# wexiangis/wmix

Hardware: AMD Instinct MI355X
Metric: 10 ms frames/s (higher is better)
Workload: dtype f32

## Files before the change

include/wmix_amd.h:

```cpp
#ifndef WMIX_AMD_H
#define WMIX_AMD_H

#include <stddef.h>
#include <stdint.h>

#ifdef __cplusplus
extern "C" {
#endif

#define WMX_EINVAL (-10001)
#define WMX_ENODEV (-10002)
#define WMX_ESTATE (-10003)
#define WMX_EHIP_BASE (-11000)
#define WMX_IS_HIP_ERROR(rc) ((rc) <= WMX_EHIP_BASE && (rc) > WMX_EHIP_BASE - 10000)

const char *wmx_last_error(void);
int wmx_device_count(void);
int wmx_handle_device(const void *handle);
int wmx_version(void);
const char *wmx_build_info(void);



#define WMX_LAW_A 0
// ... 227 lines not shown
int wmx_rtp_reset_streams(wmx_rtp *h, const int32_t *host_idx, int n, void *stream);
int wmx_rtp_export(wmx_rtp *h, int stream_index, uint16_t *seq, uint32_t *timestamp);
#define WMX_RTP_SEQ_MISORDER 16
#define WMX_RTP_CALLS_COUNT(c) ((c) & 7u)
#define WMX_RTP_CALLS_SLOT(c, j) (((c) >> (4 + 4 * (j))) & 3u)
#define WMX_RTP_CALLS_SILENCE(c, j) (((c) >> (6 + 4 * (j))) & 1u)
int wmx_rtp_sequence_legs(wmx_rtp *h, int max_packets, int max_gap, const uint16_t *d_seq_raw, uint32_t *d_len, uint32_t *d_calls,
                          void *stream);
int wmx_rtp_reset_sequence(wmx_rtp *h, const int32_t *host_idx, int n, void *stream);
int wmx_rtp_export_sequence(wmx_rtp *h, uint16_t *next, uint8_t *synced, uint32_t *lost, uint32_t *late, uint32_t *dup,
                            uint32_t *resync, uint32_t *overflow, void *stream);
int wmx_rtp_conceal_legs(wmx_rtp *h, int max_packets, const int16_t *d_pcm, long source_stride, long pcm_packet_stride,
                         const uint32_t *d_len, const uint32_t *d_calls, int16_t *d_pcm_out, uint32_t *d_len_out, void *stream);
int wmx_rtp_reset_conceal(wmx_rtp *h, const int32_t *host_idx, int n, void *stream);
int wmx_rtp_export_conceal(wmx_rtp *h, int16_t *hist, uint32_t *concealed, void *stream);
int wmx_rtp_detect_dtmf_legs(wmx_rtp *h, int max_packets, const uint8_t *d_in, long leg_stride, long packet_stride,
                             const int32_t *d_recv, int16_t *d_pcm, long source_stride, long pcm_packet_stride, const uint32_t *d_len,
                             const uint32_t *d_calls, int event_pt, int suppress, void *stream);
int wmx_rtp_reset_dtmf(wmx_rtp *h, const int32_t *host_idx, int n, void *stream);
int wmx_rtp_export_dtmf(wmx_rtp *h, uint32_t *count, uint8_t *ring, void *stream);
#define WMX_CODEC_REFERENCE 0
#define WMX_CODEC_PCMA 1
#define WMX_CODEC_PCMU 2
#define WMX_CODEC_BY_PT 3
int wmx_rtp_set_codecs(wmx_rtp *h, const int32_t *host_idx, int n, int in_codec, int out_law, void *stream);
int wmx_rtp_export_codecs(wmx_rtp *h, uint8_t *in_codec, uint8_t *out_law, uint32_t *refused, void *stream);
int wmx_rtp_ingest_legs_codecs(wmx_rtp *h, int max_packets, const uint8_t *d_packets, long leg_stride, long packet_stride,
                               const int32_t *d_recv_bytes, int16_t *d_pcm, long source_stride, long pcm_packet_stride,
                               uint32_t *d_len, uint16_t *d_seq_raw, void *stream);

typedef struct wmx_pipe wmx_pipe;
int wmx_pipe_create(wmx_pipe **out, int n_streams, int slots, int law, int agc_value, unsigned stages);
int wmx_pipe_create_pcm(wmx_pipe **out, int n_streams, int slots, int chn, int freq, int interval_ms, int agc_value, unsigned stages);
int wmx_pipe_create_pcm_calls(wmx_pipe **out, int n_streams, int slots, int chn, int freq, int interval_ms, int agc_value, unsigned stages);
int wmx_pipe_destroy(wmx_pipe *h);
int wmx_pipe_slots(const wmx_pipe *h);
int wmx_pipe_datagram_bytes(const wmx_pipe *h);
uint8_t *wmx_pipe_in(wmx_pipe *h, int slot);
const uint8_t *wmx_pipe_out(wmx_pipe *h, int slot);
int16_t *wmx_pipe_far(wmx_pipe *h, int slot);
int wmx_pipe_submit(wmx_pipe *h, const int16_t *d_far, int *slot, void *stream);
int wmx_pipe_wait(wmx_pipe *h, int slot);
long wmx_pipe_failed_steps(const wmx_pipe *h);
int wmx_pipe_poll(wmx_pipe *h, int slot);
int wmx_pipe_step_resident(wmx_pipe *h, const uint8_t *d_in, long in_stride, const int16_t *d_far, uint8_t *d_out, long out_stride,
                           void *stream);
wmx_chain *wmx_pipe_chain(wmx_pipe *h);
wmx_rtp *wmx_pipe_senders(wmx_pipe *h);

typedef struct wmx_conf wmx_conf;
int wmx_conf_create(wmx_conf **out, int n_legs, int slots, int max_packets, int law);
int wmx_conf_destroy(wmx_conf *h);
int wmx_conf_set_conferences(wmx_conf *h, int n_conf, const int32_t *host_off, const int32_t *host_members, void *stream);
int wmx_conf_mute(wmx_conf *h, const uint8_t *host_mask, void *stream);
int wmx_conf_speakers(wmx_conf *h, int max_speakers, uint32_t floor, int decay_shift);
int wmx_conf_sequence(wmx_conf *h, int on, int max_gap);
int wmx_conf_export_sequence(wmx_conf *h, uint16_t *next, uint8_t *synced, uint32_t *lost, uint32_t *late, uint32_t *dup,
                             uint32_t *resync, uint32_t *overflow, void *stream);
int wmx_conf_conceal(wmx_conf *h, int on);
int wmx_conf_export_conceal(wmx_conf *h, uint32_t *concealed, void *stream);
int wmx_conf_dtmf(wmx_conf *h, int on, int suppress, int event_pt);
int wmx_conf_export_dtmf(wmx_conf *h, uint32_t *count, uint8_t *ring, void *stream);
int wmx_conf_denoise(wmx_conf *h, int on);
wmx_nsx *wmx_conf_denoiser(wmx_conf *h);
int wmx_conf_level(wmx_conf *h, int on, int value);
wmx_agc *wmx_conf_leveller(wmx_conf *h);
int wmx_conf_gate(wmx_conf *h, int on);
wmx_vad *wmx_conf_gater(wmx_conf *h);
int wmx_conf_export_gate(wmx_conf *h, uint8_t *reduce, uint32_t *voiced, uint32_t *unvoiced, void *stream);
int wmx_conf_set_codecs(wmx_conf *h, const int32_t *host_idx, int n, int in_codec, int out_law, void *stream);
int wmx_conf_export_codecs(wmx_conf *h, uint8_t *in_codec, uint8_t *out_law, uint32_t *refused, void *stream);
int wmx_conf_set_play_correct(wmx_conf *h, uint32_t bytes);
int wmx_conf_reset_legs(wmx_conf *h, const int32_t *host_idx, int n, void *stream);
int wmx_conf_slots(const wmx_conf *h);
int wmx_conf_in_row_bytes(const wmx_conf *h);
uint8_t *wmx_conf_in(wmx_conf *h, int slot);
int32_t *wmx_conf_recv(wmx_conf *h, int slot);
const uint8_t *wmx_conf_out(wmx_conf *h, int slot);
int wmx_conf_next_slot(const wmx_conf *h);
int wmx_conf_submit(wmx_conf *h, int *slot, void *stream);
int wmx_conf_wait(wmx_conf *h, int slot);
int wmx_conf_poll(wmx_conf *h, int slot);
int wmx_conf_step_resident(wmx_conf *h, const uint8_t *d_in, const int32_t *d_recv, uint8_t *d_out, void *stream);
int wmx_conf_export_legs(wmx_conf *h, uint32_t *head, uint32_t *tick, uint32_t *dropped, uint32_t *env, uint8_t *speaking, void *stream);
wmx_mix *wmx_conf_mix(wmx_conf *h);
wmx_rtp *wmx_conf_senders(wmx_conf *h);

typedef struct wmx_rt wmx_rt;
int wmx_rt_create_pcm(wmx_rt **out, long n_streams, int sub_batch, int slots, int chn, int freq, int interval_ms, int agc_value, unsigned stages);
int wmx_rt_create_rtp(wmx_rt **out, long n_streams, int sub_batch, int slots, int law, int agc_value, unsigned stages);
int wmx_rt_create_pcm_calls(wmx_rt **out, long n_streams, int sub_batch, int slots, int chn, int freq, int interval_ms, int agc_value, unsigned stages);
int wmx_rt_destroy(wmx_rt *h);
int wmx_rt_set_compute_streams(wmx_rt *h, int n);
int wmx_rt_batches(const wmx_rt *h);
int wmx_rt_batch_streams(const wmx_rt *h, int batch);
wmx_pipe *wmx_rt_pipe(wmx_rt *h, int batch);
int16_t *wmx_rt_far(wmx_rt *h, int slot);
int wmx_rt_submit(wmx_rt *h, const int16_t *d_far, int *slot, void *stream);
#define WMX_DROPPED 1
int wmx_rt_try_submit(wmx_rt *h, const int16_t *d_far, int *slot, void *stream);
long wmx_rt_dropped_ticks(const wmx_rt *h);
int wmx_rt_next_slot(const wmx_rt *h);
int wmx_rt_wait(wmx_rt *h);
int wmx_rt_poll(wmx_rt *h);
int wmx_rt_tick(wmx_rt *h, const int16_t *d_far, int *slot, void *stream);
int wmx_rt_step_resident(wmx_rt *h, uint8_t *d_rows, long stride, const int16_t *d_far, uint8_t *d_out, long out_stride, void *stream);

typedef struct wmx_pkgfifo wmx_pkgfifo;
int wmx_pkgfifo_create(wmx_pkgfifo **out, int n_streams, int n_slots, int pkg_bytes, int interval_ms, int frame_bytes);
int wmx_pkgfifo_destroy(wmx_pkgfifo *h);
int wmx_pkgfifo_add(wmx_pkgfifo *h, const uint8_t *d_pkgs, long stride, void *stream);
int wmx_pkgfifo_get(wmx_pkgfifo *h, uint8_t *d_out, long stride, int delayms, void *stream);

typedef struct wmx_tick wmx_tick;
int wmx_tick_create(wmx_tick **out, int n_groups, int rec_per_group, int chn, int freq, int interval_ms, int aec_delay_ms, int agc_value,
                    unsigned stages);
int wmx_tick_destroy(wmx_tick *h);
int wmx_tick_set_stages(wmx_tick *h, unsigned stages, int agc_value);
int wmx_tick_play_ns(wmx_tick *h, int on);
int wmx_tick_rw_test(wmx_tick *h, int on);
int wmx_tick_bridge(wmx_tick *h, int parties);
int wmx_tick_bridge_mute(wmx_tick *h, const uint8_t *host_mask, void *stream);
int wmx_tick_bridge_conferences(wmx_tick *h, int n_conf, const int32_t *host_off, const int32_t *host_members, void *stream);
int wmx_tick_bridge_speakers(wmx_tick *h, int max_speakers, uint32_t floor, int decay_shift);
int wmx_tick_bridge_speaking(wmx_tick *h, uint8_t *host_speaking, uint32_t *host_env, void *stream);
int wmx_tick_set_play_correct(wmx_tick *h, uint32_t bytes);
int wmx_tick_package_samples(const wmx_tick *h);
int wmx_tick_load(wmx_tick *h, const int16_t *d_src, uint32_t srcU8Len, int freq, int channels, int sample, int n_src, long group_stride,
                  long source_stride, int reduce, uint32_t *head, uint32_t *tick, void *stream);
int wmx_tick_play(wmx_tick *h, int16_t *d_play, long play_stride, void *stream);
const int16_t *wmx_tick_far(const wmx_tick *h);
int wmx_tick_record(wmx_tick *h, int16_t *d_rec, long rec_stride, int16_t *d_rec_1x8000, long out_stride, uint32_t out_capacity,
                    uint32_t *out_len, void *stream);
int wmx_tick_run(wmx_tick *h, int16_t *d_play, long play_stride, int16_t *d_rec, long rec_stride, int16_t *d_rec_1x8000, long out_stride,
                 uint32_t out_capacity, uint32_t *out_len, void *stream);
wmx_mix *wmx_tick_mix(wmx_tick *h);
wmx_chain *wmx_tick_chain(wmx_tick *h);
wmx_pkgfifo *wmx_tick_fifo(wmx_tick *h);

int wmx_debug_fft(int kind, int n_batch, void *d_data, int32_t *d_aux, void *stream);
int wmx_debug_spl(int kind, const int32_t *d_a, const int32_t *d_b, const int32_t *d_c, int32_t *d_y, size_t n, void *stream);
int wmx_debug_ns_libm(int kind, const float *x, float *y, size_t n);
int wmx_debug_ns_libm_device(int kind, const float *d_x, const float *d_a, const float *d_b, float *d_y, size_t n, void *stream);
int wmx_debug_ns_libm_dbl(int kind, const float *x, double *y, size_t n);
int wmx_debug_ns_libm_dbl_device(int kind, const float *d_x, double *d_y, size_t n, void *stream);
int wmx_debug_aec_libm_device(int kind, const float *d_x, float *d_y, size_t n, void *stream);
int wmx_debug_ns_window(int L, float *host_window);
int wmx_debug_div(const float *d_a, const float *d_b, float *d_q_ordinary, float *d_q_ieee, size_t n, void *stream);
int wmx_debug_div_host(const float *a, const float *b, float *q, size_t n);
int wmx_debug_aec_decide(const float *sd_rows, const float *se_rows, const int32_t *prev_state, int32_t *out, size_t n);
int wmx_debug_aec_decide_device(const float *d_sd_rows, const float *d_se_rows, const int32_t *d_prev_state, int32_t *d_out, size_t n, void *stream);
int wmx_debug_pow(const float *x, const float *e, float *y, size_t n);
int wmx_debug_pow_device(const float *d_x, const float *d_e, float *d_y, size_t n, void *stream);

#ifdef __cplusplus
}
#endif
#endif
```

wmix_amd/csrc/aec.hip:

```cpp
#include <algorithm>
#include <chrono>
#include <cmath>
#include <cstdlib>
#include <cstring>
#include <cstddef>
#include <unordered_map>
#include <vector>
#include "wmx_internal.h"
#include "aec_ctl.h"
#include "aec_gate.h"
#include "cohort_hip.h"
#include "fft_regs.h"
#include "libm_dev.h"

namespace wmx {
namespace {

constexpr int BP = 68;
enum : int {
    AS_W_RE = 0,
    AS_W_IM = AS_W_RE + 12 * BP,
    AS_DPOW = AS_W_IM + 12 * BP,
    AS_DMIN = AS_DPOW + BP,
    AS_DINIT = AS_DMIN + BP,
    AS_SD = AS_DINIT + BP,
    AS_SE = AS_SD + BP,
    AS_SX = AS_SE + BP,
    AS_SDE_RE = AS_SX + BP,
    AS_SDE_IM = AS_SDE_RE + BP,
    AS_SXD_RE = AS_SDE_IM + BP,
    AS_SXD_IM = AS_SXD_RE + BP,
    AS_DPREV = AS_SXD_IM + BP,
    AS_EPREV = AS_DPREV + 64,
    AS_OUTBUF = AS_EPREV + 64,
    AS_NEAR_RING = AS_OUTBUF + 64,
    AS_OUT_RING = AS_NEAR_RING + kAecRing,
    AS_SCAL = AS_OUT_RING + kAecRing,
    AS_HNLFBMIN = AS_SCAL + 0,
    AS_HNLFBLOCALMIN = AS_SCAL + 1,
    AS_HNLXDAVGMIN = AS_SCAL + 2,
    AS_OVERDRIVE = AS_SCAL + 3,
    AS_OVERDRIVESM = AS_SCAL + 4,
    AS_HNLNEWMIN = AS_SCAL + 5,
    AS_HNLMINCTR = AS_SCAL + 6,
    AS_DELAYIDX = AS_SCAL + 7,
    AS_STNEAR = AS_SCAL + 8,
    AS_ECHOSTATE = AS_SCAL + 9,
    AS_DIVERGE = AS_SCAL + 10,
    AS_NOISECTR = AS_SCAL + 12,
    AS_DELAYCTR = AS_SCAL + 13,
    AS_NSEED = AS_SCAL + 11,
    AS_WORDS = AS_SCAL + 16,
};
static_assert(AS_WORDS % 4 == 0, "state block must be a whole number of 16-byte chunks");

struct AecFarBufs {
    float *pre;
    float *tring;
    float *hist;
    float *nyq;
    float *hist_w;
    float *xpow_seq;
    float *xpow;
    size_t group_words;
};
__device__ __forceinline__ AecFarBufs far_group(const AecFarBufs &F, int g) {
    const size_t o = (size_t)g * F.group_words;
    return AecFarBufs{F.pre + o, F.tring + o, F.hist + o, F.nyq + o, F.hist_w + o, F.xpow_seq + o, F.xpow + o, F.group_words};
}

struct AecConsts {
    FftTables tab;
    float hanning[BP], weight[BP], overdrive[BP];
};
constexpr int kAecConstWords = sizeof(AecConsts) / 4;
struct AecConstsNear {
    FftTables tab;
    float hanning[BP];
};
static_assert(offsetof(AecConsts, weight) == sizeof(AecConstsNear), "AecConstsNear is a prefix of AecConsts");
constexpr int kAecConstNearWords = sizeof(AecConstsNear) / 4;

__device__ __forceinline__ float sat16f(float v) { return v > 32767.f ? 32767.f : (v < -32768.f ? -32768.f : v); }

__device__ __forceinline__ v2f cmul_conj_w(float wr, float wi, v2f t) { return v2f{wr, wr} * t + v2f{wi, -wi} * swap(t); }

__device__ __forceinline__ void unpack_bin(const float *a, int b, float &re, float &im) {
    if (b == 0) {
        re = a[0];
        im = 0.f;
    } else if (b == kAecPart) {
        re = a[1];
        im = 0.f;
    } else {
        re = a[2 * b];
        im = a[2 * b + 1];
    }
}

template <class Src>
__device__ __forceinline__ void aec_fft_fwd(float *row, const FftTables *T, int gl, Src src) {
    Cx v[4];
#pragma unroll
    for (int m = 0; m < 4; m++) v[m] = src(fft64_src_point(gl, m));
    fft64_regs<false>(v, T, gl);
#pragma unroll
    for (int m = 0; m < 4; m++) *reinterpret_cast<float2 *>(row + 2 * (gl + 16 * m)) = make_float2(v[m].r, v[m].i);
}

__global__ __launch_bounds__(64) void aec_far_kernel(AecFarBufs F_all, const float *__restrict__ consts_g, AecPlan *plans,
                                                     int n_packets, int n_classes, const int32_t *__restrict__ plan_of,
                                                     const int16_t *far_pcm, long far_packet_stride,
                                                     long far_group_stride, int chn, float gpow1np, int plan_by_value,
                                                     const AecPlan plan_value) {
    __shared__ AecConstsNear K;
    __shared__ float fa[4][132];
    const int lane = threadIdx.x;
    if (plan_by_value) {
        const int *src = reinterpret_cast<const int *>(&plan_value);
        int *dst = reinterpret_cast<int *>(plans);
        constexpr int NW = (int)(sizeof(AecPlan) / 4), NIT = (NW + 63) / 64;
        int v[NIT];
#pragma unroll
        for (int k = 0; k < NIT; k++) v[k] = src[lane + 64 * k < NW ? lane + 64 * k : 0];
#pragma unroll
        for (int k = 0; k < NIT; k++)
            if (lane + 64 * k < NW) dst[lane + 64 * k] = v[k];
        __threadfence();
        wave_sync();
    }
    const AecFarBufs F = far_group(F_all, (int)blockIdx.x);
    if (far_pcm) far_pcm += (size_t)blockIdx.x * far_group_stride;
    plans += plan_of ? plan_of[blockIdx.x] : (int)blockIdx.x;
    __shared__ float lpre[kAecPreLen];
    float xp0, xp1;
    {
        float *dst = reinterpret_cast<float *>(&K);
        constexpr int NIT = (kAecConstNearWords + 63) / 64, NP = kAecPreLen / 64;
        static_assert(kAecPreLen % 64 == 0, "whole rows of the pre-buffer per lane");
        float c[NIT], pr[NP];
#pragma unroll
        for (int k = 0; k < NIT; k++) c[k] = consts_g[lane + 64 * k < kAecConstNearWords ? lane + 64 * k : 0];
#pragma unroll
        for (int k = 0; k < NP; k++) pr[k] = F.pre[lane + 64 * k];
        xp0 = F.xpow[lane];
        xp1 = F.xpow[lane == 0 ? kAecPart : 0];
#pragma unroll
        for (int k = 0; k < NIT; k++)
            if (lane + 64 * k < kAecConstNearWords) dst[lane + 64 * k] = c[k];
#pragma unroll
        for (int k = 0; k < NP; k++) lpre[lane + 64 * k] = pr[k];
    }
    wave_sync();
    bool xpow_dirty = false;
    __shared__ int lplan[sizeof(AecPlan) / 4];
    for (int p = 0; p < n_packets; p++) {
        {
            const int *src = reinterpret_cast<const int *>(&plans[(size_t)p * n_classes]);
            constexpr int NW = (int)(sizeof(AecPlan) / 4);
            static_assert(NW <= 64, "one word of the plan per lane");
            wave_sync();
            if (lane < NW) lplan[lane] = src[lane];
            wave_sync();
        }
        const AecPlan &lp = *reinterpret_cast<const AecPlan *>(lplan);
        auto rf = [](int v) { return __builtin_amdgcn_readfirstlane(v); };
        struct {
            int has_far, far_n, pre_wr, n_part, n_blk;
            int pre_rd[4], pslot[4], bslot[4], hist_n[4], unwritten[4];
        } pl;
        pl.has_far = rf(lp.has_far);
        pl.far_n = rf(lp.far_n);
        pl.pre_wr = rf(lp.pre_wr);
        pl.n_part = rf(lp.n_part);
        pl.n_blk = rf(lp.n_blk);
#pragma unroll
        for (int q = 0; q < 4; q++) {
            pl.pre_rd[q] = rf(lp.part[q].pre_rd);
            pl.pslot[q] = rf(lp.part[q].far_slot);
            pl.bslot[q] = rf(lp.blk[q].far_slot);
            pl.hist_n[q] = rf(lp.blk[q].hist_n);
            pl.unwritten[q] = rf(lp.blk[q].flags) & kAecFlagFarUnwritten;
        }
        const bool consume = rf(lp.has_near) && !rf(lp.passthrough);
        unsigned tw[4];
        if (consume) {
#pragma unroll
            for (int k = 0; k < 4; k++) {
                if (k >= pl.n_blk) break;
                tw[k] = reinterpret_cast<const unsigned *>(F.tring)[(size_t)pl.bslot[k] * 64 + lane];
            }
        }
        if (pl.has_far) {
            const int16_t *src = far_pcm + (size_t)p * far_packet_stride;
            {
                int16_t s3[3];
#pragma unroll
                for (int j = 0; j < 3; j++) s3[j] = src[(lane + 64 * j < pl.far_n ? lane + 64 * j : 0) * chn];
#pragma unroll
                for (int j = 0; j < 3; j++)
                    if (lane + 64 * j < pl.far_n) {
                        const int at = (pl.pre_wr + lane + 64 * j) % kAecPreLen;
                        lpre[at] = (float)s3[j];
                        F.pre[at] = (float)s3[j];
                    }
            }
            wave_sync();
#pragma unroll
            for (int q = 0; q < 4; q++) {
                if (q >= pl.n_part) break;
                const float a = lpre[(pl.pre_rd[q] + 2 * lane) % kAecPreLen], b = lpre[(pl.pre_rd[q] + 2 * lane + 1) % kAecPreLen];
                reinterpret_cast<unsigned *>(F.tring)[(size_t)pl.pslot[q] * 64 + lane] =
                    (unsigned)(unsigned short)(short)a | ((unsigned)(unsigned short)(short)b << 16);
            }
            wave_sync();
        }
        if (consume) {
            const int gl = fft_index(lane), grp = fft_group(lane);
#pragma unroll
            for (int k0 = 0; k0 < 4; k0 += 2) {
                if (k0 >= pl.n_blk) break;
#pragma unroll
                for (int j = 0; j < 2; j++) {
                    const int k = k0 + j;
                    if (k >= pl.n_blk || pl.unwritten[k]) continue;
                    float t0 = (float)(short)(tw[k] & 0xffffu), t1 = (float)(short)(tw[k] >> 16);
                    if (pl.has_far) {
#pragma unroll
                        for (int q = 0; q < 4; q++) {
                            if (q >= pl.n_part) break;
                            if (pl.pslot[q] != pl.bslot[k]) continue;
                            t0 = lpre[(pl.pre_rd[q] + 2 * lane) % kAecPreLen];
                            t1 = lpre[(pl.pre_rd[q] + 2 * lane + 1) % kAecPreLen];
                        }
                    }
                    const int i0 = 2 * lane, i1 = 2 * lane + 1;
                    fa[2 * j][i0] = t0;
                    fa[2 * j][i1] = t1;
                    fa[2 * j + 1][i0] = t0 * (i0 < kAecPart ? K.hanning[i0] : K.hanning[2 * kAecPart - i0]);
                    fa[2 * j + 1][i1] = t1 * (i1 < kAecPart ? K.hanning[i1] : K.hanning[2 * kAecPart - i1]);
                }
                wave_sync();
#ifndef WMX_AEC_EXP_NOFARFFT
                aec_fft_fwd(fa[grp], &K.tab, gl, [&](int p) {
                    const v2f c = ld_pt(fa[grp], p);
                    return Cx{c.x, c.y};
                });
#endif
                wave_sync();
                const SplitLane cf = rdft128_fwd_coef(&K.tab, lane);
#pragma unroll
                for (int j = 0; j < 2; j++) {
                    const int k = k0 + j;
                    if (k >= pl.n_blk) continue;
                    v2f P = v2f{0.f, 0.f}, Wd = v2f{0.f, 0.f};
                    float xr64 = 0.f, w64 = 0.f;
                    const float xi64 = 0.f;
                    if (!pl.unwritten[k]) {
                        P = rdft128_fwd_bin_u(fa[2 * j], cf, lane);
                        Wd = rdft128_fwd_bin_u(fa[2 * j + 1], cf, lane);
                        if (lane == 0) P.y = 0.f, Wd.y = 0.f;
                        xr64 = fa[2 * j][0] - fa[2 * j][1];
                        w64 = fa[2 * j + 1][0] - fa[2 * j + 1][1];
                    }
                    const int hs = pl.hist_n[k] % kAecHist;
                    F.hist[hs * 130 + lane] = P.x;
                    F.hist[hs * 130 + kAecPart1 + lane] = P.y;
                    F.hist[(hs + kAecHist) * 130 + lane] = P.x;
                    F.hist[(hs + kAecHist) * 130 + kAecPart1 + lane] = P.y;
                    F.hist_w[hs * 130 + lane] = Wd.x;
                    F.hist_w[hs * 130 + kAecPart1 + lane] = Wd.y;
                    if (lane < 2) {
                        const int at = lane == 0 ? kAecPart : kAecPart1 + kAecPart;
                        F.hist[hs * 130 + at] = lane == 0 ? xr64 : xi64;
                        F.hist[(hs + kAecHist) * 130 + at] = lane == 0 ? xr64 : xi64;
                        F.hist_w[hs * 130 + at] = lane == 0 ? w64 : 0.f;
                    }
                    if (lane < 4) F.nyq[2 * (hs + (lane >> 1) * kAecHist) + (lane & 1)] = (lane & 1) ? xi64 : xr64;
                    {
                        const float xr = P.x, xi = P.y;
                        const float far_spectrum = (xr * xr) + (xi * xi);
                        xp0 = 0.9f * xp0 + gpow1np * far_spectrum;
                        F.xpow_seq[hs * BP + lane] = xp0;
                    }
                    {
                        const float far_spectrum = (xr64 * xr64) + (xi64 * xi64);
                        xp1 = 0.9f * xp1 + gpow1np * far_spectrum;
                        if (lane == 0) F.xpow_seq[hs * BP + kAecPart] = xp1;
                    }
                    xpow_dirty = true;
                }
                wave_sync();
            }
        }
    }
    if (xpow_dirty) {
        F.xpow[lane] = xp0;
        if (lane == 0) F.xpow[kAecPart] = xp1;
    }
}

constexpr int kAecWavesPerBlock = 4;
#ifdef WMX_AEC_PROF
__device__ unsigned long long g_aec_prof[16];
#define AEC_PROF(i)                                                              \
    do {                                                                         \
        const long long t_now = clock64();                                       \
        if (lane == 0) W.prof[i] += (unsigned long long)(t_now - t_prev);        \
        t_prev = clock64();                                                      \
    } while (0)
#define AEC_PROF_START long long t_prev = clock64()
#elif defined(WMX_AEC_EXP_BARRIERS)
#define AEC_PROF(i) __builtin_amdgcn_s_barrier()
#define AEC_PROF_START
#else
#define AEC_PROF(i)
#define AEC_PROF_START
#endif
#ifdef WMX_AEC_GATE_PROF
__device__ unsigned long long g_aec_gate[2];
#endif
constexpr int AS_LDS0 = AS_DPOW;
constexpr int AS_LDS_WORDS = AS_WORDS - AS_DPOW;
#ifndef WMX_AEC_FAS
#define WMX_AEC_FAS 138
#endif
constexpr int FAS = WMX_AEC_FAS;

struct alignas(16) AecWaveLds {
    float st[AS_LDS_WORDS];
    float wn[24];
    float fa[8][FAS];
    float cur[64], enew[64];
    int16_t park[kAecFrame];
#ifdef WMX_AEC_PROF
    unsigned long long prof[16];
#endif
};
#define AEC_ST(x) W.st[(x) - AS_LDS0]

struct AecTaps {
    v2f t[12];
};

__device__ __forceinline__ float uniform_ld(const float *p) {
    return *reinterpret_cast<const float __attribute__((address_space(4))) *>(reinterpret_cast<size_t>(p));
}

typedef const float __attribute__((address_space(1))) *GlobalRow;
__device__ __forceinline__ GlobalRow uniform_row(const float *base, int row, int row_words) {
    const float *p = base + (size_t)row * row_words;
    asm volatile("" : "+s"(p));
    return (GlobalRow)p;
}

__device__ __forceinline__ float row_ld(GlobalRow row, unsigned lane_bytes, int word) {
    return *(GlobalRow)((const char __attribute__((address_space(1))) *)(row + word) + lane_bytes);
}

constexpr int kHistRowBytes = 130 * 4, kHistMid = 2860;
struct HistRows {
    GlobalRow base;
    unsigned voff;
};
__device__ __forceinline__ unsigned hist_row_now(int n) { return ((unsigned)n & (unsigned)(kAecHist - 1)) + (unsigned)kAecHist; }
__device__ __forceinline__ HistRows hist_rows(const float *hist, int n, int lane) {
    return HistRows{uniform_row(hist, 0, 0), hist_row_now(n) * (unsigned)kHistRowBytes - (unsigned)kHistMid + 4u * (unsigned)lane};
}
__device__ __forceinline__ void wait_vm() { __builtin_amdgcn_s_waitcnt(0x0f70); }
__device__ __forceinline__ float hist_ld(const HistRows &H, int p, int word) {
    const long imm = kHistMid - kHistRowBytes * p + 4 * word;
    return *(GlobalRow)((const char __attribute__((address_space(1))) *)H.base + (size_t)H.voff + imm);
}

__device__ __noinline__ static float aec_powf(float x, float y, const PowTables *__restrict__ t) { return fast_pow(x, y, t); }

__device__ __forceinline__ int ring_at(int pos, int i) {
    const int t = pos + i;
    return t >= kAecRing ? t - kAecRing : t;
}
__device__ __forceinline__ float *fa_row(AecWaveLds &W, int r) { return &W.fa[0][0] + __umul24((unsigned)r, (unsigned)FAS); }
__device__ __forceinline__ int opaque_lane(int x) {
#ifndef WMX_AEC_HOIST
    asm volatile("" : "+v"(x));
#endif
    __builtin_assume(x >= 0 && x < 64);
    return x;
}

template <int MULT>
__device__ __forceinline__ void aec_block(const AecConstsNear &K, const float *__restrict__ curves_g, const PowTables *__restrict__ powtab, AecWaveLds &W, AecTaps &taps,
                                          const AecFarBufs &F, const AecBlkPlan &bp, const AecNoiseEntry *__restrict__ noise_tab, const int lane_in) {
    int lane = opaque_lane(lane_in);
    int *Si = reinterpret_cast<int *>(W.st) - AS_LDS0;
    const float mu = MULT == 1 ? 0.6f : 0.5f, err_thr = MULT == 1 ? 2e-6f : 1.5e-6f;
    const float scale = 2.0f / 128;
    const int n = bp.hist_n;
    int blk_flags;
    {
        int nctr = __builtin_amdgcn_readfirstlane(Si[AS_NOISECTR]), dctr = __builtin_amdgcn_readfirstlane(Si[AS_DELAYCTR]);
        blk_flags = nctr > 50 ? kAecFlagNoiseMin : 0;
        if (nctr < 500 * MULT) {
            nctr++;
            blk_flags |= kAecFlagNoiseInit;
        }
        dctr++;
        if (dctr == 10 * MULT) dctr = 0;
        if (dctr == 0) blk_flags |= kAecFlagDelayEst;
        if (lane == 0) {
            Si[AS_NOISECTR] = nctr;
            Si[AS_DELAYCTR] = dctr;
        }
    }
    int g = fft_group(lane), gl = fft_index(lane);
#define AEC_RELANE()              \
    do {                          \
        lane = opaque_lane(lane); \
        g = fft_group(lane);      \
        gl = fft_index(lane);     \
    } while (0)
    float *xw = W.fa[1], *dw = W.fa[2], *ew = W.fa[3];
    float *t0 = W.fa[4], *t1 = W.fa[5], *t2 = W.fa[6], *t3 = W.fa[7];
    AEC_PROF_START;

    const unsigned xpow_row = ((unsigned)n & (unsigned)(kAecHist - 1)) * (unsigned)BP;
    const float xpow_lane = row_ld(uniform_row(F.xpow_seq, 0, 0), 4u * (xpow_row + (unsigned)lane), 0);
    W.cur[lane] = AEC_ST(AS_NEAR_RING + ring_at(bp.near_rd, lane));
    wave_sync();
    AEC_PROF(0);
    AEC_RELANE();
    {
        float xr[12], xi[12];
        const HistRows H = hist_rows(F.hist, n, lane);
#pragma unroll
        for (int p = 0; p < 12; p++) {
            xr[p] = hist_ld(H, p, 0);
            xi[p] = hist_ld(H, p, kAecPart1);
        }
        wait_vm();
        const float *NQ = F.nyq + 2 * (hist_row_now(n) - 11);
        typedef float v8f __attribute__((ext_vector_type(8)));
        typedef const v8f __attribute__((address_space(4), aligned(8))) *ConstV8;
        const ConstV8 NQ8 = reinterpret_cast<ConstV8>(reinterpret_cast<size_t>(NQ));
        v8f nq[3];
#pragma unroll
        for (int j = 0; j < 3; j++) nq[j] = NQ8[j];
        float y64 = 0.f;
        v2f y2 = v2f{0.f, 0.f};
#pragma unroll
        for (int p = 0; p < 12; p++) {
            y2 = y2 + cmul_w(xr[p], xi[p], taps.t[p]);
            const float nr = nq[(2 * (11 - p)) >> 3][(2 * (11 - p)) & 7];
            y64 += nr * W.wn[p];
        }
        AEC_PROF(1);
        v2f pt = rdft128_inv_point_lanes(v2f{y2.x, lane == 0 ? y64 : y2.y}, &K.tab, lane);
        pt = fft64_lanes<true>(pt, &K.tab, lane);
        if (lane >= 32) {
            const int i = 2 * (lane - 32);
            W.enew[i] = W.cur[i] - pt.x * scale;
            W.enew[i + 1] = W.cur[i + 1] - pt.y * scale;
        }
    }
    wave_sync();
    AEC_RELANE();
    {
        const bool win = g & 1, err = g >= 2;
        aec_fft_fwd(W.fa[g], &K.tab, gl, [&](int p) {
            const int i = 2 * (p & 31);
            float x0, x1, h0, h1;
            if (p < 32) {
                const float *prev = &AEC_ST(err ? AS_EPREV : AS_DPREV);
                x0 = prev[i], x1 = prev[i + 1];
                h0 = K.hanning[i], h1 = K.hanning[i + 1];
                if (g == 2) x0 = 0.f, x1 = 0.f;
            } else {
                const float *now = err ? W.enew : W.cur;
                x0 = now[i], x1 = now[i + 1];
                h0 = K.hanning[kAecPart - i], h1 = K.hanning[kAecPart - i - 1];
            }
            return Cx{win ? x0 * h0 : x0, win ? x1 * h1 : x1};
        });
    }
    wave_sync();
    AEC_PROF(2);
    AEC_RELANE();
    float dwr, dwi, dw64, dfr, dfi, df64;
    {
        const SplitLane cf = rdft128_fwd_coef(&K.tab, lane);
        const v2f dwb = rdft128_fwd_bin_u(W.fa[1], cf, lane), dfb = rdft128_fwd_bin_u(W.fa[0], cf, lane);
        dwr = dwb.x, dwi = dwb.y, dw64 = W.fa[1][0] - W.fa[1][1];
        dfr = dfb.x, dfi = dfb.y, df64 = W.fa[0][0] - W.fa[0][1];
    }
    {
        struct Pw {
            float dpow, dmin, dinit;
        };
        auto power = [&](int b, float re, float im) {
            Pw r;
            const float ns = re * re + im * im;
            r.dpow = 0.9f * AEC_ST(AS_DPOW + b) + 0.1f * ns;
            r.dmin = AEC_ST(AS_DMIN + b);
            if (blk_flags & kAecFlagNoiseMin) {
                const float down = (r.dpow + 0.1f * (r.dmin - r.dpow)) * 1.0002f, up = r.dmin * 1.0002f;
                r.dmin = r.dpow < r.dmin ? down : up;
            }
            r.dinit = 0.f;
            if (blk_flags & kAecFlagNoiseInit) {
                r.dinit = AEC_ST(AS_DINIT + b);
                const float track = 0.999f * r.dinit + 0.001f * r.dmin;
                r.dinit = r.dmin > r.dinit ? track : r.dmin;
            }
            return r;
        };
        auto put = [&](int b, const Pw &r) {
            AEC_ST(AS_DPOW + b) = r.dpow;
            if (blk_flags & kAecFlagNoiseMin) AEC_ST(AS_DMIN + b) = r.dmin;
            if (blk_flags & kAecFlagNoiseInit) AEC_ST(AS_DINIT + b) = r.dinit;
        };
        const Pw a = power(lane, dfr, dfi);
        put(lane, a);
#if !defined(WMX_AEC_EXP) || WMX_AEC_EXP < 1
        const Pw c = power(kAecPart, df64, 0.f);
        if (lane == 0) put(kAecPart, c);
#endif
    }
    float ewr, ewi, ew64, efr, efi, ef64r, ef64i = 0.f;
    {
        {
            const SplitLane cf = rdft128_fwd_coef(&K.tab, lane);
            const v2f ewb = rdft128_fwd_bin_u(W.fa[3], cf, lane), efb = rdft128_fwd_bin_u(W.fa[2], cf, lane);
            ewr = ewb.x, ewi = ewb.y, ew64 = W.fa[3][0] - W.fa[3][1];
            efr = efb.x, efi = efb.y, ef64r = W.fa[2][0] - W.fa[2][1];
        }
        auto scale_err = [&](float xp, float &er, float &ei) {
            er /= (xp + 1e-10f);
            ei /= (xp + 1e-10f);
            float abs_ef = sqrtf(er * er + ei * ei);
            if (abs_ef > err_thr) {
                abs_ef = err_thr / (abs_ef + 1e-10f);
                er *= abs_ef;
                ei *= abs_ef;
            }
            er *= mu;
            ei *= mu;
        };
        const float xp64 = uniform_ld(F.xpow_seq + xpow_row + kAecPart);
        scale_err(xpow_lane, efr, efi);
#if !defined(WMX_AEC_EXP) || WMX_AEC_EXP < 1
        scale_err(xp64, ef64r, ef64i);
#else
        ef64r *= xp64;
#endif
    }
    wave_sync();
    AEC_RELANE();
    const float e64r = ef64r, e64i = ef64i;
    const int delayIdx0 = Si[AS_DELAYIDX];
    float xwr_pre = 0.f, xwi_pre = 0.f;
#pragma unroll
    for (int pass = 0; pass < 2; pass++) {
        const int base = 8 * pass, cnt = pass == 0 ? 8 : 4;
        if (pass == 1) {
            const unsigned xw_row = ((unsigned)(n - delayIdx0) & (unsigned)(kAecHist - 1)) * 130u;
            const GlobalRow Xw = uniform_row(F.hist_w, 0, 0);
            xwr_pre = row_ld(Xw, 4u * (xw_row + (unsigned)lane), 0);
            xwi_pre = row_ld(Xw, 4u * (xw_row + (unsigned)lane), kAecPart1);
        }
        float nyq_r, nyq_i;
        {
            const unsigned l = (unsigned)lane < 11u ? (unsigned)lane : 11u;
            const v2f v = *reinterpret_cast<const v2f __attribute__((address_space(1))) *>(
                (const char __attribute__((address_space(1))) *)uniform_row(F.nyq, 0, 0) + 8u * (hist_row_now(n) - (unsigned)base - l));
            nyq_r = v.x;
            nyq_i = -v.y;
        }
        {
            float xr[8], xi[8];
            const HistRows H = hist_rows(F.hist, n, lane);
#pragma unroll
            for (int q = 0; q < 8; q++) {
                if (q >= cnt) continue;
                xr[q] = hist_ld(H, base + q, 0);
                xi[q] = hist_ld(H, base + q, kAecPart1);
            }
            wait_vm();
#pragma unroll
            for (int q = 0; q < 8; q++) {
                if (q >= cnt) continue;
                st_pt(W.fa[q], lane, cmul_conj_w(xr[q], xi[q], v2f{efr, efi}));
            }
        }
        wave_sync();
        if (lane < cnt) fa_row(W, lane)[1] = nyq_r * e64r - nyq_i * e64i;
        wave_sync();
        AEC_RELANE();
        if (pass == 0) {
            float *row0 = W.fa[g], *row1 = W.fa[4 + g];
            Cx2 v[4];
#pragma unroll
            for (int m = 0; m < 4; m++) v[m] = rdft128_inv_point_x2(row0, row1, &K.tab, gl, m);
            fft64_regs_x2<true>(v, &K.tab, gl);
            const v2f sc = bc(scale), z = bc(0.f);
            const v2f ar = v[0].r * sc, ai = v[0].i * sc, cr = v[1].r * sc, ci = v[1].i * sc;
            v[0] = Cx2{v2f{row_bitrev(ar.x, lane), row_bitrev(ar.y, lane)}, v2f{row_bitrev(ai.x, lane), row_bitrev(ai.y, lane)}};
            v[2] = Cx2{v2f{row_bitrev(cr.x, lane), row_bitrev(cr.y, lane)}, v2f{row_bitrev(ci.x, lane), row_bitrev(ci.y, lane)}};
            v[1] = Cx2{z, z};
            v[3] = Cx2{z, z};
            fft64_regs_x2<false>(v, &K.tab, gl);
#pragma unroll
            for (int m = 0; m < 4; m++) {
                *reinterpret_cast<float2 *>(row0 + 2 * (gl + 16 * m)) = make_float2(v[m].r.x, v[m].i.x);
                *reinterpret_cast<float2 *>(row1 + 2 * (gl + 16 * m)) = make_float2(v[m].r.y, v[m].i.y);
            }
        } else {
            float *row = W.fa[g];
            Cx v[4];
            {
                const v2f p0 = rdft128_inv_point_m<0>(row, &K.tab, gl), p1 = rdft128_inv_point_m<1>(row, &K.tab, gl);
                const v2f p2 = rdft128_inv_point_m<2>(row, &K.tab, gl), p3 = rdft128_inv_point_m<3>(row, &K.tab, gl);
                v[0] = Cx{p0.x, p0.y}, v[1] = Cx{p1.x, p1.y}, v[2] = Cx{p2.x, p2.y}, v[3] = Cx{p3.x, p3.y};
                fft64_regs<true>(v, &K.tab, gl);
            }
            const Cx a = Cx{row_bitrev(v[0].r * scale, lane), row_bitrev(v[0].i * scale, lane)};
            const Cx c = Cx{row_bitrev(v[1].r * scale, lane), row_bitrev(v[1].i * scale, lane)};
            v[0] = a;
            v[1] = Cx{0.f, 0.f};
            v[2] = c;
            v[3] = Cx{0.f, 0.f};
            fft64_regs<false>(v, &K.tab, gl);
#pragma unroll
            for (int m = 0; m < 4; m++) *reinterpret_cast<float2 *>(row + 2 * (gl + 16 * m)) = make_float2(v[m].r, v[m].i);
        }
        wave_sync();
        AEC_RELANE();
        {
            const SplitLane cf = rdft128_fwd_coef(&K.tab, lane);
#pragma unroll
            for (int q = 0; q < 8; q++) {
                if (q >= cnt) continue;
                const v2f d = rdft128_fwd_bin_u(W.fa[q], cf, lane);
                taps.t[base + q] = taps.t[base + q] + d;
            }
            if (lane < cnt) W.wn[base + lane] += fa_row(W, lane)[0] - fa_row(W, lane)[1];
        }
        wave_sync();
    }
    AEC_PROF(3);

    AEC_RELANE();
    constexpr int prefSize = 24 / MULT, minPref = 4 / MULT;
    const float gc0 = MULT == 1 ? 0.9f : 0.93f, gc1 = MULT == 1 ? 0.1f : 0.07f;
    int delayIdx = delayIdx0;
    if (blk_flags & kAecFlagDelayEst) {
#pragma unroll
        for (int p = 0; p < 12; p++) {
            float *dst = W.fa[p >> 1] + (p & 1) * 66;
            dst[lane] = taps.t[p].x * taps.t[p].x + taps.t[p].y * taps.t[p].y;
            if (lane == 0) dst[64] = W.wn[p] * W.wn[p] + 0.f * 0.f;
        }
        wave_sync();
        if (lane < 12) {
            const float *src = W.fa[lane >> 1] + (lane & 1) * 66;
            float en = 0.f;
            for (int j = 0; j < kAecPart1; j++) en += src[j];
            W.wn[12 + lane] = en;
        }
        wave_sync();
        float best = 0.f;
        delayIdx = 0;
        for (int p = 0; p < 12; p++)
            if (W.wn[12 + p] > best) {
                best = W.wn[12 + p];
                delayIdx = p;
            }
        wave_sync();
        if (lane == 0) Si[AS_DELAYIDX] = delayIdx;
    }
    AEC_PROF(4);
    {
        const float *Xw = F.hist_w + (size_t)(((unsigned)(n - delayIdx) & (unsigned)(kAecHist - 1)) * 130u);
        if (delayIdx != delayIdx0) {
            xwr_pre = Xw[lane];
            xwi_pre = Xw[kAecPart1 + lane];
        }
        xw[lane] = xwr_pre;
        xw[66 + lane] = xwi_pre;
        if (lane == 0) {
            xw[kAecPart] = uniform_ld(Xw + kAecPart);
            xw[66 + kAecPart] = uniform_ld(Xw + kAecPart1 + kAecPart);
        }
        dw[lane] = dwr;
        dw[66 + lane] = dwi;
        ew[lane] = ewr;
        ew[66 + lane] = ewi;
        if (lane == 0) {
            dw[kAecPart] = dw64;
            dw[66 + kAecPart] = 0.f;
            ew[kAecPart] = ew64;
            ew[66 + kAecPart] = 0.f;
        }
    }
    wave_sync();
    AecGate gate = AecGate{0, 0, 0};
    {
        struct Psd {
            float sd, se, sx, sde_r, sde_i, sxd_r, sxd_i;
        };
        auto psd = [&](int b) {
            const float dr = dw[b], di = dw[66 + b], er = ew[b], ei = ew[66 + b];
            const float xr = xw[b], xi = xw[66 + b];
            Psd r;
            r.sd = gc0 * AEC_ST(AS_SD + b) + gc1 * (dr * dr + di * di);
            r.se = gc0 * AEC_ST(AS_SE + b) + gc1 * (er * er + ei * ei);
            const float xx = xr * xr + xi * xi;
            r.sx = gc0 * AEC_ST(AS_SX + b) + gc1 * (xx > 15.f ? xx : 15.f);
            r.sde_r = gc0 * AEC_ST(AS_SDE_RE + b) + gc1 * (dr * er + di * ei);
            r.sde_i = gc0 * AEC_ST(AS_SDE_IM + b) + gc1 * (dr * ei - di * er);
            r.sxd_r = gc0 * AEC_ST(AS_SXD_RE + b) + gc1 * (dr * xr + di * xi);
            r.sxd_i = gc0 * AEC_ST(AS_SXD_IM + b) + gc1 * (dr * xi - di * xr);
            return r;
        };
        auto put = [&](int b, const Psd &r) {
            AEC_ST(AS_SX + b) = r.sx;
            AEC_ST(AS_SD + b) = r.sd;
            AEC_ST(AS_SE + b) = r.se;
            AEC_ST(AS_SDE_RE + b) = r.sde_r;
            AEC_ST(AS_SDE_IM + b) = r.sde_i;
            AEC_ST(AS_SXD_RE + b) = r.sxd_r;
            AEC_ST(AS_SXD_IM + b) = r.sxd_i;
        };
        const Psd a = psd(lane);
        put(lane, a);
#if !defined(WMX_AEC_EXP) || WMX_AEC_EXP < 1
        const Psd c = psd(kAecPart);
        if (lane == 0) put(kAecPart, c);
        float sd_t = a.sd, se_t = a.se;
        aec_gate_wave_sums(sd_t, se_t);
        gate = aec_gate_decide(sd_t + c.sd, se_t + c.se, Si[AS_DIVERGE]);
        gate.decided = __builtin_amdgcn_readfirstlane(gate.decided);
#endif
    }
    wave_sync();
    AEC_PROF(5);
    int diverge = gate.diverge;
    bool reset_filter = gate.reset;
#ifdef WMX_AEC_GATE_PROF
    if (lane == 0) atomicAdd(&g_aec_gate[gate.decided ? 0 : 1], 1ull);
#endif
    if (!gate.decided) {
        float sdSum, seSum;
#if defined(WMX_AEC_EXP) && WMX_AEC_EXP >= 2
        sdSum = AEC_ST(AS_SD), seSum = AEC_ST(AS_SE + 1);
#else
        aec_gate_ordered_sums(&AEC_ST(AS_SD), &AEC_ST(AS_SE), lane, sdSum, seSum);
#endif
        diverge = ((Si[AS_DIVERGE] ? 1.05f : 1.0f) * seSum > sdSum) ? 1 : 0;
        reset_filter = seSum > (19.95f * sdSum);
    }
    wave_sync();
    if (lane == 0) Si[AS_DIVERGE] = diverge;
    if (reset_filter) {
#pragma unroll
        for (int p = 0; p < 12; p++) {
            taps.t[p] = v2f{0.f, 0.f};
            if (lane == 0) W.wn[p] = 0.f;
        }
    }
    AEC_PROF(6);
    AEC_RELANE();
    const uint32_t nseed = (uint32_t)__builtin_amdgcn_readfirstlane(Si[AS_NSEED]);
    const uint2 *jump = reinterpret_cast<const uint2 *>(noise_tab + kAecNoiseTab);
    const uint2 jl = jump[(lane + 63) & 63], j64 = jump[63];
    const AecNoiseEntry nz = noise_tab[((nseed * jl.x + jl.y) & 0x7FFFFFFFu) >> 16];
    const float nz_c = nz.c, nz_s = nz.s;
    if (lane == 0) Si[AS_NSEED] = (int)((nseed * j64.x + j64.y) & 0x7FFFFFFFu);
    {
        auto coh = [&](int b, float &cde, float &cxd) {
            const float sde_r = AEC_ST(AS_SDE_RE + b), sde_i = AEC_ST(AS_SDE_IM + b), sxd_r = AEC_ST(AS_SXD_RE + b),
                        sxd_i = AEC_ST(AS_SXD_IM + b);
            cde = (sde_r * sde_r + sde_i * sde_i) / (AEC_ST(AS_SD + b) * AEC_ST(AS_SE + b) + 1e-10f);
            cxd = (sxd_r * sxd_r + sxd_i * sxd_i) / (AEC_ST(AS_SX + b) * AEC_ST(AS_SD + b) + 1e-10f);
        };
        float a0, a1, c0, c1;
        coh(lane, a0, a1);
#if !defined(WMX_AEC_EXP) || WMX_AEC_EXP < 1
        coh(kAecPart, c0, c1);
#else
        c0 = a0, c1 = a1;
#endif
        if (diverge) {
            ew[lane] = dw[lane];
            ew[66 + lane] = dw[66 + lane];
        }
        t0[lane] = a0;
        t1[lane] = a1;
        if (lane == 0) {
            if (diverge) {
                ew[kAecPart] = dw[kAecPart];
                ew[66 + kAecPart] = dw[66 + kAecPart];
            }
            t0[kAecPart] = c0;
            t1[kAecPart] = c1;
        }
    }
    wave_sync();
    float hNlXdAvg, hNlDeAvg;
#if defined(WMX_AEC_EXP) && WMX_AEC_EXP >= 2
    hNlXdAvg = t1[5] * prefSize, hNlDeAvg = t0[5] * prefSize;
#else
    {
        const float *mine = lane == 1 ? t0 : t1;
        float acc = 0.f;
#pragma unroll
        for (int i = minPref; i < prefSize + minPref; i++) acc += mine[i];
        hNlXdAvg = __int_as_float(__builtin_amdgcn_readlane(__float_as_int(acc), 0));
        hNlDeAvg = __int_as_float(__builtin_amdgcn_readlane(__float_as_int(acc), 1));
    }
#endif
    hNlXdAvg /= prefSize;
    hNlXdAvg = 1 - hNlXdAvg;
    hNlDeAvg /= prefSize;
    float hNlXdAvgMin = AEC_ST(AS_HNLXDAVGMIN), hNlFbMin = AEC_ST(AS_HNLFBMIN), hNlFbLocalMin = AEC_ST(AS_HNLFBLOCALMIN);
    float overDrive = AEC_ST(AS_OVERDRIVE), overDriveSm = AEC_ST(AS_OVERDRIVESM);
    int stNear = Si[AS_STNEAR], echoState, hNlNewMin = Si[AS_HNLNEWMIN], hNlMinCtr = Si[AS_HNLMINCTR];
    if (hNlXdAvg < 0.75f && hNlXdAvg < hNlXdAvgMin) hNlXdAvgMin = hNlXdAvg;
    if (hNlDeAvg > 0.98f && hNlXdAvg > 0.9f)
        stNear = 1;
    else if (hNlDeAvg < 0.95f || hNlXdAvg < 0.8f)
        stNear = 0;
    int mode;
    float hNlFb, hNlFbLow;
    if (hNlXdAvgMin == 1) {
        echoState = 0;
        overDrive = 5.0f;
        if (stNear == 1) {
            mode = 0;
            hNlFb = hNlDeAvg;
            hNlFbLow = hNlDeAvg;
        } else {
            mode = 1;
            hNlFb = hNlXdAvg;
            hNlFbLow = hNlXdAvg;
        }
    } else {
        if (stNear == 1) {
            echoState = 0;
            mode = 0;
            hNlFb = hNlDeAvg;
            hNlFbLow = hNlDeAvg;
        } else {
            echoState = 1;
            mode = 2;
            hNlFb = 0.f;
            hNlFbLow = 0.f;
        }
    }
    for (int b = lane; b < kAecPart1; b += 64) {
        const float cde = t0[b], cxd = 1 - t1[b];
        t2[b] = mode == 0 ? cde : (mode == 1 ? cxd : (cde < cxd ? cde : cxd));
    }
    wave_sync();
#if defined(WMX_AEC_EXP) && WMX_AEC_EXP >= 2
    if (mode == 3) {
#else
    if (mode == 2) {
#endif
        constexpr int i75 = (int)(0.75f * (prefSize - 1)), i50 = (int)(0.5f * (prefSize - 1));
        if (lane < prefSize) {
            const float v = t2[minPref + lane];
            int rank = 0;
            for (int i = 0; i < prefSize; i++) {
                const float u = t2[minPref + i];
                rank += (u < v || (u == v && i < lane)) ? 1 : 0;
            }
            if (rank == i75) t3[0] = v;
            if (rank == i50) t3[1] = v;
        }
        wave_sync();
        hNlFb = t3[0];
        hNlFbLow = t3[1];
        wave_sync();
    }
    if (hNlFbLow < 0.6f && hNlFbLow < hNlFbLocalMin) {
        hNlFbLocalMin = hNlFbLow;
        hNlFbMin = hNlFbLow;
        hNlNewMin = 1;
        hNlMinCtr = 0;
    }
    {
        float t = hNlFbLocalMin + 0.0008f / MULT;
        hNlFbLocalMin = t < 1 ? t : 1;
        t = hNlXdAvgMin + 0.0006f / MULT;
        hNlXdAvgMin = t < 1 ? t : 1;
    }
    if (hNlNewMin == 1) hNlMinCtr++;
    if (hNlMinCtr == 2) {
        hNlNewMin = 0;
        hNlMinCtr = 0;
        const float od = -18.4f / (log_d(hNlFbMin + 1e-10f) + 1e-10f);
        overDrive = od > 5.0f ? od : 5.0f;
    }
    if (overDrive < overDriveSm)
        overDriveSm = 0.99f * overDriveSm + 0.01f * overDrive;
    else
        overDriveSm = 0.9f * overDriveSm + 0.1f * overDrive;
    if (lane == 0) {
        AEC_ST(AS_HNLXDAVGMIN) = hNlXdAvgMin;
        AEC_ST(AS_HNLFBMIN) = hNlFbMin;
        AEC_ST(AS_HNLFBLOCALMIN) = hNlFbLocalMin;
        AEC_ST(AS_OVERDRIVE) = overDrive;
        AEC_ST(AS_OVERDRIVESM) = overDriveSm;
        Si[AS_STNEAR] = stNear;
        Si[AS_ECHOSTATE] = echoState;
        Si[AS_HNLNEWMIN] = hNlNewMin;
        Si[AS_HNLMINCTR] = hNlMinCtr;
    }
    AEC_PROF(7);
    AEC_RELANE();
    const int noise_off = (blk_flags & kAecFlagNoiseInit) ? AS_DINIT : AS_DMIN;
    v2f out_spec = v2f{0.f, 0.f};
    float out_nyq = 0.f;
#if defined(WMX_AEC_EXP) && WMX_AEC_EXP >= 1
    for (int b = lane; b < kAecPart; b += 64) {
#else
    for (int b = lane; b < kAecPart1; b += 64) {
#endif
        float h = t2[b];
        const float wc = curves_g[b];
        if (h > hNlFb) h = wc * hNlFb + (1 - wc) * h;
        h = aec_powf(h, overDriveSm * curves_g[BP + b], powtab);
        float er = ew[b] * h, ei = ew[66 + b] * h;
        ei *= -1;
        float ur = 0.f, ui = 0.f;
        if (b >= 1) {
            const float noise = sqrtf(AEC_ST(noise_off + b));
            ur = noise * nz_c;
            ui = -noise * nz_s;
            if (b == kAecPart) ui = 0.f;
        }
        const float v = 1 - h * h;
        const float tmp = sqrtf(v > 0 ? v : 0);
        er += tmp * ur;
        ei += tmp * ui;
        if (b == kAecPart)
            out_nyq = er;
        else
            out_spec = v2f{er, -ei};
    }
    AEC_PROF(8);
    AEC_RELANE();
    {
        if (lane == 0) out_spec.y = out_nyq;
        v2f pt = rdft128_inv_point_lanes(out_spec, &K.tab, lane);
        pt = fft64_lanes<true>(pt, &K.tab, lane);
        const int i = 2 * (lane & 31);
        if (lane < 32) {
            const float o0 = sat16f(pt.x * scale * K.hanning[i] + AEC_ST(AS_OUTBUF + i));
            const float o1 = sat16f(pt.y * scale * K.hanning[i + 1] + AEC_ST(AS_OUTBUF + i + 1));
            AEC_ST(AS_OUT_RING + ring_at(bp.out_wr, i)) = o0;
            AEC_ST(AS_OUT_RING + ring_at(bp.out_wr, i + 1)) = o1;
        }
        wave_sync();
        if (lane >= 32) {
            AEC_ST(AS_OUTBUF + i) = pt.x * scale * K.hanning[kAecPart - i];
            AEC_ST(AS_OUTBUF + i + 1) = pt.y * scale * K.hanning[kAecPart - i - 1];
        }
    }
    AEC_ST(AS_DPREV + lane) = W.cur[lane];
    AEC_ST(AS_EPREV + lane) = W.enew[lane];
    wave_sync();
    AEC_PROF(9);
#undef AEC_RELANE
}

template <int MULT>
#ifndef WMX_AEC_WAVES
#define WMX_AEC_WAVES 4
#endif
__global__ __attribute__((amdgpu_waves_per_eu(WMX_AEC_WAVES, WMX_AEC_WAVES))) __launch_bounds__(64 * kAecWavesPerBlock) void aec_near_kernel(float *__restrict__ state, AecFarBufs F_all,
                                                                          const float *__restrict__ consts_g,
                                                                          const AecPlan *__restrict__ plans, int n_packets, int n_classes,
                                                                          const int32_t *__restrict__ plan_of,
                                                                          const AecNoiseEntry *__restrict__ noise_tab,
                                                                          const int16_t *near_pcm, int16_t *out_pcm, int n_streams,
                                                                          long stream_stride, long packet_stride, int chn, int pkg,
                                                                          const int *__restrict__ stream_far, const uint8_t *__restrict__ active,
                                                                          const int *__restrict__ order) {
    __shared__ AecConstsNear K;
    __shared__ AecWaveLds Wv[kAecWavesPerBlock];
    const int lane = threadIdx.x & 63;
    const int wave = __builtin_amdgcn_readfirstlane(threadIdx.x >> 6);
    int sidx;
    if (order) {
        const unsigned i = blockIdx.x, per = gridDim.x >> 3;
        sidx = __builtin_amdgcn_readfirstlane(order[((i & 7u) * per + (i >> 3)) * kAecWavesPerBlock + wave]);
    } else {
        sidx = blockIdx.x * kAecWavesPerBlock + wave;
    }
    const bool live = sidx >= 0 && stream_active(active, sidx, n_streams);
    const int sl = (sidx >= 0 && sidx < n_streams) ? sidx : 0;
    const int grp = stream_far ? __builtin_amdgcn_readfirstlane(stream_far[sl]) : 0;
    const AecFarBufs F = far_group(F_all, grp);
    plans += plan_of ? __builtin_amdgcn_readfirstlane(plan_of[grp]) : grp;
    float *gst = state + (size_t)sl * AS_WORDS;
    constexpr int kConstIt = (kAecConstNearWords + 64 * kAecWavesPerBlock - 1) / (64 * kAecWavesPerBlock);
    float kc[kConstIt];
#pragma unroll
    for (int k = 0; k < kConstIt; k++) {
        const int i = threadIdx.x + 64 * kAecWavesPerBlock * k;
        kc[k] = consts_g[i < kAecConstNearWords ? i : 0];
    }
    int16_t pcm0[2][2];
    {
        const int16_t *in0 = near_pcm + (size_t)sl * stream_stride;
#pragma unroll
        for (int s = 0; s < 2; s++)
#pragma unroll
            for (int h = 0; h < 2; h++) {
                const int i = lane + 64 * h;
                const bool want = i < kAecFrame && s * kAecFrame + i < pkg;
                const int16_t v = in0[want ? (s * kAecFrame + i) * chn : 0];
                pcm0[s][h] = want ? v : (int16_t)0;
            }
    }
    AecTaps taps;
#pragma unroll
    for (int p = 0; p < 12; p++) {
        taps.t[p].x = gst[AS_W_RE + p * BP + lane];
        taps.t[p].y = gst[AS_W_IM + p * BP + lane];
    }
    const float wn0 = gst[AS_W_RE + (lane < 12 ? lane : 0) * BP + kAecPart];
    constexpr int kChunks = (AS_LDS_WORDS / 4 + 63) / 64;
    float4 c[kChunks];
    {
        const float4 *g4 = reinterpret_cast<const float4 *>(gst + AS_LDS0);
#pragma unroll
        for (int k = 0; k < kChunks; k++) {
            const int i = lane + 64 * k;
            c[k] = g4[i < AS_LDS_WORDS / 4 ? i : i - 64];
        }
    }
#pragma unroll
    for (int k = 0; k < kConstIt; k++) {
        const int i = threadIdx.x + 64 * kAecWavesPerBlock * k;
        if (i < kAecConstNearWords) reinterpret_cast<float *>(&K)[i] = kc[k];
    }
    asm volatile("s_waitcnt lgkmcnt(0)\n\ts_barrier" ::: "memory");
    if (!live) return;
    const PowTables *powtab = reinterpret_cast<const PowTables *>(consts_g + kAecConstWords);
    AecWaveLds &W = Wv[wave];
#ifdef WMX_AEC_PROF
    if (lane < 16) W.prof[lane] = 0;
#endif
    AEC_PROF_START;
    if (lane < 12) W.wn[lane] = wn0;
    {
        float4 *s4 = reinterpret_cast<float4 *>(W.st);
#pragma unroll
        for (int k = 0; k < kChunks; k++) {
            const int i = lane + 64 * k;
            s4[i < AS_LDS_WORDS / 4 ? i : i - 64] = c[k];
        }
    }
#pragma unroll
    for (int h = 0; h < 2; h++) {
        const int i = lane + 64 * h;
        if (i < kAecFrame) {
            W.fa[0][i] = (float)pcm0[0][h];
            W.park[i] = pcm0[1][h];
        }
    }
    wave_sync();
    AEC_PROF(10);
    for (int p = 0; p < n_packets; p++) {
        const AecPlan &pl = plans[(size_t)p * n_classes];
        if (!pl.has_near) continue;
        const size_t off = (size_t)sidx * stream_stride + (size_t)p * packet_stride;
        const int16_t *in = near_pcm + off;
        int16_t *out = out_pcm + off;
        const bool keep = pl.has_near != kAecNearDiscard;
        if (pl.passthrough) {
            for (int i = lane; keep && i < pkg; i += 64) {
                const int16_t v = in[i * chn];
                for (int c = 0; c < chn; c++) out[i * chn + c] = v;
            }
            continue;
        }
        for (int s = 0; s < pl.n_sub; s++) {
            const AecSubPlan &sp = pl.sub[s];
            const int ln = opaque_lane(lane);
#pragma unroll
            for (int h = 0; h < 2; h++) {
                const int i = ln + 64 * h;
                if (i >= kAecFrame) continue;
                const float v = (p == 0 && s < 2) ? (s == 0 ? W.fa[0][i] : (float)W.park[i]) : (float)in[(s * kAecFrame + i) * chn];
                AEC_ST(AS_NEAR_RING + ring_at(sp.near_wr, i)) = v;
            }
            wave_sync();
            for (int k = 0; k < sp.n_blocks; k++)
                aec_block<MULT>(K, consts_g + kAecConstNearWords, powtab, W, taps, F, pl.blk[sp.first_blk + k], noise_tab, lane);
            for (int i = opaque_lane(lane); keep && i < kAecFrame; i += 64) {
                const int16_t v = (int16_t)AEC_ST(AS_OUT_RING + ring_at(sp.out_rd, i));
                for (int c = 0; c < chn; c++) out[(s * kAecFrame + i) * chn + c] = v;
            }
            wave_sync();
        }
    }
    wave_sync();
    AEC_PROF(11);
    asm volatile("" : "+s"(gst));
    float __attribute__((address_space(1))) *gout = (float __attribute__((address_space(1))) *)gst;
    const int ln = opaque_lane(lane);
#pragma unroll
    for (int p = 0; p < 12; p++) {
        gout[AS_W_RE + p * BP + ln] = taps.t[p].x;
        gout[AS_W_IM + p * BP + ln] = taps.t[p].y;
// ... 699 lines not shown
```

wmix_amd/csrc/fft_ooura.h:

```cpp
#pragma once
#include <hip/hip_runtime.h>
#include <cmath>
#include <cstring>
#include "wmx_internal.h"

namespace wmx {

struct FftTables {
    float w2;
    float pad[3];
    float W1[32][2];
    float W2[32][2];
    float W3[32][2];
    float c[64];
};
static_assert(sizeof(FftTables) == (4 + 64 * 3 + 64) * 4, "FftTables layout");
constexpr int kFftTableWords = sizeof(FftTables) / 4;

inline int host_bitrev(int q, int bits) {
    int r = 0;
    for (int b = 0; b < bits; b++)
        if (q & (1 << b)) r |= 1 << (bits - 1 - b);
    return r;
}

inline void host_expand_twiddles(const float *w, int n, FftTables *t) {
    volatile float tmp;
    t->w2 = w[2];
    t->W1[0][0] = t->W2[0][0] = t->W3[0][0] = 1.f;
    t->W1[1][0] = w[2];
    t->W2[1][1] = 1.f;
    t->W3[1][0] = -w[2];
    for (int b = 2; b < n / 8; b++) {
        int k1 = 2 * (b >> 1), k2 = 2 * k1;
        float wk2r = w[k1], wk2i = w[k1 + 1], wk1r, wk1i, two;
        if ((b & 1) == 0) {
            wk1r = w[k2];
            wk1i = w[k2 + 1];
            two = 2 * wk2i;
            t->W2[b][0] = wk2r;
            t->W2[b][1] = wk2i;
        } else {
            wk1r = w[k2 + 2];
            wk1i = w[k2 + 3];
            two = 2 * wk2r;
            t->W2[b][0] = -wk2i;
            t->W2[b][1] = wk2r;
        }
        tmp = two * wk1i;
        t->W3[b][0] = wk1r - tmp;
        tmp = two * wk1r;
        t->W3[b][1] = tmp - wk1i;
        t->W1[b][0] = wk1r;
        t->W1[b][1] = wk1i;
    }
}

inline void fft_tables_ooura(int n, FftTables *t) {
    std::memset(t, 0, sizeof(*t));
    float w[64];
    const int nw = n >> 2, nwh = nw >> 1;
    {
        float delta = (float)atan(1.0f) / nwh;
        w[0] = 1;
        w[1] = 0;
        w[nwh] = (float)cos(delta * nwh);
        w[nwh + 1] = w[nwh];
        for (int j = 2; j < nwh; j += 2) {
            float x = (float)cos(delta * j), y = (float)sin(delta * j);
            w[j] = x;
            w[j + 1] = y;
            w[nw - j] = y;
            w[nw - j + 1] = x;
        }
        int bits = 0;
        while ((1 << bits) < nwh) bits++;
        for (int q = 0; q < nwh; q++) {
            int r = host_bitrev(q, bits);
            if (r > q) {
                float a = w[2 * q], b = w[2 * q + 1];
                w[2 * q] = w[2 * r];
                w[2 * q + 1] = w[2 * r + 1];
                w[2 * r] = a;
                w[2 * r + 1] = b;
            }
        }
    }
    {
        const int nc = n >> 2, nch = nc >> 1;
        float delta = (float)atan(1.0f) / nch;
        t->c[0] = (float)cos(delta * nch);
        t->c[nch] = 0.5f * t->c[0];
        for (int j = 1; j < nch; j++) {
            t->c[j] = 0.5f * (float)cos(delta * j);
            t->c[nc - j] = 0.5f * (float)sin(delta * j);
        }
    }
    host_expand_twiddles(w, n, t);
}

inline void fft_tables_aec128(FftTables *t) {
    static const unsigned kW[64] = {
        0x3f800000, 0x00000000, 0x3f3504f3, 0x3f3504f3, 0x3f6c835f, 0x3ec3ef16, 0x3ec3ef16, 0x3f6c835f,
        0x3f7b14be, 0x3e47c5c2, 0x3f0e39da, 0x3f54db31, 0x3f54db31, 0x3f0e39da, 0x3e47c5c2, 0x3f7b14be,
        0x3f7ec46d, 0x3dc8bd36, 0x3f22679a, 0x3f45e403, 0x3f61c598, 0x3ef15aea, 0x3e94a031, 0x3f74fa0b,
        0x3f74fa0b, 0x3e94a031, 0x3ef15aea, 0x3f61c598, 0x3f45e403, 0x3f22679a, 0x3dc8bd36, 0x3f7ec46d,
        0x3f3504f3, 0x3effb10f, 0x3efec46d, 0x3efd3aac, 0x3efb14be, 0x3ef853f8, 0x3ef4fa0b, 0x3ef10908,
        0x3eec835f, 0x3ee76bd7, 0x3ee1c598, 0x3edb941a, 0x3ed4db31, 0x3ecd9f02, 0x3ec5e403, 0x3ebdaefa,
        0x3eb504f3, 0x3eabeb4a, 0x3ea2679a, 0x3e987fc0, 0x3e8e39da, 0x3e839c3d, 0x3e715aea, 0x3e5ae880,
        0x3e43ef16, 0x3e2c7cd4, 0x3e14a031, 0x3df8cfcd, 0x3dc7c5c2, 0x3d964083, 0x3d48bd36, 0x3cc8fb30,
    };
    std::memset(t, 0, sizeof(*t));
    float w[64];
    std::memcpy(w, kW, sizeof(w));
    std::memcpy(t->c, w + 32, 32 * sizeof(float));
    host_expand_twiddles(w, 128, t);
}


__device__ __forceinline__ int dev_bitrev(int q, int bits) { return (int)(__brev((unsigned)q) >> (32 - bits)); }

struct Cx { float r, i; };

typedef float v2f __attribute__((ext_vector_type(2)));
__device__ __forceinline__ v2f cx(Cx a) { return v2f{a.r, a.i}; }
__device__ __forceinline__ v2f swap(v2f a) { return __builtin_shufflevector(a, a, 1, 0); }
#define WMX_PK_ADD(name, mods)                                                      \
    __device__ __forceinline__ v2f name(v2f a, v2f b) {                             \
        v2f d;                                                                      \
        asm("v_pk_add_f32 %0, %1, %2 " mods : "=v"(d) : "v"(a), "v"(b));           \
        return d;                                                                   \
    }
WMX_PK_ADD(add_i, "op_sel:[0,1] op_sel_hi:[1,0] neg_lo:[0,1]")
WMX_PK_ADD(sub_i, "op_sel:[0,1] op_sel_hi:[1,0] neg_hi:[0,1]")
WMX_PK_ADD(add_swap, "op_sel:[0,1] op_sel_hi:[1,0]")
WMX_PK_ADD(sub_swap, "op_sel:[0,1] op_sel_hi:[1,0] neg_lo:[0,1] neg_hi:[0,1]")
WMX_PK_ADD(add_conj, "neg_hi:[0,1]")
WMX_PK_ADD(sub_conj, "neg_lo:[0,1]")
WMX_PK_ADD(conj_sub, "neg_hi:[1,1]")
WMX_PK_ADD(conj_add, "neg_lo:[0,1] neg_hi:[1,0]")
#undef WMX_PK_ADD
__device__ __forceinline__ v2f cmul_w(float wr, float wi, v2f t) { return v2f{wr, wr} * t + v2f{-wi, wi} * swap(t); }

__device__ __forceinline__ void bfly4_v(int b, const FftTables *T, v2f v[4]) {
    const v2f x0 = v[0] + v[1], x1 = v[0] - v[1], x2 = v[2] + v[3], x3 = v[2] - v[3];
    v[0] = x0 + x2;
    const float m = b == 1 ? 1.f : 0.f;
    const float w1r = T->W1[b][0], w1i = T->W1[b][1], w2r = T->W2[b][0], w2i = T->W2[b][1];
    const float w3r = T->W3[b][0], w3i = T->W3[b][1];
    v2f t1 = add_i(x1, x3);
    v2f t3 = sub_i(x1, x3);
    t1 = __builtin_elementwise_fma(v2f{-m, m}, swap(t1), t1);
    t3 = __builtin_elementwise_fma(v2f{m, -m}, swap(t3), t3);
    v[2] = cmul_w(w2r, w2i, x0 - x2);
    v[1] = cmul_w(w1r, w1i, t1);
    v[3] = cmul_w(w3r, w3i, t3);
}

__device__ __forceinline__ void bfly4(int b, const FftTables *T, Cx A, Cx B, Cx C, Cx D, float2 &o0, float2 &o1, float2 &o2,
                                      float2 &o3) {
    v2f v[4] = {cx(A), cx(B), cx(C), cx(D)};
    bfly4_v(b, T, v);
    o0 = make_float2(v[0].x, v[0].y);
    o1 = make_float2(v[1].x, v[1].y);
    o2 = make_float2(v[2].x, v[2].y);
    o3 = make_float2(v[3].x, v[3].y);
}

__device__ __forceinline__ void bfly4_store(float *a, int p0, int hc, int b, const FftTables *T, Cx A, Cx B, Cx C, Cx D) {
    const int p1 = p0 + hc, p2 = p1 + hc, p3 = p2 + hc;
    float2 o0, o1, o2, o3;
    bfly4(b, T, A, B, C, D, o0, o1, o2, o3);
    *reinterpret_cast<float2 *>(a + 2 * p0) = o0;
    *reinterpret_cast<float2 *>(a + 2 * p1) = o1;
    *reinterpret_cast<float2 *>(a + 2 * p2) = o2;
    *reinterpret_cast<float2 *>(a + 2 * p3) = o3;
}

template <bool INVERSE>
__device__ __forceinline__ void bfly4_close_v(v2f v[4]) {
    const v2f x2 = v[2] + v[3], x3 = v[2] - v[3];
    if constexpr (!INVERSE) {
        const v2f x0 = v[0] + v[1], x1 = v[0] - v[1];
        v[0] = x0 + x2;
        v[2] = x0 - x2;
        v[1] = add_i(x1, x3);
        v[3] = sub_i(x1, x3);
    } else {
        const v2f x0 = conj_sub(v[0], v[1]), x1 = conj_add(v[0], v[1]);
        v[0] = add_conj(x0, x2);
        v[2] = sub_conj(x0, x2);
        v[1] = sub_swap(x1, x3);
        v[3] = add_swap(x1, x3);
    }
}
template <bool INVERSE>
__device__ __forceinline__ void bfly4_close(Cx A, Cx B, Cx C, Cx D, float2 &o0, float2 &o1, float2 &o2, float2 &o3) {
    v2f v[4] = {cx(A), cx(B), cx(C), cx(D)};
    bfly4_close_v<INVERSE>(v);
    o0 = make_float2(v[0].x, v[0].y);
    o1 = make_float2(v[1].x, v[1].y);
    o2 = make_float2(v[2].x, v[2].y);
    o3 = make_float2(v[3].x, v[3].y);
}

__device__ __forceinline__ Cx ld_cx(const float *a, int p) {
    float2 v = *reinterpret_cast<const float2 *>(a + 2 * p);
    return Cx{v.x, v.y};
}

template <int NC, bool INVERSE>
__device__ __forceinline__ void fft_complex_passes(float *a, const FftTables *T, int lane) {
    static_assert(NC / 4 <= 64, "one butterfly per lane");
    constexpr int BITS = (NC == 128) ? 7 : 6;
    constexpr int NB = NC / 4;
    {
        Cx A{0.f, 0.f}, B = A, C = A, D = A;
        const bool act = lane < NB;
        if (act) {
            const int r0 = dev_bitrev(lane, BITS - 2);
            A = ld_cx(a, r0);
            B = ld_cx(a, r0 + NC / 2);
            C = ld_cx(a, r0 + NC / 4);
            D = ld_cx(a, r0 + 3 * NC / 4);
        }
        wave_sync();
        if (act) bfly4_store(a, 4 * lane, 1, lane, T, A, B, C, D);
        wave_sync();
    }
#pragma unroll
    for (int hc = 4; hc * 4 < NC; hc *= 4) {
        if (lane < NB) {
            const int b = lane / hc, j = lane % hc, p0 = b * 4 * hc + j;
            bfly4_store(a, p0, hc, b, T, ld_cx(a, p0), ld_cx(a, p0 + hc), ld_cx(a, p0 + 2 * hc), ld_cx(a, p0 + 3 * hc));
        }
        wave_sync();
    }
    constexpr int HC = (NC == 128) ? 64 : 16;
    if constexpr (HC * 4 == NC) {
        if (lane < HC) {
            const int p0 = lane, p1 = p0 + HC, p2 = p1 + HC, p3 = p2 + HC;
            const Cx A = ld_cx(a, p0), B = ld_cx(a, p1), C = ld_cx(a, p2), D = ld_cx(a, p3);
            float2 o0, o1, o2, o3;
            bfly4_close<INVERSE>(A, B, C, D, o0, o1, o2, o3);
            *reinterpret_cast<float2 *>(a + 2 * p0) = o0;
            *reinterpret_cast<float2 *>(a + 2 * p1) = o1;
            *reinterpret_cast<float2 *>(a + 2 * p2) = o2;
            *reinterpret_cast<float2 *>(a + 2 * p3) = o3;
        }
    } else {
        for (int p0 = lane; p0 < HC; p0 += 64) {
            const int p1 = p0 + HC;
            const Cx A = ld_cx(a, p0), B = ld_cx(a, p1);
            float2 o0, o1;
            if constexpr (!INVERSE) {
                o0 = make_float2(A.r + B.r, A.i + B.i);
                o1 = make_float2(A.r - B.r, A.i - B.i);
            } else {
                o0 = make_float2(A.r + B.r, -A.i - B.i);
                o1 = make_float2(A.r - B.r, -A.i + B.i);
            }
            *reinterpret_cast<float2 *>(a + 2 * p0) = o0;
            *reinterpret_cast<float2 *>(a + 2 * p1) = o1;
        }
    }
    wave_sync();
}

template <int NC, bool INVERSE>
__device__ __forceinline__ void fft_real_split(float *a, const FftTables *T, int lane) {
    constexpr int NQ = NC / 2;
    for (int q = lane; q < NQ; q += 64) {
        if (q == 0) continue;
        const int j = 2 * q, k = 2 * NC - j;
        const float wkr = 0.5f - T->c[NQ - q], wki = T->c[q];
        const float aj = a[j], aj1 = a[j + 1], ak = a[k], ak1 = a[k + 1];
        const float xr = aj - ak, xi = aj1 + ak1;
        if constexpr (!INVERSE) {
            const float yr = wkr * xr - wki * xi, yi = wkr * xi + wki * xr;
            a[j] = aj - yr;
            a[j + 1] = aj1 - yi;
            a[k] = ak + yr;
            a[k + 1] = ak1 - yi;
        } else {
            const float yr = wkr * xr + wki * xi, yi = wkr * xi - wki * xr;
            a[j] = aj - yr;
            a[j + 1] = yi - aj1;
            a[k] = ak + yr;
            a[k + 1] = yi - ak1;
        }
    }
    if constexpr (INVERSE) {
        if (lane == 0) {
            a[1] = -a[1];
            a[NC + 1] = -a[NC + 1];
        }
    }
    wave_sync();
}

template <int NC>
__device__ __forceinline__ void rdft_forward(float *a, const FftTables *T, int lane) {
    fft_complex_passes<NC, false>(a, T, lane);
    fft_real_split<NC, false>(a, T, lane);
    if (lane == 0) {
        const float a0 = a[0], a1 = a[1];
        a[0] = a0 + a1;
        a[1] = a0 - a1;
    }
    wave_sync();
}

template <int NC>
__device__ __forceinline__ void rdft_inverse(float *a, const FftTables *T, int lane) {
    if (lane == 0) {
        const float a0 = a[0], a1 = a[1];
        const float h = 0.5f * (a0 - a1);
        a[1] = h;
        a[0] = a0 - h;
    }
    wave_sync();
    fft_real_split<NC, true>(a, T, lane);
    fft_complex_passes<NC, true>(a, T, lane);
}

}
```

wmix_amd/csrc/fft_regs.h:

```cpp
#pragma once
#include <cstddef>
#include "fft_ooura.h"

namespace wmx {

__device__ __forceinline__ int fft_group(int lane) { return lane & 3; }
__device__ __forceinline__ int fft_index(int lane) { return lane >> 2; }
template <int CTRL, int BANK_MASK = 0xf>
__device__ __forceinline__ float dpp_mov(float old, float v) {
    return __int_as_float(__builtin_amdgcn_update_dpp(__float_as_int(old), __float_as_int(v), CTRL, 0xf, BANK_MASK, false));
}
template <int X>
__device__ __forceinline__ void xstage1(float &lo, float &hi) {
    typedef unsigned v2u __attribute__((ext_vector_type(2)));
    if constexpr (X == 1) {
        const float nlo = dpp_mov<0x124, 0xA>(lo, hi);
        const float nhi = dpp_mov<0x12C, 0x5>(hi, lo);
        lo = nlo, hi = nhi;
    } else if constexpr (X == 2) {
        const float nlo = dpp_mov<0x128, 0xC>(lo, hi);
        const float nhi = dpp_mov<0x128, 0x3>(hi, lo);
        lo = nlo, hi = nhi;
    } else if constexpr (X == 4) {
        const v2u r = __builtin_amdgcn_permlane16_swap(__float_as_uint(lo), __float_as_uint(hi), false, false);
        lo = __uint_as_float(r.x), hi = __uint_as_float(r.y);
    } else {
        const v2u r = __builtin_amdgcn_permlane32_swap(__float_as_uint(lo), __float_as_uint(hi), false, false);
        lo = __uint_as_float(r.x), hi = __uint_as_float(r.y);
    }
}
template <int X>
__device__ __forceinline__ void xstage(v2f &lo, v2f &hi) {
    float lx = lo.x, hx = hi.x, ly = lo.y, hy = hi.y;
    xstage1<X>(lx, hx);
    xstage1<X>(ly, hy);
    lo = v2f{lx, ly};
    hi = v2f{hx, hy};
}

template <int XA, int XB>
__device__ __forceinline__ void transpose4(v2f v[4]) {
    xstage<XA>(v[0], v[1]);
    xstage<XA>(v[2], v[3]);
    xstage<XB>(v[0], v[2]);
    xstage<XB>(v[1], v[3]);
}

__device__ __forceinline__ int fft64_src_point(int gl, int m) {
    return dev_bitrev(gl, 4) + ((m & 1) << 5) + ((m & 2) << 3);
}

template <bool INVERSE>
__device__ __forceinline__ void fft64_regs(v2f v[4], const FftTables *T, int gl) {
    bfly4_v(gl, T, v);
    transpose4<1, 2>(v);
    bfly4_v(gl >> 2, T, v);
    transpose4<4, 8>(v);
    bfly4_close_v<INVERSE>(v);
}
template <bool INVERSE>
__device__ __forceinline__ void fft64_regs(Cx c[4], const FftTables *T, int gl) {
    v2f v[4] = {cx(c[0]), cx(c[1]), cx(c[2]), cx(c[3])};
    fft64_regs<INVERSE>(v, T, gl);
#pragma unroll
    for (int m = 0; m < 4; m++) c[m] = Cx{v[m].x, v[m].y};
}

struct Cx2 {
    v2f r, i;
};
__device__ __forceinline__ v2f bc(float x) { return v2f{x, x}; }

__device__ __forceinline__ void bfly4_x2(int b, const FftTables *T, Cx2 v[4]) {
    const v2f x0r = v[0].r + v[1].r, x0i = v[0].i + v[1].i, x1r = v[0].r - v[1].r, x1i = v[0].i - v[1].i;
    const v2f x2r = v[2].r + v[3].r, x2i = v[2].i + v[3].i, x3r = v[2].r - v[3].r, x3i = v[2].i - v[3].i;
    v[0].r = x0r + x2r;
    v[0].i = x0i + x2i;
    const v2f m = bc(b == 1 ? 1.f : 0.f);
    const v2f w1r = bc(T->W1[b][0]), w1i = bc(T->W1[b][1]), w2r = bc(T->W2[b][0]), w2i = bc(T->W2[b][1]);
    const v2f w3r = bc(T->W3[b][0]), w3i = bc(T->W3[b][1]);
    v2f tr = x0r - x2r, ti = x0i - x2i;
    v[2].r = w2r * tr - w2i * ti;
    v[2].i = w2r * ti + w2i * tr;
    tr = x1r - x3i;
    ti = x1i + x3r;
    {
        const v2f a = __builtin_elementwise_fma(-m, ti, tr), c = __builtin_elementwise_fma(m, tr, ti);
        tr = a;
        ti = c;
    }
    v[1].r = w1r * tr - w1i * ti;
    v[1].i = w1r * ti + w1i * tr;
    tr = x1r + x3i;
    ti = x1i - x3r;
    {
        const v2f a = __builtin_elementwise_fma(m, ti, tr), c = __builtin_elementwise_fma(-m, tr, ti);
        tr = a;
        ti = c;
    }
    v[3].r = w3r * tr - w3i * ti;
    v[3].i = w3r * ti + w3i * tr;
}

template <bool INVERSE>
__device__ __forceinline__ void bfly4_close_x2(Cx2 v[4]) {
    const v2f x0r = v[0].r + v[1].r, x1r = v[0].r - v[1].r, x2r = v[2].r + v[3].r, x2i = v[2].i + v[3].i, x3r = v[2].r - v[3].r,
              x3i = v[2].i - v[3].i;
    if constexpr (!INVERSE) {
        const v2f x0i = v[0].i + v[1].i, x1i = v[0].i - v[1].i;
        v[0] = Cx2{x0r + x2r, x0i + x2i};
        v[2] = Cx2{x0r - x2r, x0i - x2i};
        v[1] = Cx2{x1r - x3i, x1i + x3r};
        v[3] = Cx2{x1r + x3i, x1i - x3r};
    } else {
        const v2f x0i = -v[0].i - v[1].i, x1i = -v[0].i + v[1].i;
        v[0] = Cx2{x0r + x2r, x0i - x2i};
        v[2] = Cx2{x0r - x2r, x0i + x2i};
        v[1] = Cx2{x1r - x3i, x1i - x3r};
        v[3] = Cx2{x1r + x3i, x1i + x3r};
    }
}

template <int XA, int XB>
__device__ __forceinline__ void transpose4_x2(Cx2 v[4]) {
    xstage<XA>(v[0].r, v[1].r);
    xstage<XA>(v[0].i, v[1].i);
    xstage<XA>(v[2].r, v[3].r);
    xstage<XA>(v[2].i, v[3].i);
    xstage<XB>(v[0].r, v[2].r);
    xstage<XB>(v[0].i, v[2].i);
    xstage<XB>(v[1].r, v[3].r);
    xstage<XB>(v[1].i, v[3].i);
}

template <bool INVERSE>
__device__ __forceinline__ void fft64_regs_x2(Cx2 v[4], const FftTables *T, int gl) {
    bfly4_x2(gl, T, v);
    transpose4_x2<1, 2>(v);
    bfly4_x2(gl >> 2, T, v);
    transpose4_x2<4, 8>(v);
    bfly4_close_x2<INVERSE>(v);
}

__device__ __forceinline__ int mirror64(int p) {
    int q = (64 - p) & 63;
    asm("" : "+v"(q));
    return q;
}

__device__ __forceinline__ v2f ld_pt(const float *row, int p) {
    const float2 v = *reinterpret_cast<const float2 *>(row + 2 * p);
    return v2f{v.x, v.y};
}
__device__ __forceinline__ void st_pt(float *row, int p, v2f c) { *reinterpret_cast<float2 *>(row + 2 * p) = make_float2(c.x, c.y); }

template <int M>
__device__ __forceinline__ v2f rdft128_inv_point_m(const float *a, const FftTables *T, int b) {
    constexpr int OFF = M == 0 ? 0 : (M == 1 ? 32 : (M == 2 ? 16 : 48));
    const int p = dev_bitrev(b, 4) + OFF;
    const v2f own = ld_pt(a, p), other = ld_pt(a, mirror64(p));
    const int q = (M & 1) ? 64 - p : p;
    float wr = 0.5f - T->c[32 - q], wi = T->c[q];
    if constexpr (M == 1) {
        wr = b == 0 ? 0.f : wr;
        wi = b == 0 ? 0.f : wi;
    }
    const v2f x = own + v2f{-other.x, other.y};
    const v2f y = (M & 1) ? cmul_w(wr, wi, x) : cmul_w(wr, -wi, x);
    v2f out = conj_add(own, y);
    if constexpr (M == 0) {
        const float h = 0.5f * (own.x - own.y);
        out = b == 0 ? v2f{own.x - h, -h} : out;
    }
    return out;
}

__device__ __forceinline__ Cx2 rdft128_inv_point_x2(const float *a0, const float *a1, const FftTables *T, int b, int m) {
    v2f u, w;
    switch (m) {
        case 0: u = rdft128_inv_point_m<0>(a0, T, b), w = rdft128_inv_point_m<0>(a1, T, b); break;
        case 1: u = rdft128_inv_point_m<1>(a0, T, b), w = rdft128_inv_point_m<1>(a1, T, b); break;
        case 2: u = rdft128_inv_point_m<2>(a0, T, b), w = rdft128_inv_point_m<2>(a1, T, b); break;
        default: u = rdft128_inv_point_m<3>(a0, T, b), w = rdft128_inv_point_m<3>(a1, T, b); break;
    }
    return Cx2{v2f{u.x, w.x}, v2f{u.y, w.y}};
}

struct SplitLane {
    float wr, wi, z;
};
__device__ __forceinline__ SplitLane rdft128_fwd_coef(const FftTables *T, int lane) {
    const int q = lane < 32 ? lane : 64 - lane;
    float wr = 0.5f - T->c[32 - q], wi = T->c[q];
    wi = lane < 32 ? wi : -wi;
    wr = (lane & 31) == 0 ? 0.f : wr;
    wi = lane == 0 ? 0.5f : (lane == 32 ? 0.f : wi);
    return SplitLane{wr, wi, lane == 0 ? 0.f : 1.f};
}
__device__ __forceinline__ v2f rdft128_fwd_bin_u(const float *a, SplitLane s, int lane) {
    const v2f own = ld_pt(a, lane), other = ld_pt(a, mirror64(lane));
    const v2f x = own + v2f{-other.x, other.y};
    return (own - cmul_w(s.wr, s.wi, x)) * v2f{1.f, s.z};
}

__device__ __forceinline__ v2f lane_fetch(v2f v, int src_lane) {
    return v2f{__int_as_float(__builtin_amdgcn_ds_bpermute(src_lane << 2, __float_as_int(v.x))),
               __int_as_float(__builtin_amdgcn_ds_bpermute(src_lane << 2, __float_as_int(v.y)))};
}

template <int KIND>
__device__ __forceinline__ v2f bfly4_lane(int j, int b, const FftTables *T, v2f A, v2f B, v2f C, v2f D) {
    const float s1 = (j & 1) ? -1.f : 1.f, s2 = (j & 2) ? -1.f : 1.f;
    if constexpr (KIND == 2) {
        A.y = -A.y;
        B.y = -B.y;
    }
    const v2f xa = v2f{fmaf(s1, B.x, A.x), fmaf(s1, B.y, A.y)};
    const v2f xb = v2f{fmaf(s1, D.x, C.x), fmaf(s1, D.y, C.y)};
    v2f r;
    if constexpr (KIND == 2)
        r = (j & 1) ? v2f{-xb.y, -xb.x} : v2f{xb.x, -xb.y};
    else
        r = (j & 1) ? v2f{-xb.y, xb.x} : xb;
    v2f t = v2f{fmaf(s2, r.x, xa.x), fmaf(s2, r.y, xa.y)};
    if constexpr (KIND != 0) return t;
    const float ms = (b == 1 && (j & 1)) ? (j == 1 ? 1.f : -1.f) : 0.f;
    t = __builtin_elementwise_fma(v2f{-ms, ms}, swap(t), t);
    static_assert(offsetof(FftTables, W2) == offsetof(FftTables, W1) + 32 * 2 * sizeof(float) &&
                      offsetof(FftTables, W3) == offsetof(FftTables, W1) + 64 * 2 * sizeof(float),
                  "W1 | W2 | W3 contiguous");
    const float *wp = &T->W1[0][0] + 2 * (j == 0 ? 0 : (j - 1) * 32 + b);
    return cmul_w(wp[0], wp[1], t);
}

template <bool INVERSE>
__device__ __forceinline__ v2f fft64_lanes(v2f pt, const FftTables *T, int lane) {
    {
        const int bt = lane >> 2, r0 = dev_bitrev(bt, 4);
        const v2f A = lane_fetch(pt, r0), B = lane_fetch(pt, r0 + 32), C = lane_fetch(pt, r0 + 16), D = lane_fetch(pt, r0 + 48);
        pt = bfly4_lane<0>(lane & 3, bt, T, A, B, C, D);
    }
    {
        const int base = lane & 0x33;
        const v2f A = lane_fetch(pt, base), B = lane_fetch(pt, base + 4), C = lane_fetch(pt, base + 8), D = lane_fetch(pt, base + 12);
        pt = bfly4_lane<0>((lane >> 2) & 3, lane >> 4, T, A, B, C, D);
    }
    {
        const int base = lane & 15;
        const v2f A = lane_fetch(pt, base), B = lane_fetch(pt, base + 16), C = lane_fetch(pt, base + 32), D = lane_fetch(pt, base + 48);
        pt = bfly4_lane<INVERSE ? 2 : 1>(lane >> 4, 0, T, A, B, C, D);
    }
    return pt;
}

__device__ __forceinline__ v2f rdft128_inv_point_lanes(v2f own, const FftTables *T, int lane) {
    const v2f other = lane_fetch(own, mirror64(lane));
    const int q = lane < 32 ? lane : 64 - lane;
    const float wkr = 0.5f - T->c[32 - q], wki = T->c[q];
    const v2f aj = lane < 32 ? own : other, ak = lane < 32 ? other : own;
    const float xr = aj.x - ak.x, xi = aj.y + ak.y;
    const float yr = wkr * xr + wki * xi, yi = wkr * xi - wki * xr;
    float re = lane < 32 ? aj.x - yr : ak.x + yr;
    float im = lane < 32 ? yi - aj.y : yi - ak.y;
    const float h = 0.5f * (own.x - own.y);
    re = lane == 0 ? own.x - h : (lane == 32 ? own.x : re);
    im = lane == 0 ? -h : (lane == 32 ? -own.y : im);
    return v2f{re, im};
}

__device__ __forceinline__ float row_bitrev(float v, int lane) {
    const int src = (dev_bitrev(lane >> 2, 4) << 2) | (lane & 3);
    return __int_as_float(__builtin_amdgcn_ds_bpermute(src << 2, __float_as_int(v)));
}

}
```

wmix_amd/csrc/ns.hip:

```cpp
#include <cmath>
#include <vector>
#include "stage_life.h"
#include "fft_ooura.h"
#include "libm_dev.h"
#include "ns_layout.h"

namespace wmx {
namespace {

constexpr int kStartupShort = 50;
constexpr int kStartupLong = 200;
constexpr int kHistBins = 1000;
constexpr int kUpdateWindow = 500;
constexpr int kStartBand = 5;

constexpr int kNsWavesPerBlock = 4;

template <int L>
struct NsConstLds {
    FftTables tab;
    float window[L];
    float logi[NsLayout<L>::MP];
    NsLibmTables lm;
};
template <int L>
struct alignas(16) NsWaveLds {
    static constexpr int MP = NsLayout<L>::MP;
    float fa[L];
    float magn[MP], lmagn[MP], noise[MP], snrp[MP], sprob[MP], pause[MP];
    float r0[MP], r1[MP], r2[MP];
#ifdef WMX_NS_PROF
    unsigned long long prof[16];
#endif
};
#ifdef WMX_NS_PROF
__device__ unsigned long long g_ns_prof[16];
#define NS_PROF(i)                                                         \
    do {                                                                   \
        const long long t_now = clock64();                                 \
        if (lane == 0) W.prof[i] += (unsigned long long)(t_now - prof_t0); \
        prof_t0 = clock64();                                               \
    } while (0)
#else
#define NS_PROF(i)
#endif
static_assert(2 * NsLayout<256>::MP >= 256 && 2 * NsLayout<128>::MP >= 128, "r0..r1 must hold L floats");

__device__ __forceinline__ float sat16f(float v) { return v > 32767.f ? 32767.f : (v < -32768.f ? -32768.f : v); }

__device__ __forceinline__ float sum_range(const float *x, int lo, int hi, int lane) {
    float acc = 0.f;
    int i = lo;
#pragma unroll 1
    for (; i < hi && (i & 3); i++) acc += x[i];
#pragma unroll 4
    for (; i + 8 <= hi; i += 8) {
        const float4 a = *reinterpret_cast<const float4 *>(x + i), b = *reinterpret_cast<const float4 *>(x + i + 4);
        acc += a.x;
        acc += a.y;
        acc += a.z;
        acc += a.w;
        acc += b.x;
        acc += b.y;
        acc += b.z;
        acc += b.w;
    }
#pragma unroll 1
    for (; i < hi; i++) acc += x[i];
    return acc;
}

template <int MP4>
__device__ __forceinline__ float sum_lanes(const float *mine) {
    float acc = 0.f;
#pragma unroll 4
    for (int i = 0; i < MP4; i += 2) {
        const float4 a = *reinterpret_cast<const float4 *>(mine + 4 * i);
        acc += a.x;
        acc += a.y;
        acc += a.z;
        acc += a.w;
        if (i + 1 < MP4) {
            const float4 b = *reinterpret_cast<const float4 *>(mine + 4 * i + 4);
            acc += b.x;
            acc += b.y;
            acc += b.z;
            acc += b.w;
        }
    }
    return acc;
}
__device__ __noinline__ static float tanh_call(float x, const NsLibmTables *m) { return fast_tanh(x, *m); }
__device__ __forceinline__ float lane_value(float v, int k) { return __int_as_float(__builtin_amdgcn_readlane(__float_as_int(v), k)); }

template <int L, int CHN>
__device__ void ns_frame(const NsConstLds<L> &K, NsWaveLds<L> &W, float *__restrict__ st, unsigned short *__restrict__ hist,
                         const int16_t *in, int16_t *out, const int pkg, const int lane_in) {
    using Y = NsLayout<L>;
    constexpr int chn = CHN;
    int lane = lane_in;
#define NS_RELANE() asm volatile("" : "+v"(lane))
    NS_RELANE();
#ifdef WMX_NS_PROF
    long long prof_t0 = clock64();
#endif
    constexpr int M = Y::M, B = Y::B, NT = L / 64, NC = L / 2;
    struct StF {
        GlobalF g;
        unsigned i;
        __device__ __forceinline__ operator float() const { return row_ld(g, i); }
        __device__ __forceinline__ void operator=(float v) const { row_st(g, i, v); }
    };
    struct StI {
        GlobalF g;
        unsigned i;
        __device__ __forceinline__ operator int() const { return __float_as_int(row_ld(g, i)); }
        __device__ __forceinline__ void operator=(int v) const { row_st(g, i, __int_as_float(v)); }
    };
    const GlobalF st_row = global_row(st, 0);
#define ST(idx) (StF{st_row, (unsigned)(idx)})
#define STI(idx) (StI{st_row, (unsigned)(idx)})
    float *tdst = W.r0;

    const float scv = lane < 24 ? ST(Y::SCALARS + lane) : 0.f;
#define SCF(f) lane_value(scv, Y::f - Y::SCALARS)
#define SCI(f) __float_as_int(lane_value(scv, Y::f - Y::SCALARS))
    float buf[NT], hb[NT], synt[NT];
#pragma unroll
    for (int k = 0; k < NT; k++) {
        const int i = lane + 64 * k;
        constexpr int KEEP = L - B;
        const bool all_old = 64 * k + 63 < KEEP, all_new = 64 * k >= KEEP;
        const bool is_old = all_old || (!all_new && i < KEEP);
        float o = 0.f, oh = 0.f;
        int16_t n = 0, nh = 0;
        if (!all_new) o = ST(Y::IN_BUF + (is_old ? i + B : 0));
        if (!all_old) n = in[(is_old ? 0 : i - KEEP) * chn];
        buf[k] = is_old ? o : (float)n;
        synt[k] = (64 * k < KEEP && i < KEEP) ? ST(Y::SYNT_BUF + (i < KEEP ? i : 0)) : 0.f;
        hb[k] = 0.f;
        if (chn == 2) {
            if (!all_new) oh = ST(Y::HB_BUF + (is_old ? i + B : 0));
            if (!all_old) nh = in[(is_old ? 0 : i - KEEP) * chn + 1];
            hb[k] = is_old ? oh : (float)nh;
        }
    }
#if defined(WMX_NS_EXP) && WMX_NS_EXP == 1
    constexpr int NI = M / 64;
#else
    constexpr int NI = (M + 63) / 64;
#endif
    float pf_quant[NI], pf_dens[NI][3], pf_lq[NI][3], pf_pause[NI];
#pragma unroll
    for (int k = 0; k < NI; k++) {
        const int b = lane + 64 * k < M ? lane + 64 * k : M - 1;
        pf_pause[k] = ST(Y::MAGN_AVG_PAUSE + b);
        pf_quant[k] = ST(Y::QUANTILE + b);
#pragma unroll
        for (int q = 0; q < 3; q++) {
            pf_dens[k][q] = ST(Y::DENSITY + q * Y::MP + b);
            pf_lq[k][q] = ST(Y::LQUANTILE + q * Y::MP + b);
        }
    }
    wave_sync();
#pragma unroll
    for (int k = 0; k < NT; k++) {
        const int i = lane + 64 * k;
        if (64 * k + 63 < B) continue;
        if (i >= B) {
            ST(Y::IN_BUF + i) = buf[k];
            if (chn == 2) ST(Y::HB_BUF + i) = hb[k];
        }
    }
    float e1[NT];
    bool any_term = false;
#pragma unroll
    for (int k = 0; k < NT; k++) {
        const int i = lane + 64 * k;
        const float w = K.window[i] * buf[k];
        W.fa[i] = w;
        e1[k] = w * w;
        any_term |= e1[k] != 0.0f;
    }
    wave_sync();
    NS_PROF(0);

    float hb_gain = 1.f;
    const bool zero_frame = __builtin_amdgcn_ballot_w64(any_term) == 0;
    float t_re[(Y::M + 63) / 64], t_im[(Y::M + 63) / 64], t_prev[(Y::M + 63) / 64], t_snrq[(Y::M + 63) / 64];

    if (!zero_frame) {
        const int block_ind = SCI(S_BLOCK_IND) + 1;
        STI(Y::S_BLOCK_IND) = block_ind;
        const int update_flag = SCI(S_UPDATE_FLAG);
        const bool startup = block_ind < kStartupShort;
        const float overdrive = 1.1f, denoise_bound = 0.125f;

        NS_RELANE();
        rdft_forward<NC>(W.fa, &K.tab, lane);
        if (lane < Y::MP - M) W.r0[M + lane] = 0.f;
        NS_PROF(1);

        NS_RELANE();
#pragma unroll
        for (int k = 0; k < NI; k++) {
            const int b0 = lane + 64 * k;
            const bool ok = (64 * k + 63 < M) || b0 < M;
            const int b = ok ? b0 : M - 1;
            float re, im, mg;
            if (k == NI - 1) {
                re = W.fa[1];
                im = 0.f;
                mg = fabsf(re) + 1.f;
            } else {
                const float a0 = W.fa[2 * b], a1 = W.fa[2 * b + 1];
                const bool dc = k == 0 && b == 0;
                re = a0;
                im = dc ? 0.f : a1;
                const float g = sqrtf(re * re + im * im) + 1.f;
                mg = dc ? fabsf(re) + 1.f : g;
            }
            const float lm = fast_log_ge1(mg, K.lm);
            const float pz = pf_pause[k];
            t_re[k] = re;
            t_im[k] = im;
            if (!ok) continue;
            W.magn[b] = mg;
            W.lmagn[b] = lm;
            W.pause[b] = pz;
            W.r0[b] = re * re + im * im;
            W.r1[b] = b >= kStartBand ? K.logi[b] * lm : 0.f;
            W.r2[b] = b >= 1 ? lm : 0.f;
            W.snrp[b] = b >= kStartBand ? lm : 0.f;
        }
        wave_sync();
        NS_PROF(2);
        float signal_energy, sum_magn, avg_magn, flat_mean, avg_pause, sum_log_magn = 0.f, sum_log_i_log_magn = 0.f;
        {
            const float *mine =
                lane == 1 ? W.magn : (lane == 2 ? W.r2 : (lane == 3 ? W.pause : (lane == 4 ? W.snrp : (lane == 5 ? W.r1 : W.r0))));
            const float acc = sum_lanes<Y::MP / 4>(mine);
            const float mean = acc / ((float)M);
            signal_energy = lane_value(mean, 0);
            sum_magn = lane_value(acc, 1);
            avg_magn = lane_value(mean, 1);
            flat_mean = lane_value(mean, 2);
            avg_pause = lane_value(mean, 3);
            if (startup) {
                sum_log_magn = lane_value(acc, 4);
                sum_log_i_log_magn = lane_value(acc, 5);
            }
        }
        const float magn0 = W.magn[0];
        wave_sync();
        NS_PROF(3);

        NS_RELANE();
        int updates = SCI(S_UPDATES);
        if (updates < kStartupLong) updates++;
        STI(Y::S_UPDATES) = updates;
        const int cnt0 = SCI(S_COUNTER + 0), cnt1 = SCI(S_COUNTER + 1), cnt2 = SCI(S_COUNTER + 2);
        float pf_nprev[NI], pf_mprev[NI], pf_smooth[NI], pf_lrt[NI];
#pragma unroll
        for (int k = 0; k < NI; k++) {
            const int b = lane + 64 * k < M ? lane + 64 * k : M - 1;
            pf_nprev[k] = ST(Y::NOISE_PREV + b);
            pf_mprev[k] = ST(Y::MAGN_PREV + b);
            pf_smooth[k] = ST(Y::SMOOTH + b);
            pf_lrt[k] = ST(Y::LOG_LRT + b);
        }
#pragma unroll
        for (int k = 0; k < NI; k++) {
            const int b0 = lane + 64 * k;
            const bool ok = (64 * k + 63 < M) || b0 < M;
            const int b = ok ? b0 : M - 1;
            const float lm = W.lmagn[b];
            float quant = pf_quant[k], lq = 0.f;
#pragma unroll
            for (int q = 0; q < 3; q++) {
                const int cnt = q == 0 ? cnt0 : (q == 1 ? cnt1 : cnt2);
                const float c1 = (float)(cnt + 1), cf = (float)cnt;
                float dens = pf_dens[k][q];
                lq = pf_lq[k][q];
                float delta;
                if (dens > 1.0f)
                    delta = div_ordinary(40.f * 1.f, dens);
                else
                    delta = 40.f;
                lq += div_ordinary(lm > lq ? 0.25f * delta : -((1.f - 0.25f) * delta), c1);
                if (fabsf(lm - lq) < 0.01f) {
                    dens = div_ordinary(cf * dens + 1.f / (2.f * 0.01f), c1);
                    if (ok) ST(Y::DENSITY + q * Y::MP + b) = dens;
                }
                if (ok) ST(Y::LQUANTILE + q * Y::MP + b) = lq;
                if (cnt >= kStartupLong && updates >= kStartupLong) quant = fast_exp(lq, K.lm);
            }
            if (updates < kStartupLong) quant = fast_exp(lq, K.lm);
            if (ok) {
                if (updates < kStartupLong || cnt0 >= kStartupLong || cnt1 >= kStartupLong || cnt2 >= kStartupLong) ST(Y::QUANTILE + b) = quant;
                W.noise[b] = quant;
            }
        }
        STI(Y::S_COUNTER + 0) = cnt0 >= kStartupLong ? 1 : cnt0 + 1;
        STI(Y::S_COUNTER + 1) = cnt1 >= kStartupLong ? 1 : cnt1 + 1;
        STI(Y::S_COUNTER + 2) = cnt2 >= kStartupLong ? 1 : cnt2 + 1;

        NS_RELANE();
        NS_PROF(4);
        if (startup) {
            const float white = SCF(S_WHITE) + avg_magn * overdrive;
            ST(Y::S_WHITE) = white;
            const float sum_log_i = K.logi[Y::MP - 2], sum_log_i_sq = K.logi[Y::MP - 1];
            float t1 = sum_log_i_sq * ((float)(M - kStartBand));
            t1 -= (sum_log_i * sum_log_i);
            float t2 = (sum_log_i_sq * sum_log_magn - sum_log_i * sum_log_i_log_magn);
            float t3 = t2 / t1;
            if (t3 < 0.f) t3 = 0.f;
            const float pink_num = SCF(S_PINK_NUM) + t3;
            ST(Y::S_PINK_NUM) = pink_num;
            t2 = (sum_log_i * sum_log_magn);
            t2 -= ((float)(M - kStartBand)) * sum_log_i_log_magn;
            t3 = t2 / t1;
            if (t3 < 0.f) t3 = 0.f;
            if (t3 > 1.f) t3 = 1.f;
            const float pink_exp = SCF(S_PINK_EXP) + t3;
            ST(Y::S_PINK_EXP) = pink_exp;
            float pnum = 0.0f, pexp = 0.0f;
            if (pink_exp > 0.f) {
                pnum = exp_d(pink_num / (float)(block_ind + 1));
                pnum *= (float)(block_ind + 1);
                pexp = pink_exp / (float)(block_ind + 1);
            }
#pragma unroll 1
            for (int b = lane; b < M; b += 64) {
                float pn;
                if (pink_exp == 0.f) {
                    pn = white;
                } else {
                    const float band = (float)(b < kStartBand ? kStartBand : b);
                    pn = div_pow_d(pnum, band, pexp);
                }
                W.r1[b] = pn;
                float nz = W.noise[b];
                nz *= (float)(block_ind);
                const float t = pn * (float)(kStartupShort - block_ind);
                nz += (t / (float)(block_ind + 1));
                nz /= (float)kStartupShort;
                W.noise[b] = nz;
            }
        }
        float feat_norm = SCF(S_FEAT_NORM);
        if (block_ind < kStartupLong) {
            feat_norm *= (float)block_ind;
            feat_norm += signal_energy;
            feat_norm /= (float)(block_ind + 1);
        }

        NS_RELANE();
#pragma unroll
        for (int k = 0; k < NI; k++) {
            const int b0 = lane + 64 * k;
            const bool ok = (64 * k + 63 < M) || b0 < M;
            const int b = ok ? b0 : M - 1;
            const float mg = W.magn[b], nz = W.noise[b];
            const float np = pf_nprev[k];
            const float pe = div_ordinary(pf_mprev[k], np + 0.0001f) * pf_smooth[k];
            float sq = 0.f;
            if (mg > nz) sq = div_ordinary(mg, nz + 0.0001f) - 1.f;
            const float dm = mg - avg_magn, dp = W.pause[b] - avg_pause;
            t_prev[k] = pe;
            t_snrq[k] = sq;
            if (!ok) continue;
            W.r0[b] = dm * dp;
            W.r2[b] = dp * dp;
            W.lmagn[b] = dm * dm;
        }
#pragma unroll
        for (int k = 0; k < NI; k++) {
            const int b0 = lane + 64 * k;
            const bool ok = (64 * k + 63 < M) || b0 < M;
            const int b = ok ? b0 : M - 1;
            const float sp = 0.98f * t_prev[k] + (1.f - 0.98f) * t_snrq[k];
            const float t1 = 1.f + 2.f * sp;
            const float t2 = div_ordinary(2.f * sp, t1 + 0.0001f);
            const float bessel = (t_snrq[k] + 1.f) * t2;
            float v = pf_lrt[k];
            v += 0.5f * (bessel - fast_log_ge1(t1, K.lm) - v);
            if (!ok) continue;
            ST(Y::LOG_LRT + b) = v;
            W.sprob[b] = v;
        }
        wave_sync();
        NS_PROF(5);
        float feat_flat = SCF(S_FEAT_FLAT);
        {
            float den = sum_magn;
            den -= magn0;
            den = den / (float)M;
            const float tmp = fast_exp(flat_mean, K.lm) / den;
            feat_flat += 0.3f * (tmp - feat_flat);
        }
        float cov, var_pause, var_magn, ksum;
        {
            const float acc = sum_lanes<Y::MP / 4>(lane == 1 ? W.r2 : (lane == 2 ? W.lmagn : (lane == 3 ? W.sprob : W.r0)));
            const float mean = acc / ((float)M);
            cov = lane_value(mean, 0);
            var_pause = lane_value(mean, 1);
            var_magn = lane_value(mean, 2);
            ksum = lane_value(mean, 3);
        }
        wave_sync();
        NS_PROF(6);
        float feat_acc = SCF(S_FEAT_ACC) + signal_energy;
        float feat_diff = SCF(S_FEAT_DIFF);
        {
            float d = var_magn - (cov * cov) / (var_pause + 0.0001f);
            d = d / (feat_norm + 0.0001f);
            feat_diff += 0.3f * (d - feat_diff);
        }
        float feat_lrt = SCF(S_FEAT_LRT);
        float thr_lrt = SCF(S_THR_LRT), thr_flat = SCF(S_THR_FLAT), thr_diff = SCF(S_THR_DIFF);
        float w_lrt = SCF(S_W_LRT), w_flat = SCF(S_W_FLAT), w_diff = SCF(S_W_DIFF);
        if (update_flag >= 1) {
            const int countdown = SCI(S_COUNTDOWN) - 1;
            if (countdown > 0) {
                if (lane == 0) {
                    auto bump = [&](int i) { atomicAdd(reinterpret_cast<unsigned *>(hist) + (i >> 1), (i & 1) ? 0x10000u : 1u); };
                    if ((feat_lrt < kHistBins * 0.1f) && (feat_lrt >= 0.0f)) bump((int)(feat_lrt / 0.1f));
                    if ((feat_flat < kHistBins * 0.05f) && (feat_flat >= 0.0f)) bump(kHistBins + (int)(feat_flat / 0.05f));
                    if ((feat_diff < kHistBins * 0.1f) && (feat_diff >= 0.0f)) bump(2 * kHistBins + (int)(feat_diff / 0.1f));
                }
                STI(Y::S_COUNTDOWN) = countdown;
            } else {
                unsigned hc_[3][8];
#pragma unroll
                for (int w_ = 0; w_ < 3; w_++) {
                    const unsigned *hsrc_ = reinterpret_cast<const unsigned *>(hist + w_ * kHistBins);
#pragma unroll
                    for (int q = 0; q < 8; q++) {
                        const int d_ = 64 * q + lane;
                        const unsigned v_ = hsrc_[d_ < kHistBins / 2 ? d_ : 0];
                        hc_[w_][q] = d_ < kHistBins / 2 ? v_ : 0u;
                    }
                }
#define NS_WALK(which, ...)                                                                                        \
    {                                                                                                              \
        constexpr int CH_ = 2 * L, QPC_ = L / 64, NCH_ = 8 / QPC_;  \
        const unsigned(&c_)[8] = hc_[which];                                                                       \
        _Pragma("unroll") for (int part_ = 0; part_ < NCH_; part_++) {                                             \
            unsigned *stage_ = reinterpret_cast<unsigned *>(W.fa);                                                 \
            _Pragma("unroll") for (int q = 0; q < QPC_; q++) stage_[64 * q + lane] = c_[QPC_ * part_ + q];         \
            wave_sync();                                                                                           \
            const unsigned short *h16_ = reinterpret_cast<const unsigned short *>(W.fa);                           \
            _Pragma("unroll 1") for (int base = CH_ * part_; base < CH_ * part_ + CH_ && base < kHistBins; base += 64) { \
                const int hv = (int)h16_[base - CH_ * part_ + lane];                                               \
                unsigned long long m = __builtin_amdgcn_ballot_w64(hv != 0);                                       \
                while (m) {                                                                                        \
                    const int j = __builtin_ctzll(m);                                                              \
                    m &= m - 1;                                                                                    \
                    const int i = base + j, h = __builtin_amdgcn_readlane(hv, j);                                  \
                    __VA_ARGS__                                                                                    \
                }                                                                                                  \
            }                                                                                                      \
            wave_sync();                                                                                           \
        }                                                                                                          \
    }
                static_assert(L == 128 || L == 256, "the staging above is sized for these");
                float avg = 0.0f, avg_compl = 0.0f, avg_sq = 0.0f;
                int num = 0;
                NS_WALK(0, {
                    const float mid = ((float)i + 0.5f) * 0.1f;
                    if (mid <= 1.f) {
                        avg += h * mid;
                        num += h;
                    }
                    avg_sq += h * mid * mid;
                    avg_compl += h * mid;
                })
                if (num > 0) avg = avg / ((float)num);
                avg_compl = avg_compl / ((float)kUpdateWindow);
                avg_sq = avg_sq / ((float)kUpdateWindow);
                const float fluct = avg_sq - avg * avg_compl;
                if (fluct < 0.05f) {
                    thr_lrt = 1.f;
                } else {
                    thr_lrt = 1.2f * avg;
                    if (thr_lrt < 0.2f) thr_lrt = 0.2f;
                    if (thr_lrt > 1.f) thr_lrt = 1.f;
                }
                int w1a = 0, w2a = 0, w1b = 0, w2b = 0;
                float p1a = 0.0f, p2a = 0.0f, p1b = 0.0f, p2b = 0.0f;
                {
                    int max1 = 0, max2 = 0;
                    NS_WALK(1, {
                        const float mid = ((float)i + 0.5f) * 0.05f;
                        if (h > max1) {
                            max2 = max1, w2a = w1a, p2a = p1a;
                            max1 = h, w1a = h, p1a = mid;
                        } else if (h > max2) {
                            max2 = h, w2a = h, p2a = mid;
                        }
                    })
                }
                {
                    int max1 = 0, max2 = 0;
                    NS_WALK(2, {
                        const float mid = ((float)i + 0.5f) * 0.1f;
                        if (h > max1) {
                            max2 = max1, w2b = w1b, p2b = p1b;
                            max1 = h, w1b = h, p1b = mid;
                        } else if (h > max2) {
                            max2 = h, w2b = h, p2b = mid;
                        }
                    })
                }
#undef NS_WALK
                const int thres_weight = 150;
                int use_flat = 1, use_diff = 1;
                if ((fabsf(p2a - p1a) < 2 * 0.05f) && (w2a > 0.5f * w1a)) {
                    w1a += w2a;
                    p1a = 0.5f * (p1a + p2a);
                }
                if (w1a < thres_weight || p1a < 0.6f) use_flat = 0;
                if (use_flat == 1) {
                    thr_flat = 0.9f * p1a;
                    if (thr_flat < 0.1f) thr_flat = 0.1f;
                    if (thr_flat > 0.95f) thr_flat = 0.95f;
                }
                if ((fabsf(p2b - p1b) < 2 * 0.1f) && (w2b > 0.5f * w1b)) {
                    w1b += w2b;
                    p1b = 0.5f * (p1b + p2b);
                }
                thr_diff = 1.2f * p1b;
                if (w1b < thres_weight) use_diff = 0;
                if (thr_diff < 0.16f) thr_diff = 0.16f;
                if (thr_diff > 1.f) thr_diff = 1.f;
                if (fluct < 0.05f) use_diff = 0;
                const float fsum = (float)(1 + use_flat + use_diff);
                w_lrt = 1.f / fsum;
                w_flat = ((float)use_flat) / fsum;
                w_diff = ((float)use_diff) / fsum;
                wave_sync();
                for (int i = lane; i < 3 * kHistBins; i += 64) hist[i] = 0;
                STI(Y::S_COUNTDOWN) = kUpdateWindow;
                if (update_flag == 1) {
                    STI(Y::S_UPDATE_FLAG) = 0;
                } else {
                    feat_acc = feat_acc / ((float)kUpdateWindow);
                    feat_norm = 0.5f * (feat_acc + feat_norm);
                    feat_acc = 0.f;
                }
                ST(Y::S_THR_LRT) = thr_lrt;
                ST(Y::S_THR_FLAT) = thr_flat;
                ST(Y::S_THR_DIFF) = thr_diff;
                ST(Y::S_W_LRT) = w_lrt;
                ST(Y::S_W_FLAT) = w_flat;
                ST(Y::S_W_DIFF) = w_diff;
            }
        }
        ST(Y::S_FEAT_FLAT) = feat_flat;
        ST(Y::S_FEAT_DIFF) = feat_diff;
        ST(Y::S_FEAT_NORM) = feat_norm;
        ST(Y::S_FEAT_ACC) = feat_acc;

        NS_RELANE();
        NS_PROF(7);
        feat_lrt = ksum;
        ST(Y::S_FEAT_LRT) = feat_lrt;
        float prior = SCF(S_PRIOR);
        {
            float width = 4.0f;
            if (ksum < thr_lrt) width = 2.f * 4.0f;
            const float a0 = width * (ksum - thr_lrt);
            width = 4.0f;
            if (feat_flat > thr_flat) width = 2.f * 4.0f;
            const float a1 = (float)1 * width * (thr_flat - feat_flat);
            width = 4.0f;
            if (feat_diff < thr_diff) width = 2.f * 4.0f;
            const float a2 = width * (feat_diff - thr_diff);
            const float th = fast_tanh(lane == 1 ? a1 : (lane == 2 ? a2 : a0), K.lm);
            const float ind0 = 0.5f * (lane_value(th, 0) + 1.f);
            const float ind1 = 0.5f * (lane_value(th, 1) + 1.f);
            const float ind2 = 0.5f * (lane_value(th, 2) + 1.f);
            const float ind = w_lrt * ind0 + w_flat * ind1 + w_diff * ind2;
            prior += 0.1f * (ind - prior);
            if (prior > 1.f) prior = 1.f;
            if (prior < 0.01f) prior = 0.01f;
            ST(Y::S_PRIOR) = prior;
        }
        const float gain_prior = (1.f - prior) / (prior + 0.0001f);
#pragma unroll
        for (int k = 0; k < NI; k++) {
            const int b0 = lane + 64 * k;
            const bool ok = (64 * k + 63 < M) || b0 < M;
            const int b = ok ? b0 : M - 1;
            float inv = fast_exp(-W.sprob[b], K.lm);
            inv = gain_prior * inv;
            const float spb = 1.f / (1.f + inv);
            if (ok) W.sprob[b] = spb;
        }
        wave_sync();
        NS_PROF(8);
        NS_RELANE();
#pragma unroll
        for (int k = 0; k < NI; k++) {
            const int b0 = lane + 64 * k;
            const bool ok = (64 * k + 63 < M) || b0 < M;
            const int b = ok ? b0 : M - 1;
            const float ps = W.sprob[b], pn = 1.f - ps, mg = W.magn[b], np = pf_nprev[k];
            float gamma_old = 0.9f;
            if (b > 0 && W.sprob[b - 1] > 0.2f) gamma_old = 0.99f;
            const float tmp = gamma_old * np + (1.f - gamma_old) * (pn * mg + ps * np);
            float gamma = 0.9f;
            if (ps > 0.2f) gamma = 0.99f;
            if (ps < 0.2f) {
                float pz = W.pause[b];
                pz += 0.05f * (mg - pz);
                if (ok) ST(Y::MAGN_AVG_PAUSE + b) = pz;
            }
            float nz;
            if (gamma == gamma_old) {
                nz = tmp;
            } else {
                nz = gamma * np + (1.f - gamma) * (pn * mg + ps * np);
                if (tmp < nz) nz = tmp;
            }
            float init_est = 0.f;
            if (startup) {
                init_est = ST(Y::INIT_MAGN + b) + mg;
                if (ok) ST(Y::INIT_MAGN + b) = init_est;
            }
            float cur = 0.f;
            if (mg > nz) cur = div_ordinary(mg, nz + 0.0001f) - 1.f;
            const float snr = 0.98f * t_prev[k] + (1.f - 0.98f) * cur;
            float f = div_ordinary(snr, overdrive + snr);
            if (f < denoise_bound) f = denoise_bound;
            if (f > 1.f) f = 1.f;
            if (startup) {
                float ft = (init_est - overdrive * W.r1[b]);
                ft /= (init_est + 0.0001f);
                if (ft < denoise_bound) ft = denoise_bound;
                if (ft > 1.f) ft = 1.f;
                f *= (float)(block_ind);
                ft *= (float)(kStartupShort - block_ind);
                f += ft;
                f /= (float)(kStartupShort);
            }
            const float re = t_re[k] * f, im = t_im[k] * f;
            if (!ok) continue;
            ST(Y::SMOOTH + b) = f;
            ST(Y::MAGN_PREV + b) = mg;
            ST(Y::NOISE_PREV + b) = nz;
            W.snrp[b] = f;
            if (b == 0)
                W.fa[0] = re;
            else if (b == M - 1)
                W.fa[1] = re;
            else {
                W.fa[2 * b] = re;
                W.fa[2 * b + 1] = im;
            }
        }
        wave_sync();
        NS_PROF(9);
        NS_RELANE();
        rdft_inverse<NC>(W.fa, &K.tab, lane);
        NS_PROF(10);
        float td[NT];
#pragma unroll
        for (int k = 0; k < NT; k++) {
            const int i = lane + 64 * k;
            td[k] = W.fa[i] * (2.f / L);
            tdst[i] = td[k] * td[k];
        }
        wave_sync();
        NS_PROF(11);
        float factor = 1.f;
        if (block_ind > kStartupLong) {
#pragma unroll
            for (int k = 0; k < NT; k++) W.fa[lane + 64 * k] = e1[k];
            wave_sync();
            const float acc = sum_lanes<L / 4>(lane == 1 ? W.fa : tdst);
            const float energy2 = lane_value(acc, 0), energy1 = lane_value(acc, 1);
            float gain = sqrtf(energy2 / (energy1 + 1.f));
            float factor1 = 1.f, factor2 = 1.f;
            if (gain > 0.5f) {
                factor1 = 1.f + 1.3f * (gain - 0.5f);
                if (gain * factor1 > 1.f) factor1 = 1.f / gain;
            }
            if (gain < 0.5f) {
                if (gain <= denoise_bound) gain = denoise_bound;
                factor2 = 1.f - 0.3f * (0.5f - gain);
            }
            factor = prior * factor1 + (1.f - prior) * factor2;
        }
#pragma unroll
        for (int k = 0; k < NT; k++) {
            const int i = lane + 64 * k;
            const float w = K.window[i] * td[k];
            synt[k] += factor * w;
        }
        if (chn == 2) {
            constexpr int D = M / 4;
            float avg_prob = sum_range(W.sprob, M - D - 1, M - 1, lane);
            avg_prob = avg_prob / ((float)D);
            avg_prob *= sum_magn / sum_magn;
            float avg_gain = sum_range(W.snrp, M - D - 1, M - 1, lane);
            avg_gain = avg_gain / ((float)D);
            const float t = 2.f * avg_prob - 1.f;
            const float gain_mod = 0.5f * (1.f + tanh_call(1.0f * t, &K.lm));
            float g = 0.5f * gain_mod + 0.5f * avg_gain;
            if (avg_prob >= 0.5f) g = 0.25f * gain_mod + 0.75f * avg_gain;
            g = g * 1.0f;
            if (g < denoise_bound) g = denoise_bound;
            if (g > 1.f) g = 1.f;
            hb_gain = g;
        }
        wave_sync();
        NS_PROF(12);
    }

        NS_RELANE();
#pragma unroll
    for (int k = 0; k < NT; k++) {
        const int i = lane + 64 * k;
        if (i >= B) ST(Y::SYNT_BUF + i - B) = synt[k];
        tdst[i] = sat16f(synt[k]);
        if (chn == 2) W.fa[i] = zero_frame ? sat16f(hb[k]) : sat16f(hb_gain * hb[k]);
    }
    wave_sync();
    for (int i = lane; i < pkg; i += 64) {
        const float lo = (i < B) ? tdst[i] : 0.f;
        out[i * chn] = (int16_t)lo;
        if (chn == 2) out[i * chn + 1] = (int16_t)((i < B) ? W.fa[i] : 0.f);
    }
    wave_sync();
    NS_PROF(13);
#undef NS_RELANE
#undef SCF
#undef SCI
#undef ST
#undef STI
}

#ifndef WMX_NS_W128
#define WMX_NS_W128 7
#endif
#ifndef WMX_NS_W256
#define WMX_NS_W256 5
#endif
template <int L>
struct NsOcc {
    static constexpr int kWaves = L == 128 ? WMX_NS_W128 : WMX_NS_W256;
};
template <int L, int CHN>
__global__ __launch_bounds__(64 * kNsWavesPerBlock) __attribute__((amdgpu_waves_per_eu(NsOcc<L>::kWaves, NsOcc<L>::kWaves))) void ns_kernel(float *__restrict__ state, unsigned short *__restrict__ hists,
                                                                      const float *__restrict__ consts, const int16_t *in, int16_t *out,
                                                                      int n_streams, int n_packets, long stream_stride,
                                                                      long packet_stride, int pkg, const uint8_t *__restrict__ active) {
    using Y = NsLayout<L>;
    __shared__ NsConstLds<L> K;
    __shared__ NsWaveLds<L> Wv[kNsWavesPerBlock];
    {
        float *dst = reinterpret_cast<float *>(&K);
        constexpr int NCONST = sizeof(NsConstLds<L>) / 4, NIT = (NCONST + 64 * kNsWavesPerBlock - 1) / (64 * kNsWavesPerBlock);
        float c[NIT];
#pragma unroll
        for (int k = 0; k < NIT; k++) {
            const int i = threadIdx.x + 64 * kNsWavesPerBlock * k;
            c[k] = consts[i < NCONST ? i : 0];
        }
#pragma unroll
        for (int k = 0; k < NIT; k++) {
            const int i = threadIdx.x + 64 * kNsWavesPerBlock * k;
            if (i < NCONST) dst[i] = c[k];
        }
    }
    __syncthreads();
    const int lane = threadIdx.x & 63;
    const int wave = __builtin_amdgcn_readfirstlane(threadIdx.x >> 6);
    const int sidx = blockIdx.x * kNsWavesPerBlock + wave;
    if (!stream_active(active, sidx, n_streams)) return;
    float *st = state + (size_t)sidx * Y::WORDS;
    unsigned short *hist = hists + (size_t)sidx * 3 * kHistBins;
    {
        float *wb = Wv[wave].magn;
        constexpr int NARR = 9;
        if (lane < NARR * (Y::MP - Y::M)) wb[(lane / (Y::MP - Y::M)) * Y::MP + Y::M + lane % (Y::MP - Y::M)] = 0.f;
    }
#ifdef WMX_NS_PROF
    if (lane < 16) Wv[wave].prof[lane] = 0;
#endif
    for (int p = 0; p < n_packets; p++) {
        const size_t off = (size_t)sidx * stream_stride + (size_t)p * packet_stride;
        ns_frame<L, CHN>(K, Wv[wave], st, hist, in + off, out + off, pkg, lane);
    }
#ifdef WMX_NS_PROF
    if (lane < 16) atomicAdd(&g_ns_prof[lane], Wv[wave].prof[lane]);
#endif
}
#ifdef WMX_NS_PROF
extern "C" int wmx_debug_ns_prof(unsigned long long *out16, int reset) {
    (void)hipDeviceSynchronize();
    (void)hipMemcpyFromSymbol(out16, HIP_SYMBOL(g_ns_prof), sizeof(unsigned long long) * 16);
    if (reset) {
        unsigned long long z[16] = {0};
        (void)hipMemcpyToSymbol(HIP_SYMBOL(g_ns_prof), z, sizeof(z));
    }
    return 0;
}
#endif

}
}

struct wmx_ns {
    int device;
    int n_streams, chn, freq, L, pkg;
    float *d_state;
    unsigned short *d_hist;
    float *d_consts;
    float *d_tmpl;
    size_t words;
    wmx::StreamLife life;
};

namespace {

template <int L>
void build_ns_template(std::vector<float> &st, std::vector<float> &consts) {
    using Y = wmx::NsLayout<L>;
    st.assign(Y::WORDS, 0.f);
    int *sti = reinterpret_cast<int *>(st.data());
    for (int q = 0; q < 3; q++)
        for (int b = 0; b < Y::M; b++) {
            st[Y::LQUANTILE + q * Y::MP + b] = 8.f;
            st[Y::DENSITY + q * Y::MP + b] = 0.3f;
        }
    for (int q = 0; q < 3; q++) sti[Y::S_COUNTER + q] = (int)floor((float)(200 * (q + 1)) / (float)3);
    for (int b = 0; b < Y::M; b++) {
        st[Y::SMOOTH + b] = 1.f;
        st[Y::LOG_LRT + b] = 0.5f;
    }
    sti[Y::S_UPDATES] = 0;
    sti[Y::S_BLOCK_IND] = -1;
    sti[Y::S_UPDATE_FLAG] = 2;
    sti[Y::S_COUNTDOWN] = 500;
    st[Y::S_PRIOR] = 0.5f;
    st[Y::S_FEAT_FLAT] = 0.5f;
    st[Y::S_FEAT_LRT] = 0.5f;
    st[Y::S_FEAT_DIFF] = 0.5f;
    st[Y::S_THR_LRT] = 0.5f;
    st[Y::S_THR_FLAT] = 0.5f;
    st[Y::S_THR_DIFF] = 0.5f;
    st[Y::S_W_LRT] = 1.f;
    static_assert(offsetof(wmx::NsConstLds<L>, lm) == (wmx::kFftTableWords + L + Y::MP) * 4, "constants block layout");
    consts.assign(sizeof(wmx::NsConstLds<L>) / 4, 0.f);
    wmx::ns_libm_tables(reinterpret_cast<wmx::NsLibmTables *>(consts.data() + wmx::kFftTableWords + L + Y::MP));
    wmx::FftTables tab;
    wmx::fft_tables_ooura(L, &tab);
    std::memcpy(consts.data(), &tab, sizeof(tab));
    float *win = consts.data() + wmx::kFftTableWords;
    const int ramp = (L == 128) ? 48 : 96;
    const double half_pi = 1.5707963267948966;
    for (int i = 0; i < L; i++) {
        double v = (i < ramp) ? sin(half_pi * i / ramp) : (i < L - ramp ? 1.0 : sin(half_pi * (L - i) / ramp));
        win[i] = (float)(floor(v * 1e8 + 0.5) / 1e8);
    }
    float *logi = win + L;
    volatile float acc1 = 0.0f, acc2 = 0.0f;
    for (int i = 0; i < Y::M; i++) {
        float li = (i == 0) ? 0.f : (float)log((double)(float)i);
        logi[i] = li;
        if (i >= 5) {
            acc1 = acc1 + li;
            volatile float sq = li * li;
            acc2 = acc2 + sq;
        }
    }
// ... 275 lines not shown
```

wmix_amd/csrc/wmx_internal.h:

```cpp
#pragma once
#include <hip/hip_runtime.h>
#include <cstdarg>
#include <cstdint>
#include <cstdio>
#include <cstring>
#include <vector>
#include "../../include/wmix_amd.h"
#include "build_flags.h"
#include "leg_calls.h"

#ifdef WMX_FAULT_INJECTION
namespace wmx {
hipError_t fault_point();
}
#define WMX_FAULT_OR(expr) (wmx::fault_point() != hipSuccess ? hipErrorUnknown : (expr))
#else
#define WMX_FAULT_OR(expr) (expr)
#endif

#define WMX_HIP(expr)                                                         \
    do {                                                                      \
        hipError_t _e = WMX_FAULT_OR(expr);                                   \
        if (_e != hipSuccess) return wmx::hip_fail(_e, #expr, __FILE__, __LINE__); \
    } while (0)
// ... 56 lines not shown
        set_error("%s: d_pcm %p is not on a 2-byte boundary (the rows are read and written as int16)", entry, (const void *)d_pcm);
        return WMX_EINVAL;
    }
    return 0;
}

static inline int zeroed_block(void **out, size_t bytes, const char *what, size_t fill_off = 0, int fill = 0, size_t fill_bytes = 0) {
    void *p = nullptr;
    WMX_HIP(hipMalloc(&p, bytes));
    hipError_t e = hipMemset(p, 0, bytes);
    if (e == hipSuccess && fill_bytes) e = hipMemset(static_cast<uint8_t *>(p) + fill_off, fill, fill_bytes);
    if (e == hipSuccess) e = hipDeviceSynchronize();
    if (e != hipSuccess) {
        (void)hipFree(p);
        return hip_fail(e, what, __FILE__, __LINE__);
    }
    *out = p;
    return 0;
}

static inline int upload_idx(int32_t *&d_idx, size_t &cap, const int32_t *host_idx, int n, hipStream_t s) {
    WMX_HIP(hipStreamSynchronize(s));
    if ((size_t)n > cap) {
        if (d_idx) (void)hipFree(d_idx);
        d_idx = nullptr, cap = 0;
        WMX_HIP(hipMalloc(&d_idx, (size_t)n * sizeof(int32_t)));
        cap = (size_t)n;
    }
    WMX_HIP(hipMemcpy(d_idx, host_idx, (size_t)n * sizeof(int32_t), hipMemcpyHostToDevice));
    return 0;
}

bool runtime_exiting();

struct SchedCache {
    struct Entry {
        uint64_t k0, k1;
        void *p;
        size_t n;
        int device;
        uint64_t last_use;
        hipEvent_t ev;
    };
    static constexpr size_t kMax = 64;
    std::vector<Entry *> e;
    uint64_t tick = 0;
    SchedCache() = default;
    SchedCache(const SchedCache &) = delete;
    SchedCache &operator=(const SchedCache &) = delete;
    Entry *find(uint64_t k0, uint64_t k1) {
        for (Entry *x : e)
            if (x->k0 == k0 && x->k1 == k1) {
                x->last_use = ++tick;
                return x;
            }
        return nullptr;
    }
    static void drop(Entry *x) {
        if (!runtime_exiting()) {
            DeviceScope on(x->device);
            if (x->ev) {
                (void)hipEventSynchronize(x->ev);
                (void)hipEventDestroy(x->ev);
            }
            if (x->p) (void)hipFree(x->p);
        }
        delete x;
    }
    int add(uint64_t k0, uint64_t k1, const void *host, size_t bytes, size_t n, Entry **out) {
        if (e.size() >= kMax) {
            size_t lru = 0;
            for (size_t i = 1; i < e.size(); i++)
                if (e[i]->last_use < e[lru]->last_use) lru = i;
            drop(e[lru]);
            e.erase(e.begin() + (long)lru);
        }
        int dev = -1;
        WMX_HIP(hipGetDevice(&dev));
        void *p = nullptr;
        if (bytes) {
            WMX_HIP(hipMalloc(&p, bytes));
            hipError_t er = hipMemcpy(p, host, bytes, hipMemcpyHostToDevice);
            if (er != hipSuccess) {
                (void)hipFree(p);
                return hip_fail(er, "hipMemcpy(schedule)", __FILE__, __LINE__);
            }
        }
        Entry *x = new Entry{k0, k1, p, n, dev, ++tick, nullptr};
        e.push_back(x);
        *out = x;
        return 0;
    }
    int used(Entry *x, hipStream_t s) {
        if (!x->ev) WMX_HIP(hipEventCreateWithFlags(&x->ev, hipEventDisableTiming));
        WMX_HIP(hipEventRecord(x->ev, s));
        return 0;
    }
    void clear() {
        for (Entry *x : e) drop(x);
        e.clear();
    }
    ~SchedCache() { clear(); }
};

hipStream_t legacy_stream_create();
void legacy_stream_destroy(hipStream_t s);
hipStream_t thread_stream();

int aec_fork_far(wmx_aec *h, hipStream_t stream);
void aec_cancel_fork(wmx_aec *h);
int aecm_fork_far(wmx_aecm *h, hipStream_t stream);
void aecm_cancel_fork(wmx_aecm *h);
void chain_gate_after_ns(wmx_chain *h, hipEvent_t ev);
void chain_cohorts_when_made(wmx_chain *h, int n_cohorts, const int32_t *stream_cohort);

void zoom_gather_list(int inChn, int inFreq, uint32_t inLen, int outChn, int outFreq, std::vector<int32_t> &idx);

struct MixPlayView {
    int device, n_groups, chn, freq;
    uint32_t ring_bytes, head_off;
    int16_t *d_rings;
};
MixPlayView mix_play_view(const wmx_mix *m);
void mix_played(wmx_mix *m, uint32_t bytes);

#ifdef __HIPCC__
__device__ __forceinline__ void wave_sync() {
    __builtin_amdgcn_fence(__ATOMIC_ACQ_REL, "wavefront");
    __builtin_amdgcn_wave_barrier();
    __builtin_amdgcn_fence(__ATOMIC_ACQ_REL, "wavefront");
}
__device__ __forceinline__ void touch_line(const void *p, int &sink) {
    asm volatile("global_load_ubyte %0, %1, off" : "+v"(sink) : "v"(p) : "memory");
}
typedef float __attribute__((address_space(1))) *GlobalF;
typedef const float __attribute__((address_space(1))) *GlobalCF;
__device__ __forceinline__ GlobalF global_row(float *uniform_base, int word) {
    float *p = uniform_base + word;
    asm("" : "+s"(p));
    return (GlobalF)p;
}
__device__ __forceinline__ GlobalCF global_row(const float *uniform_base, int word) {
    const float *p = uniform_base + word;
    asm("" : "+s"(p));
    return (GlobalCF)p;
}
__device__ __forceinline__ float row_ld(GlobalCF row, unsigned idx) {
    return *(GlobalCF)((const char __attribute__((address_space(1))) *)row + 4u * idx);
}
__device__ __forceinline__ void row_st(GlobalF row, unsigned idx, float v) {
    *(GlobalF)((char __attribute__((address_space(1))) *)row + 4u * idx) = v;
}

template <class T>
__global__ void fill_rows_idx(T *state, const T *tmpl, int words, const int32_t *idx, int n_idx) {
    for (int j = blockIdx.x; j < n_idx; j += gridDim.x) {
        T *dst = state + (size_t)idx[j] * words;
        for (int i = threadIdx.x; i < words; i += blockDim.x) dst[i] = tmpl ? tmpl[i] : T(0);
    }
}
__device__ __forceinline__ bool stream_active(const uint8_t *active, int sidx, int n_streams) {
    return sidx < n_streams && (!active || active[sidx] != 0);
}
__device__ __forceinline__ void touch_done(int &sink) { asm volatile("s_waitcnt vmcnt(0)" : "+v"(sink) : : "memory"); }
#endif

}

#define WMX_LAUNCH_CHECK() WMX_HIP(hipGetLastError())

#define WMX_ON_DEVICE(h)                              \
    wmx::DeviceScope _dev_scope((h) ? (h)->device : -1); \
    WMX_HIP(_dev_scope.err)
```

Baseline: 62.27 million.

## Replace lane-index comparisons with constant inverse-ballot lane masks

Swaps per-lane predicates such as lane==0, lane<32 and group tests for compile-time 64-bit masks that are applied through the inverse-ballot builtin. These go straight into the exec/SGPR mask, so no VALU compares or VGPRs are spent on them. The change is threaded through the FFT helpers with an HwLanes tag and also reaches the NS kernel. It assumes a fixed wave64 lane layout and adds debug entry points for checking the masks.

```diff
diff --git a/include/wmix_amd.h b/include/wmix_amd.h
--- a/include/wmix_amd.h
+++ b/include/wmix_amd.h
@@ -403,6 +403,9 @@
 int wmx_debug_aec_decide_device(const float *d_sd_rows, const float *d_se_rows, const int32_t *d_prev_state, int32_t *d_out, size_t n, void *stream);
 int wmx_debug_pow(const float *x, const float *e, float *y, size_t n);
 int wmx_debug_pow_device(const float *d_x, const float *d_e, float *d_y, size_t n, void *stream);
+int wmx_debug_lane_sites(void);
+const char *wmx_debug_lane_site_name(int site);
+int wmx_debug_lane_masks(int block_threads, uint64_t diverge_mask, int32_t *d_out, void *stream);
 
 #ifdef __cplusplus
 }
diff --git a/wmix_amd/csrc/aec.hip b/wmix_amd/csrc/aec.hip
--- a/wmix_amd/csrc/aec.hip
+++ b/wmix_amd/csrc/aec.hip
@@ -98,14 +98,22 @@
     }
 }
 
+template <class Src, class... Map>
+__device__ __forceinline__ void aec_fft_fwd_map(float *row, const FftTables *T, int gl, Src src, Map... map) {
+    Cx v[4];
+#pragma unroll
+    for (int m = 0; m < 4; m++) v[m] = src(fft64_src_point(gl, m));
+    fft64_regs<false>(v, T, gl, map...);
+#pragma unroll
+    for (int m = 0; m < 4; m++) *reinterpret_cast<float2 *>(row + 2 * (gl + 16 * m)) = make_float2(v[m].r, v[m].i);
+}
 template <class Src>
 __device__ __forceinline__ void aec_fft_fwd(float *row, const FftTables *T, int gl, Src src) {
-    Cx v[4];
-#pragma unroll
-    for (int m = 0; m < 4; m++) v[m] = src(fft64_src_point(gl, m));
-    fft64_regs<false>(v, T, gl);
-#pragma unroll
-    for (int m = 0; m < 4; m++) *reinterpret_cast<float2 *>(row + 2 * (gl + 16 * m)) = make_float2(v[m].r, v[m].i);
+    aec_fft_fwd_map(row, T, gl, src);
+}
+template <class Src>
+__device__ __forceinline__ void aec_fft_fwd(float *row, const FftTables *T, int gl, HwLanes hw, Src src) {
+    aec_fft_fwd_map(row, T, gl, src, hw);
 }
 
 __global__ __launch_bounds__(64) void aec_far_kernel(AecFarBufs F_all, const float *__restrict__ consts_g, AecPlan *plans,
@@ -391,6 +399,8 @@
 template <int MULT>
 __device__ __forceinline__ void aec_block(const AecConstsNear &K, const float *__restrict__ curves_g, const PowTables *__restrict__ powtab, AecWaveLds &W, AecTaps &taps,
                                           const AecFarBufs &F, const AecBlkPlan &bp, const AecNoiseEntry *__restrict__ noise_tab, const int lane_in) {
+    using namespace site;
+    constexpr HwLanes hw{};
     int lane = opaque_lane(lane_in);
     int *Si = reinterpret_cast<int *>(W.st) - AS_LDS0;
     const float mu = MULT == 1 ? 0.6f : 0.5f, err_thr = MULT == 1 ? 2e-6f : 1.5e-6f;
@@ -407,7 +417,7 @@
         dctr++;
         if (dctr == 10 * MULT) dctr = 0;
         if (dctr == 0) blk_flags |= kAecFlagDelayEst;
-        if (lane == 0) {
+        if (lanes<aec_lane0>()) {
             Si[AS_NOISECTR] = nctr;
             Si[AS_DELAYCTR] = dctr;
         }
@@ -454,9 +464,9 @@
             y64 += nr * W.wn[p];
         }
         AEC_PROF(1);
-        v2f pt = rdft128_inv_point_lanes(v2f{y2.x, lane == 0 ? y64 : y2.y}, &K.tab, lane);
-        pt = fft64_lanes<true>(pt, &K.tab, lane);
-        if (lane >= 32) {
+        v2f pt = rdft128_inv_point_lanes(v2f{y2.x, lanes<aec_lane0>() ? y64 : y2.y}, &K.tab, lane, hw);
+        pt = fft64_lanes<true>(pt, &K.tab, lane, hw);
+        if (lanes<aec_upper>()) {
             const int i = 2 * (lane - 32);
             W.enew[i] = W.cur[i] - pt.x * scale;
             W.enew[i + 1] = W.cur[i + 1] - pt.y * scale;
@@ -465,15 +475,15 @@
     wave_sync();
     AEC_RELANE();
     {
-        const bool win = g & 1, err = g >= 2;
-        aec_fft_fwd(W.fa[g], &K.tab, gl, [&](int p) {
+        const bool win = lanes<aec_win>(), err = lanes<aec_err>();
+        aec_fft_fwd(W.fa[g], &K.tab, gl, hw, [&](int p) {
             const int i = 2 * (p & 31);
             float x0, x1, h0, h1;
             if (p < 32) {
                 const float *prev = &AEC_ST(err ? AS_EPREV : AS_DPREV);
                 x0 = prev[i], x1 = prev[i + 1];
                 h0 = K.hanning[i], h1 = K.hanning[i + 1];
-                if (g == 2) x0 = 0.f, x1 = 0.f;
+                if (lanes<aec_ef>()) x0 = 0.f, x1 = 0.f;
             } else {
                 const float *now = err ? W.enew : W.cur;
                 x0 = now[i], x1 = now[i + 1];
@@ -487,7 +497,7 @@
     AEC_RELANE();
     float dwr, dwi, dw64, dfr, dfi, df64;
     {
-        const SplitLane cf = rdft128_fwd_coef(&K.tab, lane);
+        const SplitLane cf = rdft128_fwd_coef(&K.tab, lane, hw);
         const v2f dwb = rdft128_fwd_bin_u(W.fa[1], cf, lane), dfb = rdft128_fwd_bin_u(W.fa[0], cf, lane);
         dwr = dwb.x, dwi = dwb.y, dw64 = W.fa[1][0] - W.fa[1][1];
         dfr = dfb.x, dfi = dfb.y, df64 = W.fa[0][0] - W.fa[0][1];
@@ -522,13 +532,13 @@
         put(lane, a);
 #if !defined(WMX_AEC_EXP) || WMX_AEC_EXP < 1
         const Pw c = power(kAecPart, df64, 0.f);
-        if (lane == 0) put(kAecPart, c);
+        if (lanes<aec_lane0>()) put(kAecPart, c);
 #endif
     }
     float ewr, ewi, ew64, efr, efi, ef64r, ef64i = 0.f;
     {
         {
-            const SplitLane cf = rdft128_fwd_coef(&K.tab, lane);
+            const SplitLane cf = rdft128_fwd_coef(&K.tab, lane, hw);
             const v2f ewb = rdft128_fwd_bin_u(W.fa[3], cf, lane), efb = rdft128_fwd_bin_u(W.fa[2], cf, lane);
             ewr = ewb.x, ewi = ewb.y, ew64 = W.fa[3][0] - W.fa[3][1];
             efr = efb.x, efi = efb.y, ef64r = W.fa[2][0] - W.fa[2][1];
@@ -592,22 +602,22 @@
             }
         }
         wave_sync();
-        if (lane < cnt) fa_row(W, lane)[1] = nyq_r * e64r - nyq_i * e64i;
+        if (pass == 0 ? lanes<aec_upd8>() : lanes<aec_upd4>()) fa_row(W, lane)[1] = nyq_r * e64r - nyq_i * e64i;
         wave_sync();
         AEC_RELANE();
         if (pass == 0) {
             float *row0 = W.fa[g], *row1 = W.fa[4 + g];
             Cx2 v[4];
 #pragma unroll
-            for (int m = 0; m < 4; m++) v[m] = rdft128_inv_point_x2(row0, row1, &K.tab, gl, m);
-            fft64_regs_x2<true>(v, &K.tab, gl);
+            for (int m = 0; m < 4; m++) v[m] = rdft128_inv_point_x2(row0, row1, &K.tab, gl, m, hw);
+            fft64_regs_x2<true>(v, &K.tab, gl, hw);
             const v2f sc = bc(scale), z = bc(0.f);
             const v2f ar = v[0].r * sc, ai = v[0].i * sc, cr = v[1].r * sc, ci = v[1].i * sc;
             v[0] = Cx2{v2f{row_bitrev(ar.x, lane), row_bitrev(ar.y, lane)}, v2f{row_bitrev(ai.x, lane), row_bitrev(ai.y, lane)}};
             v[2] = Cx2{v2f{row_bitrev(cr.x, lane), row_bitrev(cr.y, lane)}, v2f{row_bitrev(ci.x, lane), row_bitrev(ci.y, lane)}};
             v[1] = Cx2{z, z};
             v[3] = Cx2{z, z};
-            fft64_regs_x2<false>(v, &K.tab, gl);
+            fft64_regs_x2<false>(v, &K.tab, gl, hw);
 #pragma unroll
             for (int m = 0; m < 4; m++) {
                 *reinterpret_cast<float2 *>(row0 + 2 * (gl + 16 * m)) = make_float2(v[m].r.x, v[m].i.x);
@@ -617,10 +627,10 @@
             float *row = W.fa[g];
             Cx v[4];
             {
-                const v2f p0 = rdft128_inv_point_m<0>(row, &K.tab, gl), p1 = rdft128_inv_point_m<1>(row, &K.tab, gl);
-                const v2f p2 = rdft128_inv_point_m<2>(row, &K.tab, gl), p3 = rdft128_inv_point_m<3>(row, &K.tab, gl);
+                const v2f p0 = rdft128_inv_point_m<0>(row, &K.tab, gl, hw), p1 = rdft128_inv_point_m<1>(row, &K.tab, gl, hw);
+                const v2f p2 = rdft128_inv_point_m<2>(row, &K.tab, gl, hw), p3 = rdft128_inv_point_m<3>(row, &K.tab, gl, hw);
                 v[0] = Cx{p0.x, p0.y}, v[1] = Cx{p1.x, p1.y}, v[2] = Cx{p2.x, p2.y}, v[3] = Cx{p3.x, p3.y};
-                fft64_regs<true>(v, &K.tab, gl);
+                fft64_regs<true>(v, &K.tab, gl, hw);
             }
             const Cx a = Cx{row_bitrev(v[0].r * scale, lane), row_bitrev(v[0].i * scale, lane)};
             const Cx c = Cx{row_bitrev(v[1].r * scale, lane), row_bitrev(v[1].i * scale, lane)};
@@ -628,21 +638,21 @@
             v[1] = Cx{0.f, 0.f};
             v[2] = c;
             v[3] = Cx{0.f, 0.f};
-            fft64_regs<false>(v, &K.tab, gl);
+            fft64_regs<false>(v, &K.tab, gl, hw);
 #pragma unroll
             for (int m = 0; m < 4; m++) *reinterpret_cast<float2 *>(row + 2 * (gl + 16 * m)) = make_float2(v[m].r, v[m].i);
         }
         wave_sync();
         AEC_RELANE();
         {
-            const SplitLane cf = rdft128_fwd_coef(&K.tab, lane);
+            const SplitLane cf = rdft128_fwd_coef(&K.tab, lane, hw);
 #pragma unroll
             for (int q = 0; q < 8; q++) {
                 if (q >= cnt) continue;
                 const v2f d = rdft128_fwd_bin_u(W.fa[q], cf, lane);
                 taps.t[base + q] = taps.t[base + q] + d;
             }
-            if (lane < cnt) W.wn[base + lane] += fa_row(W, lane)[0] - fa_row(W, lane)[1];
+            if (pass == 0 ? lanes<aec_upd8>() : lanes<aec_upd4>()) W.wn[base + lane] += fa_row(W, lane)[0] - fa_row(W, lane)[1];
         }
         wave_sync();
     }
@@ -657,10 +667,13 @@
         for (int p = 0; p < 12; p++) {
             float *dst = W.fa[p >> 1] + (p & 1) * 66;
             dst[lane] = taps.t[p].x * taps.t[p].x + taps.t[p].y * taps.t[p].y;
-            if (lane == 0) dst[64] = W.wn[p] * W.wn[p] + 0.f * 0.f;
+        }
+        if (lanes<aec_lane0>()) {
+#pragma unroll
+            for (int p = 0; p < 12; p++) (W.fa[p >> 1] + (p & 1) * 66)[64] = W.wn[p] * W.wn[p] + 0.f * 0.f;
         }
         wave_sync();
-        if (lane < 12) {
+        if (lanes<aec_parts>()) {
             const float *src = W.fa[lane >> 1] + (lane & 1) * 66;
             float en = 0.f;
             for (int j = 0; j < kAecPart1; j++) en += src[j];
@@ -675,7 +688,7 @@
                 delayIdx = p;
             }
         wave_sync();
-        if (lane == 0) Si[AS_DELAYIDX] = delayIdx;
+        if (lanes<aec_lane0>()) Si[AS_DELAYIDX] = delayIdx;
     }
     AEC_PROF(4);
     {
@@ -686,7 +699,7 @@
         }
         xw[lane] = xwr_pre;
         xw[66 + lane] = xwi_pre;
-        if (lane == 0) {
+        if (lanes<aec_lane0>()) {
             xw[kAecPart] = uniform_ld(Xw + kAecPart);
             xw[66 + kAecPart] = uniform_ld(Xw + kAecPart1 + kAecPart);
         }
@@ -694,7 +707,7 @@
         dw[66 + lane] = dwi;
         ew[lane] = ewr;
         ew[66 + lane] = ewi;
-        if (lane == 0) {
+        if (lanes<aec_lane0>()) {
             dw[kAecPart] = dw64;
             dw[66 + kAecPart] = 0.f;
             ew[kAecPart] = ew64;
@@ -734,7 +747,7 @@
         put(lane, a);
 #if !defined(WMX_AEC_EXP) || WMX_AEC_EXP < 1
         const Psd c = psd(kAecPart);
-        if (lane == 0) put(kAecPart, c);
+        if (lanes<aec_lane0>()) put(kAecPart, c);
         float sd_t = a.sd, se_t = a.se;
         aec_gate_wave_sums(sd_t, se_t);
         gate = aec_gate_decide(sd_t + c.sd, se_t + c.se, Si[AS_DIVERGE]);
@@ -746,7 +759,7 @@
     int diverge = gate.diverge;
     bool reset_filter = gate.reset;
 #ifdef WMX_AEC_GATE_PROF
-    if (lane == 0) atomicAdd(&g_aec_gate[gate.decided ? 0 : 1], 1ull);
+    if (lanes<aec_lane0>()) atomicAdd(&g_aec_gate[gate.decided ? 0 : 1], 1ull);
 #endif
     if (!gate.decided) {
         float sdSum, seSum;
@@ -759,12 +772,13 @@
         reset_filter = seSum > (19.95f * sdSum);
     }
     wave_sync();
-    if (lane == 0) Si[AS_DIVERGE] = diverge;
+    if (lanes<aec_lane0>()) Si[AS_DIVERGE] = diverge;
     if (reset_filter) {
 #pragma unroll
-        for (int p = 0; p < 12; p++) {
-            taps.t[p] = v2f{0.f, 0.f};
-            if (lane == 0) W.wn[p] = 0.f;
+        for (int p = 0; p < 12; p++) taps.t[p] = v2f{0.f, 0.f};
+        if (lanes<aec_lane0>()) {
+#pragma unroll
+            for (int p = 0; p < 12; p++) W.wn[p] = 0.f;
         }
     }
     AEC_PROF(6);
@@ -774,7 +788,7 @@
     const uint2 jl = jump[(lane + 63) & 63], j64 = jump[63];
     const AecNoiseEntry nz = noise_tab[((nseed * jl.x + jl.y) & 0x7FFFFFFFu) >> 16];
     const float nz_c = nz.c, nz_s = nz.s;
-    if (lane == 0) Si[AS_NSEED] = (int)((nseed * j64.x + j64.y) & 0x7FFFFFFFu);
+    if (lanes<aec_lane0>()) Si[AS_NSEED] = (int)((nseed * j64.x + j64.y) & 0x7FFFFFFFu);
     {
         auto coh = [&](int b, float &cde, float &cxd) {
             const float sde_r = AEC_ST(AS_SDE_RE + b), sde_i = AEC_ST(AS_SDE_IM + b), sxd_r = AEC_ST(AS_SXD_RE + b),
@@ -795,7 +809,7 @@
         }
         t0[lane] = a0;
         t1[lane] = a1;
-        if (lane == 0) {
+        if (lanes<aec_lane0>()) {
             if (diverge) {
                 ew[kAecPart] = dw[kAecPart];
                 ew[66 + kAecPart] = dw[66 + kAecPart];
@@ -810,7 +824,7 @@
     hNlXdAvg = t1[5] * prefSize, hNlDeAvg = t0[5] * prefSize;
 #else
     {
-        const float *mine = lane == 1 ? t0 : t1;
+        const float *mine = lanes<aec_lane1>() ? t0 : t1;
         float acc = 0.f;
 #pragma unroll
         for (int i = minPref; i < prefSize + minPref; i++) acc += mine[i];
@@ -867,7 +881,7 @@
     if (mode == 2) {
 #endif
         constexpr int i75 = (int)(0.75f * (prefSize - 1)), i50 = (int)(0.5f * (prefSize - 1));
-        if (lane < prefSize) {
+        if (MULT == 1 ? lanes<aec_pref24>() : lanes<aec_pref12>()) {
             const float v = t2[minPref + lane];
             int rank = 0;
             for (int i = 0; i < prefSize; i++) {
@@ -905,7 +919,7 @@
         overDriveSm = 0.99f * overDriveSm + 0.01f * overDrive;
     else
         overDriveSm = 0.9f * overDriveSm + 0.1f * overDrive;
-    if (lane == 0) {
+    if (lanes<aec_lane0>()) {
         AEC_ST(AS_HNLXDAVGMIN) = hNlXdAvgMin;
         AEC_ST(AS_HNLFBMIN) = hNlFbMin;
         AEC_ST(AS_HNLFBLOCALMIN) = hNlFbLocalMin;
@@ -951,18 +965,18 @@
     AEC_PROF(8);
     AEC_RELANE();
     {
-        if (lane == 0) out_spec.y = out_nyq;
-        v2f pt = rdft128_inv_point_lanes(out_spec, &K.tab, lane);
-        pt = fft64_lanes<true>(pt, &K.tab, lane);
+        if (lanes<aec_lane0>()) out_spec.y = out_nyq;
+        v2f pt = rdft128_inv_point_lanes(out_spec, &K.tab, lane, hw);
+        pt = fft64_lanes<true>(pt, &K.tab, lane, hw);
         const int i = 2 * (lane & 31);
-        if (lane < 32) {
+        if (lanes<aec_lower>()) {
             const float o0 = sat16f(pt.x * scale * K.hanning[i] + AEC_ST(AS_OUTBUF + i));
             const float o1 = sat16f(pt.y * scale * K.hanning[i + 1] + AEC_ST(AS_OUTBUF + i + 1));
             AEC_ST(AS_OUT_RING + ring_at(bp.out_wr, i)) = o0;
             AEC_ST(AS_OUT_RING + ring_at(bp.out_wr, i + 1)) = o1;
         }
         wave_sync();
-        if (lane >= 32) {
+        if (lanes<aec_upper>()) {
             AEC_ST(AS_OUTBUF + i) = pt.x * scale * K.hanning[kAecPart - i];
             AEC_ST(AS_OUTBUF + i + 1) = pt.y * scale * K.hanning[kAecPart - i - 1];
         }
diff --git a/wmix_amd/csrc/fft_ooura.h b/wmix_amd/csrc/fft_ooura.h
--- a/wmix_amd/csrc/fft_ooura.h
+++ b/wmix_amd/csrc/fft_ooura.h
@@ -3,6 +3,7 @@
 #include <cmath>
 #include <cstring>
 #include "wmx_internal.h"
+#include "lane_sites.h"
 
 namespace wmx {
 
@@ -142,10 +143,10 @@
 #undef WMX_PK_ADD
 __device__ __forceinline__ v2f cmul_w(float wr, float wi, v2f t) { return v2f{wr, wr} * t + v2f{-wi, wi} * swap(t); }
 
-__device__ __forceinline__ void bfly4_v(int b, const FftTables *T, v2f v[4]) {
+__device__ __forceinline__ void bfly4_v(int b, const FftTables *T, v2f v[4], bool b1) {
     const v2f x0 = v[0] + v[1], x1 = v[0] - v[1], x2 = v[2] + v[3], x3 = v[2] - v[3];
     v[0] = x0 + x2;
-    const float m = b == 1 ? 1.f : 0.f;
+    const float m = b1 ? 1.f : 0.f;
     const float w1r = T->W1[b][0], w1i = T->W1[b][1], w2r = T->W2[b][0], w2i = T->W2[b][1];
     const float w3r = T->W3[b][0], w3i = T->W3[b][1];
     v2f t1 = add_i(x1, x3);
@@ -156,21 +157,22 @@
     v[1] = cmul_w(w1r, w1i, t1);
     v[3] = cmul_w(w3r, w3i, t3);
 }
+__device__ __forceinline__ void bfly4_v(int b, const FftTables *T, v2f v[4]) { bfly4_v(b, T, v, b == 1); }
 
 __device__ __forceinline__ void bfly4(int b, const FftTables *T, Cx A, Cx B, Cx C, Cx D, float2 &o0, float2 &o1, float2 &o2,
-                                      float2 &o3) {
+                                      float2 &o3, bool b1) {
     v2f v[4] = {cx(A), cx(B), cx(C), cx(D)};
-    bfly4_v(b, T, v);
+    bfly4_v(b, T, v, b1);
     o0 = make_float2(v[0].x, v[0].y);
     o1 = make_float2(v[1].x, v[1].y);
     o2 = make_float2(v[2].x, v[2].y);
     o3 = make_float2(v[3].x, v[3].y);
 }
 
-__device__ __forceinline__ void bfly4_store(float *a, int p0, int hc, int b, const FftTables *T, Cx A, Cx B, Cx C, Cx D) {
+__device__ __forceinline__ void bfly4_store(float *a, int p0, int hc, int b, const FftTables *T, Cx A, Cx B, Cx C, Cx D, bool b1) {
     const int p1 = p0 + hc, p2 = p1 + hc, p3 = p2 + hc;
     float2 o0, o1, o2, o3;
-    bfly4(b, T, A, B, C, D, o0, o1, o2, o3);
+    bfly4(b, T, A, B, C, D, o0, o1, o2, o3, b1);
     *reinterpret_cast<float2 *>(a + 2 * p0) = o0;
     *reinterpret_cast<float2 *>(a + 2 * p1) = o1;
     *reinterpret_cast<float2 *>(a + 2 * p2) = o2;
@@ -209,14 +211,24 @@
     return Cx{v.x, v.y};
 }
 
-template <int NC, bool INVERSE>
+template <bool HW, uint64_t M>
+__device__ __forceinline__ bool lane_pred(bool arith) {
+    if constexpr (HW)
+        return lanes<M>();
+    else
+        return arith;
+}
+
+template <int NC, bool INVERSE, bool HW = false>
 __device__ __forceinline__ void fft_complex_passes(float *a, const FftTables *T, int lane) {
+    using namespace site;
+    constexpr uint64_t kAct = NC == 128 ? oo128_act : oo64_act;
     static_assert(NC / 4 <= 64, "one butterfly per lane");
     constexpr int BITS = (NC == 128) ? 7 : 6;
     constexpr int NB = NC / 4;
     {
         Cx A{0.f, 0.f}, B = A, C = A, D = A;
-        const bool act = lane < NB;
+        const bool act = lane_pred<HW, kAct>(lane < NB);
         if (act) {
             const int r0 = dev_bitrev(lane, BITS - 2);
             A = ld_cx(a, r0);
@@ -225,20 +237,22 @@
             D = ld_cx(a, r0 + 3 * NC / 4);
         }
         wave_sync();
-        if (act) bfly4_store(a, 4 * lane, 1, lane, T, A, B, C, D);
+        if (act) bfly4_store(a, 4 * lane, 1, lane, T, A, B, C, D, lane_pred<HW, oo_p1_b1>(lane == 1));
         wave_sync();
     }
 #pragma unroll
     for (int hc = 4; hc * 4 < NC; hc *= 4) {
-        if (lane < NB) {
+        if (lane_pred<HW, kAct>(lane < NB)) {
             const int b = lane / hc, j = lane % hc, p0 = b * 4 * hc + j;
-            bfly4_store(a, p0, hc, b, T, ld_cx(a, p0), ld_cx(a, p0 + hc), ld_cx(a, p0 + 2 * hc), ld_cx(a, p0 + 3 * hc));
+            const bool b1 = hc == 4 ? lane_pred<HW, oo_hc4_b1>(b == 1) : lane_pred<HW, oo_hc16_b1>(b == 1);
+            bfly4_store(a, p0, hc, b, T, ld_cx(a, p0), ld_cx(a, p0 + hc), ld_cx(a, p0 + 2 * hc), ld_cx(a, p0 + 3 * hc), b1);
         }
         wave_sync();
     }
     constexpr int HC = (NC == 128) ? 64 : 16;
     if constexpr (HC * 4 == NC) {
-        if (lane < HC) {
+        static_assert(HC == 16, "site::oo64_close");
+        if (lane_pred<HW, oo64_close>(lane < HC)) {
             const int p0 = lane, p1 = p0 + HC, p2 = p1 + HC, p3 = p2 + HC;
             const Cx A = ld_cx(a, p0), B = ld_cx(a, p1), C = ld_cx(a, p2), D = ld_cx(a, p3);
             float2 o0, o1, o2, o3;
@@ -267,11 +281,11 @@
     wave_sync();
 }
 
-template <int NC, bool INVERSE>
+template <int NC, bool INVERSE, bool HW = false>
 __device__ __forceinline__ void fft_real_split(float *a, const FftTables *T, int lane) {
+    using namespace site;
     constexpr int NQ = NC / 2;
-    for (int q = lane; q < NQ; q += 64) {
-        if (q == 0) continue;
+    auto pair = [&](int q) {
         const int j = 2 * q, k = 2 * NC - j;
         const float wkr = 0.5f - T->c[NQ - q], wki = T->c[q];
         const float aj = a[j], aj1 = a[j + 1], ak = a[k], ak1 = a[k + 1];
@@ -289,9 +303,16 @@
             a[k] = ak + yr;
             a[k + 1] = yi - ak1;
         }
+    };
+    if constexpr (HW) {
+        static_assert(NQ == 64 || NQ == 32, "site::oo64_split");
+        if ((NQ == 64 || lanes<oo64_split>()) && !lanes<oo_lane0>()) pair(lane);
+    } else {
+        for (int q = lane; q < NQ; q += 64)
+            if (q != 0) pair(q);
     }
     if constexpr (INVERSE) {
-        if (lane == 0) {
+        if (lane_pred<HW, oo_lane0>(lane == 0)) {
             a[1] = -a[1];
             a[NC + 1] = -a[NC + 1];
         }
@@ -299,11 +320,11 @@
     wave_sync();
 }
 
-template <int NC>
+template <int NC, bool HW = false>
 __device__ __forceinline__ void rdft_forward(float *a, const FftTables *T, int lane) {
-    fft_complex_passes<NC, false>(a, T, lane);
-    fft_real_split<NC, false>(a, T, lane);
-    if (lane == 0) {
+    fft_complex_passes<NC, false, HW>(a, T, lane);
+    fft_real_split<NC, false, HW>(a, T, lane);
+    if (lane_pred<HW, site::oo_lane0>(lane == 0)) {
         const float a0 = a[0], a1 = a[1];
         a[0] = a0 + a1;
         a[1] = a0 - a1;
@@ -311,17 +332,25 @@
     wave_sync();
 }
 
-template <int NC>
+template <int NC, bool HW = false>
 __device__ __forceinline__ void rdft_inverse(float *a, const FftTables *T, int lane) {
-    if (lane == 0) {
+    if (lane_pred<HW, site::oo_lane0>(lane == 0)) {
         const float a0 = a[0], a1 = a[1];
         const float h = 0.5f * (a0 - a1);
         a[1] = h;
         a[0] = a0 - h;
     }
     wave_sync();
-    fft_real_split<NC, true>(a, T, lane);
-    fft_complex_passes<NC, true>(a, T, lane);
-}
-
-}
+    fft_real_split<NC, true, HW>(a, T, lane);
+    fft_complex_passes<NC, true, HW>(a, T, lane);
+}
+template <int NC>
+__device__ __forceinline__ void rdft_forward(float *a, const FftTables *T, int lane, HwLanes) {
+    rdft_forward<NC, true>(a, T, lane);
+}
+template <int NC>
+__device__ __forceinline__ void rdft_inverse(float *a, const FftTables *T, int lane, HwLanes) {
+    rdft_inverse<NC, true>(a, T, lane);
+}
+
+}
diff --git a/wmix_amd/csrc/fft_regs.h b/wmix_amd/csrc/fft_regs.h
--- a/wmix_amd/csrc/fft_regs.h
+++ b/wmix_amd/csrc/fft_regs.h
@@ -1,6 +1,7 @@
 #pragma once
 #include <cstddef>
 #include "fft_ooura.h"
+#include "lane_sites.h"
 
 namespace wmx {
 
@@ -59,9 +60,17 @@
     bfly4_close_v<INVERSE>(v);
 }
 template <bool INVERSE>
-__device__ __forceinline__ void fft64_regs(Cx c[4], const FftTables *T, int gl) {
+__device__ __forceinline__ void fft64_regs(v2f v[4], const FftTables *T, int gl, HwLanes) {
+    bfly4_v(gl, T, v, lanes<site::fft_p1_b1>());
+    transpose4<1, 2>(v);
+    bfly4_v(gl >> 2, T, v, lanes<site::fft_p2_b1>());
+    transpose4<4, 8>(v);
+    bfly4_close_v<INVERSE>(v);
+}
+template <bool INVERSE, class... Map>
+__device__ __forceinline__ void fft64_regs(Cx c[4], const FftTables *T, int gl, Map... map) {
     v2f v[4] = {cx(c[0]), cx(c[1]), cx(c[2]), cx(c[3])};
-    fft64_regs<INVERSE>(v, T, gl);
+    fft64_regs<INVERSE>(v, T, gl, map...);
 #pragma unroll
     for (int m = 0; m < 4; m++) c[m] = Cx{v[m].x, v[m].y};
 }
@@ -71,12 +80,12 @@
 };
 __device__ __forceinline__ v2f bc(float x) { return v2f{x, x}; }
 
-__device__ __forceinline__ void bfly4_x2(int b, const FftTables *T, Cx2 v[4]) {
+__device__ __forceinline__ void bfly4_x2(int b, const FftTables *T, Cx2 v[4], bool b1) {
     const v2f x0r = v[0].r + v[1].r, x0i = v[0].i + v[1].i, x1r = v[0].r - v[1].r, x1i = v[0].i - v[1].i;
     const v2f x2r = v[2].r + v[3].r, x2i = v[2].i + v[3].i, x3r = v[2].r - v[3].r, x3i = v[2].i - v[3].i;
     v[0].r = x0r + x2r;
     v[0].i = x0i + x2i;
-    const v2f m = bc(b == 1 ? 1.f : 0.f);
+    const v2f m = bc(b1 ? 1.f : 0.f);
     const v2f w1r = bc(T->W1[b][0]), w1i = bc(T->W1[b][1]), w2r = bc(T->W2[b][0]), w2i = bc(T->W2[b][1]);
     const v2f w3r = bc(T->W3[b][0]), w3i = bc(T->W3[b][1]);
     v2f tr = x0r - x2r, ti = x0i - x2i;
@@ -101,6 +110,7 @@
     v[3].r = w3r * tr - w3i * ti;
     v[3].i = w3r * ti + w3i * tr;
 }
+__device__ __forceinline__ void bfly4_x2(int b, const FftTables *T, Cx2 v[4]) { bfly4_x2(b, T, v, b == 1); }
 
 template <bool INVERSE>
 __device__ __forceinline__ void bfly4_close_x2(Cx2 v[4]) {
@@ -141,6 +151,14 @@
     transpose4_x2<4, 8>(v);
     bfly4_close_x2<INVERSE>(v);
 }
+template <bool INVERSE>
+__device__ __forceinline__ void fft64_regs_x2(Cx2 v[4], const FftTables *T, int gl, HwLanes) {
+    bfly4_x2(gl, T, v, lanes<site::fft_p1_b1>());
+    transpose4_x2<1, 2>(v);
+    bfly4_x2(gl >> 2, T, v, lanes<site::fft_p2_b1>());
+    transpose4_x2<4, 8>(v);
+    bfly4_close_x2<INVERSE>(v);
+}
 
 __device__ __forceinline__ int mirror64(int p) {
     int q = (64 - p) & 63;
@@ -155,33 +173,42 @@
 __device__ __forceinline__ void st_pt(float *row, int p, v2f c) { *reinterpret_cast<float2 *>(row + 2 * p) = make_float2(c.x, c.y); }
 
 template <int M>
-__device__ __forceinline__ v2f rdft128_inv_point_m(const float *a, const FftTables *T, int b) {
+__device__ __forceinline__ v2f rdft128_inv_point_m(const float *a, const FftTables *T, int b, bool b0) {
     constexpr int OFF = M == 0 ? 0 : (M == 1 ? 32 : (M == 2 ? 16 : 48));
     const int p = dev_bitrev(b, 4) + OFF;
     const v2f own = ld_pt(a, p), other = ld_pt(a, mirror64(p));
     const int q = (M & 1) ? 64 - p : p;
     float wr = 0.5f - T->c[32 - q], wi = T->c[q];
     if constexpr (M == 1) {
-        wr = b == 0 ? 0.f : wr;
-        wi = b == 0 ? 0.f : wi;
+        wr = b0 ? 0.f : wr;
+        wi = b0 ? 0.f : wi;
     }
     const v2f x = own + v2f{-other.x, other.y};
     const v2f y = (M & 1) ? cmul_w(wr, wi, x) : cmul_w(wr, -wi, x);
     v2f out = conj_add(own, y);
     if constexpr (M == 0) {
         const float h = 0.5f * (own.x - own.y);
-        out = b == 0 ? v2f{own.x - h, -h} : out;
+        out = b0 ? v2f{own.x - h, -h} : out;
     }
     return out;
 }
-
-__device__ __forceinline__ Cx2 rdft128_inv_point_x2(const float *a0, const float *a1, const FftTables *T, int b, int m) {
+template <int M>
+__device__ __forceinline__ v2f rdft128_inv_point_m(const float *a, const FftTables *T, int b) {
+    return rdft128_inv_point_m<M>(a, T, b, b == 0);
+}
+template <int M>
+__device__ __forceinline__ v2f rdft128_inv_point_m(const float *a, const FftTables *T, int gl, HwLanes) {
+    return rdft128_inv_point_m<M>(a, T, gl, lanes<site::fft_inv_b0>());
+}
+
+template <class... Map>
+__device__ __forceinline__ Cx2 rdft128_inv_point_x2(const float *a0, const float *a1, const FftTables *T, int b, int m, Map... map) {
     v2f u, w;
     switch (m) {
-        case 0: u = rdft128_inv_point_m<0>(a0, T, b), w = rdft128_inv_point_m<0>(a1, T, b); break;
-        case 1: u = rdft128_inv_point_m<1>(a0, T, b), w = rdft128_inv_point_m<1>(a1, T, b); break;
-        case 2: u = rdft128_inv_point_m<2>(a0, T, b), w = rdft128_inv_point_m<2>(a1, T, b); break;
-        default: u = rdft128_inv_point_m<3>(a0, T, b), w = rdft128_inv_point_m<3>(a1, T, b); break;
+        case 0: u = rdft128_inv_point_m<0>(a0, T, b, map...), w = rdft128_inv_point_m<0>(a1, T, b, map...); break;
+        case 1: u = rdft128_inv_point_m<1>(a0, T, b, map...), w = rdft128_inv_point_m<1>(a1, T, b, map...); break;
+        case 2: u = rdft128_inv_point_m<2>(a0, T, b, map...), w = rdft128_inv_point_m<2>(a1, T, b, map...); break;
+        default: u = rdft128_inv_point_m<3>(a0, T, b, map...), w = rdft128_inv_point_m<3>(a1, T, b, map...); break;
     }
     return Cx2{v2f{u.x, w.x}, v2f{u.y, w.y}};
 }
@@ -189,13 +216,19 @@
 struct SplitLane {
     float wr, wi, z;
 };
+__device__ __forceinline__ SplitLane rdft128_fwd_coef(const FftTables *T, int lane, bool lower, bool wr0, bool l0, bool l32) {
+    const int q = lower ? lane : 64 - lane;
+    float wr = 0.5f - T->c[32 - q], wi = T->c[q];
+    wi = lower ? wi : -wi;
+    wr = wr0 ? 0.f : wr;
+    wi = l0 ? 0.5f : (l32 ? 0.f : wi);
+    return SplitLane{wr, wi, l0 ? 0.f : 1.f};
+}
 __device__ __forceinline__ SplitLane rdft128_fwd_coef(const FftTables *T, int lane) {
-    const int q = lane < 32 ? lane : 64 - lane;
-    float wr = 0.5f - T->c[32 - q], wi = T->c[q];
-    wi = lane < 32 ? wi : -wi;
-    wr = (lane & 31) == 0 ? 0.f : wr;
-    wi = lane == 0 ? 0.5f : (lane == 32 ? 0.f : wi);
-    return SplitLane{wr, wi, lane == 0 ? 0.f : 1.f};
+    return rdft128_fwd_coef(T, lane, lane < 32, (lane & 31) == 0, lane == 0, lane == 32);
+}
+__device__ __forceinline__ SplitLane rdft128_fwd_coef(const FftTables *T, int lane, HwLanes) {
+    return rdft128_fwd_coef(T, lane, lanes<site::fwd_lower>(), lanes<site::fwd_wr0>(), lanes<site::fwd_lane0>(), lanes<site::fwd_lane32>());
 }
 __device__ __forceinline__ v2f rdft128_fwd_bin_u(const float *a, SplitLane s, int lane) {
     const v2f own = ld_pt(a, lane), other = ld_pt(a, mirror64(lane));
@@ -208,9 +241,12 @@
                __int_as_float(__builtin_amdgcn_ds_bpermute(src_lane << 2, __float_as_int(v.y)))};
 }
 
+struct Bfly4Pred {
+    bool j_odd, j_hi, rot_p, rot_m;
+};
 template <int KIND>
-__device__ __forceinline__ v2f bfly4_lane(int j, int b, const FftTables *T, v2f A, v2f B, v2f C, v2f D) {
-    const float s1 = (j & 1) ? -1.f : 1.f, s2 = (j & 2) ? -1.f : 1.f;
+__device__ __forceinline__ v2f bfly4_lane(int j, int b, const FftTables *T, v2f A, v2f B, v2f C, v2f D, Bfly4Pred P) {
+    const float s1 = P.j_odd ? -1.f : 1.f, s2 = P.j_hi ? -1.f : 1.f;
     if constexpr (KIND == 2) {
         A.y = -A.y;
         B.y = -B.y;
@@ -219,12 +255,12 @@
     const v2f xb = v2f{fmaf(s1, D.x, C.x), fmaf(s1, D.y, C.y)};
     v2f r;
     if constexpr (KIND == 2)
-        r = (j & 1) ? v2f{-xb.y, -xb.x} : v2f{xb.x, -xb.y};
+        r = P.j_odd ? v2f{-xb.y, -xb.x} : v2f{xb.x, -xb.y};
     else
-        r = (j & 1) ? v2f{-xb.y, xb.x} : xb;
+        r = P.j_odd ? v2f{-xb.y, xb.x} : xb;
     v2f t = v2f{fmaf(s2, r.x, xa.x), fmaf(s2, r.y, xa.y)};
     if constexpr (KIND != 0) return t;
-    const float ms = (b == 1 && (j & 1)) ? (j == 1 ? 1.f : -1.f) : 0.f;
+    const float ms = P.rot_p ? 1.f : (P.rot_m ? -1.f : 0.f);
     t = __builtin_elementwise_fma(v2f{-ms, ms}, swap(t), t);
     static_assert(offsetof(FftTables, W2) == offsetof(FftTables, W1) + 32 * 2 * sizeof(float) &&
                       offsetof(FftTables, W3) == offsetof(FftTables, W1) + 64 * 2 * sizeof(float),
@@ -232,40 +268,65 @@
     const float *wp = &T->W1[0][0] + 2 * (j == 0 ? 0 : (j - 1) * 32 + b);
     return cmul_w(wp[0], wp[1], t);
 }
-
-template <bool INVERSE>
+template <int KIND>
+__device__ __forceinline__ v2f bfly4_lane(int j, int b, const FftTables *T, v2f A, v2f B, v2f C, v2f D) {
+    const bool rot = b == 1 && (j & 1);
+    return bfly4_lane<KIND>(j, b, T, A, B, C, D, Bfly4Pred{(j & 1) != 0, (j & 2) != 0, rot && j == 1, rot && j != 1});
+}
+
+template <bool INVERSE, bool HW = false>
 __device__ __forceinline__ v2f fft64_lanes(v2f pt, const FftTables *T, int lane) {
+    using namespace site;
     {
         const int bt = lane >> 2, r0 = dev_bitrev(bt, 4);
         const v2f A = lane_fetch(pt, r0), B = lane_fetch(pt, r0 + 32), C = lane_fetch(pt, r0 + 16), D = lane_fetch(pt, r0 + 48);
-        pt = bfly4_lane<0>(lane & 3, bt, T, A, B, C, D);
+        if constexpr (HW)
+            pt = bfly4_lane<0>(lane & 3, bt, T, A, B, C, D, Bfly4Pred{lanes<l1_j_odd>(), lanes<l1_j_hi>(), lanes<l1_rot_p>(), lanes<l1_rot_m>()});
+        else
+            pt = bfly4_lane<0>(lane & 3, bt, T, A, B, C, D);
     }
     {
         const int base = lane & 0x33;
         const v2f A = lane_fetch(pt, base), B = lane_fetch(pt, base + 4), C = lane_fetch(pt, base + 8), D = lane_fetch(pt, base + 12);
-        pt = bfly4_lane<0>((lane >> 2) & 3, lane >> 4, T, A, B, C, D);
+        if constexpr (HW)
+            pt = bfly4_lane<0>((lane >> 2) & 3, lane >> 4, T, A, B, C, D, Bfly4Pred{lanes<l2_j_odd>(), lanes<l2_j_hi>(), lanes<l2_rot_p>(), lanes<l2_rot_m>()});
+        else
+            pt = bfly4_lane<0>((lane >> 2) & 3, lane >> 4, T, A, B, C, D);
     }
     {
         const int base = lane & 15;
         const v2f A = lane_fetch(pt, base), B = lane_fetch(pt, base + 16), C = lane_fetch(pt, base + 32), D = lane_fetch(pt, base + 48);
-        pt = bfly4_lane<INVERSE ? 2 : 1>(lane >> 4, 0, T, A, B, C, D);
+        if constexpr (HW)
+            pt = bfly4_lane<INVERSE ? 2 : 1>(lane >> 4, 0, T, A, B, C, D, Bfly4Pred{lanes<l3_j_odd>(), lanes<l3_j_hi>(), false, false});
+        else
+            pt = bfly4_lane<INVERSE ? 2 : 1>(lane >> 4, 0, T, A, B, C, D);
     }
     return pt;
 }
-
-__device__ __forceinline__ v2f rdft128_inv_point_lanes(v2f own, const FftTables *T, int lane) {
+template <bool INVERSE>
+__device__ __forceinline__ v2f fft64_lanes(v2f pt, const FftTables *T, int lane, HwLanes) {
+    return fft64_lanes<INVERSE, true>(pt, T, lane);
+}
+
+__device__ __forceinline__ v2f rdft128_inv_point_lanes(v2f own, const FftTables *T, int lane, bool lower, bool l0, bool l32) {
     const v2f other = lane_fetch(own, mirror64(lane));
-    const int q = lane < 32 ? lane : 64 - lane;
+    const int q = lower ? lane : 64 - lane;
     const float wkr = 0.5f - T->c[32 - q], wki = T->c[q];
-    const v2f aj = lane < 32 ? own : other, ak = lane < 32 ? other : own;
+    const v2f aj = lower ? own : other, ak = lower ? other : own;
     const float xr = aj.x - ak.x, xi = aj.y + ak.y;
     const float yr = wkr * xr + wki * xi, yi = wkr * xi - wki * xr;
-    float re = lane < 32 ? aj.x - yr : ak.x + yr;
-    float im = lane < 32 ? yi - aj.y : yi - ak.y;
+    float re = lower ? aj.x - yr : ak.x + yr;
+    float im = lower ? yi - aj.y : yi - ak.y;
     const float h = 0.5f * (own.x - own.y);
-    re = lane == 0 ? own.x - h : (lane == 32 ? own.x : re);
-    im = lane == 0 ? -h : (lane == 32 ? -own.y : im);
+    re = l0 ? own.x - h : (l32 ? own.x : re);
+    im = l0 ? -h : (l32 ? -own.y : im);
     return v2f{re, im};
+}
+__device__ __forceinline__ v2f rdft128_inv_point_lanes(v2f own, const FftTables *T, int lane) {
+    return rdft128_inv_point_lanes(own, T, lane, lane < 32, lane == 0, lane == 32);
+}
+__device__ __forceinline__ v2f rdft128_inv_point_lanes(v2f own, const FftTables *T, int lane, HwLanes) {
+    return rdft128_inv_point_lanes(own, T, lane, lanes<site::inv_lower>(), lanes<site::inv_lane0>(), lanes<site::inv_lane32>());
 }
 
 __device__ __forceinline__ float row_bitrev(float v, int lane) {
diff --git a/wmix_amd/csrc/lane_debug.hip b/wmix_amd/csrc/lane_debug.hip
--- /dev/null
+++ b/wmix_amd/csrc/lane_debug.hip
@@ -0,0 +1,49 @@
+#include "wmx_internal.h"
+#include "lane_sites.h"
+
+namespace wmx {
+namespace {
+
+#define WMX_LANE_SITE_COUNT(name, mask, arith) +1
+constexpr int kLaneSites = 0 WMX_LANE_SITES(WMX_LANE_SITE_COUNT);
+#undef WMX_LANE_SITE_COUNT
+#define WMX_LANE_SITE_NAME(name, mask, arith) #name,
+const char *const kLaneSiteNames[] = {WMX_LANE_SITES(WMX_LANE_SITE_NAME)};
+#undef WMX_LANE_SITE_NAME
+
+__device__ __forceinline__ void lane_sites_eval(int32_t *out, int threads, int t) {
+    const int lane = t & 63;
+    int row = 0;
+#define WMX_LANE_SITE_EVAL(name, mask, arith) \
+    out[(size_t)(row++) * threads + t] = (lanes<site::name>() ? 1 : 0) | ((arith) ? 2 : 0);
+    WMX_LANE_SITES(WMX_LANE_SITE_EVAL)
+#undef WMX_LANE_SITE_EVAL
+}
+
+__global__ void dbg_lane_sites(int32_t *out, uint64_t diverge_mask) {
+    const int t = threadIdx.x, threads = blockDim.x;
+    if (diverge_mask == ~0ull) {
+        lane_sites_eval(out, threads, t);
+    } else if ((diverge_mask >> (t & 63)) & 1ull) {
+        lane_sites_eval(out, threads, t);
+    }
+}
+
+}
+}
+
+extern "C" int wmx_debug_lane_sites(void) { return wmx::kLaneSites; }
+
+extern "C" const char *wmx_debug_lane_site_name(int site) {
+    return site >= 0 && site < wmx::kLaneSites ? wmx::kLaneSiteNames[site] : nullptr;
+}
+
+extern "C" int wmx_debug_lane_masks(int block_threads, uint64_t diverge_mask, int32_t *d_out, void *stream) {
+    using namespace wmx;
+    if (block_threads < 64 || block_threads > 1024 || block_threads % 64 != 0 || !d_out) return WMX_EINVAL;
+    hipStream_t s = as_stream(stream);
+    hipLaunchKernelGGL(dbg_lane_sites, dim3(1), dim3((unsigned)block_threads), 0, s, d_out, diverge_mask);
+    WMX_LAUNCH_CHECK();
+    WMX_HIP(hipStreamSynchronize(s));
+    return 0;
+}
diff --git a/wmix_amd/csrc/lane_sites.h b/wmix_amd/csrc/lane_sites.h
--- /dev/null
+++ b/wmix_amd/csrc/lane_sites.h
@@ -0,0 +1,84 @@
+#pragma once
+#include "wmx_internal.h"
+
+#define WMX_LANE_SITES(X)                                                                                              \
+                                                                                                        \
+    X(aec_lane0, lane_eq(0), lane == 0)                                                                                \
+    X(aec_lane1, lane_eq(1), lane == 1)                                                                                \
+    X(aec_lower, lane_lt(32), lane < 32)                                                                               \
+    X(aec_upper, lane_ge(32), lane >= 32)                                                                              \
+    X(aec_upd8, lane_lt(8), lane < 8)                                 \
+    X(aec_upd4, lane_lt(4), lane < 4)                                                     \
+    X(aec_parts, lane_lt(12), lane < 12)                                                                               \
+    X(aec_pref24, lane_lt(24), lane < 24)                                                \
+    X(aec_pref12, lane_lt(12), lane < 12)                                               \
+    X(aec_win, lane_bit(0), ((lane & 3) & 1) != 0)                                 \
+    X(aec_err, fft_g_ge(2), (lane & 3) >= 2)                                                 \
+    X(aec_ef, fft_g_eq(2), (lane & 3) == 2)                                                         \
+                                                                                        \
+    X(fft_p1_b1, fft_gl_eq(1), (lane >> 2) == 1)                                    \
+    X(fft_p2_b1, fft_gl_hi_eq(1), ((lane >> 2) >> 2) == 1)                     \
+    X(fft_inv_b0, fft_gl_eq(0), (lane >> 2) == 0)                                \
+    X(fwd_lower, lane_lt(32), lane < 32)                                                         \
+    X(fwd_wr0, lane_eq(0) | lane_eq(32), (lane & 31) == 0)                                                             \
+    X(fwd_lane0, lane_eq(0), lane == 0)                                                                                \
+    X(fwd_lane32, lane_eq(32), lane == 32)                                                                             \
+    X(inv_lower, lane_lt(32), lane < 32)                                                  \
+    X(inv_lane0, lane_eq(0), lane == 0)                                                                                \
+    X(inv_lane32, lane_eq(32), lane == 32)                                                                             \
+     \
+                                                                                       \
+    X(l1_j_odd, lane_bit(0), ((lane & 3) & 1) != 0)                                                                    \
+    X(l1_j_hi, lane_bit(1), ((lane & 3) & 2) != 0)                                                                     \
+    X(l1_rot_p, fft_gl_eq(1) & every(4, 1), (lane >> 2) == 1 && ((lane & 3) & 1) && (lane & 3) == 1)                   \
+    X(l1_rot_m, fft_gl_eq(1) & every(4, 3), (lane >> 2) == 1 && ((lane & 3) & 1) && (lane & 3) != 1)                   \
+    X(l2_j_odd, lane_bit(2), (((lane >> 2) & 3) & 1) != 0)                                                             \
+    X(l2_j_hi, lane_bit(3), (((lane >> 2) & 3) & 2) != 0)                                                              \
+    X(l2_rot_p, lanes_where(0x3c, 0x14), (lane >> 4) == 1 && (((lane >> 2) & 3) & 1) && ((lane >> 2) & 3) == 1)        \
+    X(l2_rot_m, lanes_where(0x3c, 0x1c), (lane >> 4) == 1 && (((lane >> 2) & 3) & 1) && ((lane >> 2) & 3) != 1)        \
+    X(l3_j_odd, lane_bit(4), ((lane >> 4) & 1) != 0)                                                                   \
+    X(l3_j_hi, lane_bit(5), ((lane >> 4) & 2) != 0)                                                                    \
+                     \
+    X(oo128_act, lane_lt(32), lane < 128 / 4)                                                           \
+    X(oo64_act, lane_lt(16), lane < 64 / 4)                                                                            \
+    X(oo_p1_b1, lane_eq(1), lane == 1)                                                           \
+    X(oo_hc4_b1, fft_gl_eq(1), lane / 4 == 1)                                              \
+    X(oo_hc16_b1, fft_gl_hi_eq(1), lane / 16 == 1)                                       \
+    X(oo64_close, lane_lt(16), lane < 16)                                   \
+    X(oo64_split, lane_lt(32), lane < 64 / 2)                            \
+    X(oo_lane0, lane_eq(0), lane == 0)                                                                                 \
+             \
+    X(ns128_bin_ok, ns<128>::bin_ok(1), lane + 64 < 65)                      \
+    X(ns256_bin_ok, ns<256>::bin_ok(2), lane + 128 < 129)                                                              \
+    X(ns128_old, ns<128>::old(0), lane < 48)                  \
+    X(ns256_old, ns<256>::old(1), lane + 64 < 96)                                                                      \
+    X(ns128_kept, ns<128>::kept(1), lane + 64 >= 80)                  \
+    X(ns256_kept, ns<256>::kept(2), lane + 128 >= 160)                                                                 \
+    X(ns128_tail, ns<128>::tail(), lane < 68 - 65)                                                  \
+    X(ns256_tail, ns<256>::tail(), lane < 132 - 129)                                                                   \
+    X(ns_dc, lane_eq(0), lane == 0)                                                                \
+    X(ns_from_band, lane_ge(5), lane >= 5)                                               \
+    X(ns_from_1, lane_ge(1), lane >= 1)                                                    \
+    X(ns_scalars, lane_lt(24), lane < 24)                                                                              \
+    X(ns_lane0, lane_eq(0), lane == 0)                                                                                 \
+    X(ns_pick1, lane_eq(1), lane == 1)                        \
+    X(ns_pick2, lane_eq(2), lane == 2)                                                                                 \
+    X(ns_pick3, lane_eq(3), lane == 3)                                                                                 \
+    X(ns_pick4, lane_eq(4), lane == 4)                                                                                 \
+    X(ns_pick5, lane_eq(5), lane == 5)
+
+namespace wmx {
+namespace site {
+template <int L>
+struct ns {
+    static constexpr int M = L / 2 + 1, MP = (M + 3) & ~3, B = L == 128 ? 80 : 160, KEEP = L - B;
+    static constexpr uint64_t bin_ok(int k) { return lane_plus_lt(64 * k, M); }
+    static constexpr uint64_t old(int k) { return lane_plus_lt(64 * k, KEEP); }
+    static constexpr uint64_t kept(int k) { return lane_plus_ge(64 * k, B); }
+    static constexpr uint64_t tail() { return lane_lt(MP - M); }
+};
+#define WMX_LANE_SITE_CONST(name, mask, arith) constexpr uint64_t name = (mask);
+WMX_LANE_SITES(WMX_LANE_SITE_CONST)
+#undef WMX_LANE_SITE_CONST
+}
+}
diff --git a/wmix_amd/csrc/ns.hip b/wmix_amd/csrc/ns.hip
--- a/wmix_amd/csrc/ns.hip
+++ b/wmix_amd/csrc/ns.hip
@@ -4,6 +4,7 @@
 #include "fft_ooura.h"
 #include "libm_dev.h"
 #include "ns_layout.h"
+#include "lane_sites.h"
 
 namespace wmx {
 namespace {
@@ -98,6 +99,8 @@
                          const int16_t *in, int16_t *out, const int pkg, const int lane_in) {
     using Y = NsLayout<L>;
     constexpr int chn = CHN;
+    using SL = site::ns<L>;
+    static_assert(SL::M == Y::M && SL::MP == Y::MP && SL::B == Y::B, "lane_sites.h restates the layout");
     int lane = lane_in;
 #define NS_RELANE() asm volatile("" : "+v"(lane))
     NS_RELANE();
@@ -122,7 +125,7 @@
 #define STI(idx) (StI{st_row, (unsigned)(idx)})
     float *tdst = W.r0;
 
-    const float scv = lane < 24 ? ST(Y::SCALARS + lane) : 0.f;
+    const float scv = lanes<site::ns_scalars>() ? ST(Y::SCALARS + lane) : 0.f;
 #define SCF(f) lane_value(scv, Y::f - Y::SCALARS)
 #define SCI(f) __float_as_int(lane_value(scv, Y::f - Y::SCALARS))
     float buf[NT], hb[NT], synt[NT];
@@ -131,13 +134,17 @@
         const int i = lane + 64 * k;
         constexpr int KEEP = L - B;
         const bool all_old = 64 * k + 63 < KEEP, all_new = 64 * k >= KEEP;
-        const bool is_old = all_old || (!all_new && i < KEEP);
+        static_assert(KEEP == SL::KEEP, "lane_sites.h restates the layout");
+        const bool is_old = all_old || (!all_new && lanes_in(SL::old(k)));
         float o = 0.f, oh = 0.f;
         int16_t n = 0, nh = 0;
         if (!all_new) o = ST(Y::IN_BUF + (is_old ? i + B : 0));
         if (!all_old) n = in[(is_old ? 0 : i - KEEP) * chn];
         buf[k] = is_old ? o : (float)n;
-        synt[k] = (64 * k < KEEP && i < KEEP) ? ST(Y::SYNT_BUF + (i < KEEP ? i : 0)) : 0.f;
+        if (64 * k + 63 < KEEP)
+            synt[k] = ST(Y::SYNT_BUF + i);
+        else
+            synt[k] = (64 * k < KEEP && lanes_in(SL::old(k))) ? ST(Y::SYNT_BUF + (lanes_in(SL::old(k)) ? i : 0)) : 0.f;
         hb[k] = 0.f;
         if (chn == 2) {
             if (!all_new) oh = ST(Y::HB_BUF + (is_old ? i + B : 0));
@@ -167,7 +174,7 @@
     for (int k = 0; k < NT; k++) {
         const int i = lane + 64 * k;
         if (64 * k + 63 < B) continue;
-        if (i >= B) {
+        if (64 * k >= B || lanes_in(SL::kept(k))) {
             ST(Y::IN_BUF + i) = buf[k];
             if (chn == 2) ST(Y::HB_BUF + i) = hb[k];
         }
@@ -197,16 +204,16 @@
         const float overdrive = 1.1f, denoise_bound = 0.125f;
 
         NS_RELANE();
-        rdft_forward<NC>(W.fa, &K.tab, lane);
-        if (lane < Y::MP - M) W.r0[M + lane] = 0.f;
+        rdft_forward<NC>(W.fa, &K.tab, lane, HwLanes{});
+        if (lanes<SL::tail()>()) W.r0[M + lane] = 0.f;
         NS_PROF(1);
 
         NS_RELANE();
 #pragma unroll
         for (int k = 0; k < NI; k++) {
             const int b0 = lane + 64 * k;
-            const bool ok = (64 * k + 63 < M) || b0 < M;
-            const int b = ok ? b0 : M - 1;
+            const bool ok = (64 * k + 63 < M) || lanes_in(SL::bin_ok(k));
+            const int b = (64 * k + 63 < M) ? b0 : M - 1;
             float re, im, mg;
             if (k == NI - 1) {
                 re = W.fa[1];
@@ -214,7 +221,7 @@
                 mg = fabsf(re) + 1.f;
             } else {
                 const float a0 = W.fa[2 * b], a1 = W.fa[2 * b + 1];
-                const bool dc = k == 0 && b == 0;
+                const bool dc = k == 0 && lanes<site::ns_dc>();
                 re = a0;
                 im = dc ? 0.f : a1;
                 const float g = sqrtf(re * re + im * im) + 1.f;
@@ -229,16 +236,18 @@
             W.lmagn[b] = lm;
             W.pause[b] = pz;
             W.r0[b] = re * re + im * im;
-            W.r1[b] = b >= kStartBand ? K.logi[b] * lm : 0.f;
-            W.r2[b] = b >= 1 ? lm : 0.f;
-            W.snrp[b] = b >= kStartBand ? lm : 0.f;
+            static_assert(kStartBand == 5, "site::ns_from_band");
+            const bool from_band = k > 0 || lanes<site::ns_from_band>(), from_1 = k > 0 || lanes<site::ns_from_1>();
+            W.r1[b] = from_band ? K.logi[b] * lm : 0.f;
+            W.r2[b] = from_1 ? lm : 0.f;
+            W.snrp[b] = from_band ? lm : 0.f;
         }
         wave_sync();
         NS_PROF(2);
         float signal_energy, sum_magn, avg_magn, flat_mean, avg_pause, sum_log_magn = 0.f, sum_log_i_log_magn = 0.f;
         {
             const float *mine =
-                lane == 1 ? W.magn : (lane == 2 ? W.r2 : (lane == 3 ? W.pause : (lane == 4 ? W.snrp : (lane == 5 ? W.r1 : W.r0))));
+                lanes<site::ns_pick1>() ? W.magn : (lanes<site::ns_pick2>() ? W.r2 : (lanes<site::ns_pick3>() ? W.pause : (lanes<site::ns_pick4>() ? W.snrp : (lanes<site::ns_pick5>() ? W.r1 : W.r0))));
             const float acc = sum_lanes<Y::MP / 4>(mine);
             const float mean = acc / ((float)M);
             signal_energy = lane_value(mean, 0);
@@ -272,8 +281,8 @@
 #pragma unroll
         for (int k = 0; k < NI; k++) {
             const int b0 = lane + 64 * k;
-            const bool ok = (64 * k + 63 < M) || b0 < M;
-            const int b = ok ? b0 : M - 1;
+            const bool ok = (64 * k + 63 < M) || lanes_in(SL::bin_ok(k));
+            const int b = (64 * k + 63 < M) ? b0 : M - 1;
             const float lm = W.lmagn[b];
             float quant = pf_quant[k], lq = 0.f;
 #pragma unroll
@@ -360,8 +369,8 @@
 #pragma unroll
         for (int k = 0; k < NI; k++) {
             const int b0 = lane + 64 * k;
-            const bool ok = (64 * k + 63 < M) || b0 < M;
-            const int b = ok ? b0 : M - 1;
+            const bool ok = (64 * k + 63 < M) || lanes_in(SL::bin_ok(k));
+            const int b = (64 * k + 63 < M) ? b0 : M - 1;
             const float mg = W.magn[b], nz = W.noise[b];
             const float np = pf_nprev[k];
             const float pe = div_ordinary(pf_mprev[k], np + 0.0001f) * pf_smooth[k];
@@ -378,8 +387,8 @@
 #pragma unroll
         for (int k = 0; k < NI; k++) {
             const int b0 = lane + 64 * k;
-            const bool ok = (64 * k + 63 < M) || b0 < M;
-            const int b = ok ? b0 : M - 1;
+            const bool ok = (64 * k + 63 < M) || lanes_in(SL::bin_ok(k));
+            const int b = (64 * k + 63 < M) ? b0 : M - 1;
             const float sp = 0.98f * t_prev[k] + (1.f - 0.98f) * t_snrq[k];
             const float t1 = 1.f + 2.f * sp;
             const float t2 = div_ordinary(2.f * sp, t1 + 0.0001f);
@@ -402,7 +411,7 @@
         }
         float cov, var_pause, var_magn, ksum;
         {
-            const float acc = sum_lanes<Y::MP / 4>(lane == 1 ? W.r2 : (lane == 2 ? W.lmagn : (lane == 3 ? W.sprob : W.r0)));
+            const float acc = sum_lanes<Y::MP / 4>(lanes<site::ns_pick1>() ? W.r2 : (lanes<site::ns_pick2>() ? W.lmagn : (lanes<site::ns_pick3>() ? W.sprob : W.r0)));
             const float mean = acc / ((float)M);
             cov = lane_value(mean, 0);
             var_pause = lane_value(mean, 1);
@@ -424,7 +433,7 @@
         if (update_flag >= 1) {
             const int countdown = SCI(S_COUNTDOWN) - 1;
             if (countdown > 0) {
-                if (lane == 0) {
+                if (lanes<site::ns_lane0>()) {
                     auto bump = [&](int i) { atomicAdd(reinterpret_cast<unsigned *>(hist) + (i >> 1), (i & 1) ? 0x10000u : 1u); };
                     if ((feat_lrt < kHistBins * 0.1f) && (feat_lrt >= 0.0f)) bump((int)(feat_lrt / 0.1f));
                     if ((feat_flat < kHistBins * 0.05f) && (feat_flat >= 0.0f)) bump(kHistBins + (int)(feat_flat / 0.05f));
@@ -578,7 +587,7 @@
             width = 4.0f;
             if (feat_diff < thr_diff) width = 2.f * 4.0f;
             const float a2 = width * (feat_diff - thr_diff);
-            const float th = fast_tanh(lane == 1 ? a1 : (lane == 2 ? a2 : a0), K.lm);
+            const float th = fast_tanh(lanes<site::ns_pick1>() ? a1 : (lanes<site::ns_pick2>() ? a2 : a0), K.lm);
             const float ind0 = 0.5f * (lane_value(th, 0) + 1.f);
             const float ind1 = 0.5f * (lane_value(th, 1) + 1.f);
             const float ind2 = 0.5f * (lane_value(th, 2) + 1.f);
@@ -592,8 +601,8 @@
 #pragma unroll
         for (int k = 0; k < NI; k++) {
             const int b0 = lane + 64 * k;
-            const bool ok = (64 * k + 63 < M) || b0 < M;
-            const int b = ok ? b0 : M - 1;
+            const bool ok = (64 * k + 63 < M) || lanes_in(SL::bin_ok(k));
+            const int b = (64 * k + 63 < M) ? b0 : M - 1;
             float inv = fast_exp(-W.sprob[b], K.lm);
             inv = gain_prior * inv;
             const float spb = 1.f / (1.f + inv);
@@ -605,11 +614,11 @@
 #pragma unroll
         for (int k = 0; k < NI; k++) {
             const int b0 = lane + 64 * k;
-            const bool ok = (64 * k + 63 < M) || b0 < M;
-            const int b = ok ? b0 : M - 1;
+            const bool ok = (64 * k + 63 < M) || lanes_in(SL::bin_ok(k));
+            const int b = (64 * k + 63 < M) ? b0 : M - 1;
             const float ps = W.sprob[b], pn = 1.f - ps, mg = W.magn[b], np = pf_nprev[k];
             float gamma_old = 0.9f;
-            if (b > 0 && W.sprob[b - 1] > 0.2f) gamma_old = 0.99f;
+            if ((k > 0 || lanes<site::ns_from_1>()) && W.sprob[b - 1] > 0.2f) gamma_old = 0.99f;
             const float tmp = gamma_old * np + (1.f - gamma_old) * (pn * mg + ps * np);
             float gamma = 0.9f;
             if (ps > 0.2f) gamma = 0.99f;
@@ -652,9 +661,9 @@
             ST(Y::MAGN_PREV + b) = mg;
             ST(Y::NOISE_PREV + b) = nz;
             W.snrp[b] = f;
-            if (b == 0)
+            if (k == 0 && lanes<site::ns_dc>())
                 W.fa[0] = re;
-            else if (b == M - 1)
+            else if (k == NI - 1)
                 W.fa[1] = re;
             else {
                 W.fa[2 * b] = re;
@@ -664,7 +673,7 @@
         wave_sync();
         NS_PROF(9);
         NS_RELANE();
-        rdft_inverse<NC>(W.fa, &K.tab, lane);
+        rdft_inverse<NC>(W.fa, &K.tab, lane, HwLanes{});
         NS_PROF(10);
         float td[NT];
 #pragma unroll
@@ -680,7 +689,7 @@
 #pragma unroll
             for (int k = 0; k < NT; k++) W.fa[lane + 64 * k] = e1[k];
             wave_sync();
-            const float acc = sum_lanes<L / 4>(lane == 1 ? W.fa : tdst);
+            const float acc = sum_lanes<L / 4>(lanes<site::ns_pick1>() ? W.fa : tdst);
             const float energy2 = lane_value(acc, 0), energy1 = lane_value(acc, 1);
             float gain = sqrtf(energy2 / (energy1 + 1.f));
             float factor1 = 1.f, factor2 = 1.f;
@@ -724,7 +733,7 @@
 #pragma unroll
     for (int k = 0; k < NT; k++) {
         const int i = lane + 64 * k;
-        if (i >= B) ST(Y::SYNT_BUF + i - B) = synt[k];
+        if (64 * k >= B || (64 * k + 63 >= B && lanes_in(SL::kept(k)))) ST(Y::SYNT_BUF + i - B) = synt[k];
         tdst[i] = sat16f(synt[k]);
         if (chn == 2) W.fa[i] = zero_frame ? sat16f(hb[k]) : sat16f(hb_gain * hb[k]);
     }
diff --git a/wmix_amd/csrc/wmx_internal.h b/wmix_amd/csrc/wmx_internal.h
--- a/wmix_amd/csrc/wmx_internal.h
+++ b/wmix_amd/csrc/wmx_internal.h
@@ -232,6 +232,39 @@
     *(GlobalF)((char __attribute__((address_space(1))) *)row + 4u * idx) = v;
 }
 
+template <uint64_t M>
+__device__ __forceinline__ bool lanes() {
+    return __builtin_amdgcn_inverse_ballot_w64(M);
+}
+__device__ __forceinline__ bool lanes_in(uint64_t m) { return __builtin_amdgcn_inverse_ballot_w64(m); }
+struct HwLanes {};
+constexpr uint64_t lane_lt(int n) { return n <= 0 ? 0ull : (n >= 64 ? ~0ull : (1ull << n) - 1ull); }
+constexpr uint64_t lane_ge(int n) { return ~lane_lt(n); }
+constexpr uint64_t lane_eq(int n) { return n < 0 || n > 63 ? 0ull : 1ull << n; }
+constexpr uint64_t lane_plus_lt(int off, int n) { return lane_lt(n - off); }
+constexpr uint64_t lane_plus_ge(int off, int n) { return lane_ge(n - off); }
+constexpr uint64_t lanes_where(int and_mask, int value) {
+    uint64_t m = 0;
+    for (int l = 0; l < 64; l++)
+        if ((l & and_mask) == value) m |= 1ull << l;
+    return m;
+}
+constexpr uint64_t every(int period, int phase) {
+    uint64_t m = 0;
+    for (int l = 0; l < 64; l++)
+        if (l % period == phase) m |= 1ull << l;
+    return m;
+}
+constexpr uint64_t lane_bit(int k) { return lanes_where(1 << k, 1 << k); }
+constexpr uint64_t fft_g_eq(int g) { return every(4, g); }
+constexpr uint64_t fft_g_ge(int g) {
+    uint64_t m = 0;
+    for (int k = g < 0 ? 0 : g; k < 4; k++) m |= every(4, k);
+    return m;
+}
+constexpr uint64_t fft_gl_eq(int n) { return lanes_where(0x3c, n << 2); }
+constexpr uint64_t fft_gl_hi_eq(int n) { return lanes_where(0x30, n << 4); }
+
 template <class T>
 __global__ void fill_rows_idx(T *state, const T *tmpl, int words, const int32_t *idx, int n_idx) {
     for (int j = blockIdx.x; j < n_idx; j += gridDim.x) {
```

Measured after the change: 63.41 million (median of 6 runs). +1.8%, better.
